# mackelab/poisson-gpfa

Measured on AMD Instinct MI355X. Metric: EM iterations/sec, higher is better.
Workload: dtype f64

## Files before the change

### poisson-gpfa_amd/csrc/core.hip

```cpp
#include "ctx.h"
#include "model.h"
#include "dual.h"
#include "thin.h"
#include "hook.h"
#include "plan.h"

using namespace pgpfa;

static_assert(plan::Dims{}.NB == NB && plan::Dims{}.WIDE_MAX == WIDE_MAX, "plan.h restates two constants of the kernel headers (workspace.hip includes none)");

thread_local std::string g_err;
thread_local unsigned long long g_fail_count = 0;

int fail(const char* fmt, ...) {
  char buf[1024];
  va_list ap;
  va_start(ap, fmt);
  vsnprintf(buf, sizeof(buf), fmt, ap);
  va_end(ap);
  g_err = buf;
  ++g_fail_count;
  return 1;
}

// ... 147 lines not shown
  c->dl_used = 0;
  return 0;
}
int dl_enqueue(pgpfa_ctx* c, void* host, const void* dev, size_t bytes) {
  if (bytes == 0) return 0;
  if (!c->dl_stage) {
    if (hipHostMalloc((void**)&c->dl_stage, DL_STAGE_BYTES, hipHostMallocMapped) != hipSuccess) { (void)hipGetLastError(); c->dl_stage = nullptr; }
    if (c->dl_stage && hipHostGetDevicePointer((void**)&c->dl_stage_dev, c->dl_stage, 0) != hipSuccess) { (void)hipGetLastError(); c->dl_stage_dev = nullptr; }
    if (!c->h_seq) {
      if (hipHostMalloc((void**)&c->h_seq, 64, hipHostMallocMapped) != hipSuccess ||
          hipHostGetDevicePointer((void**)&c->d_seq, c->h_seq, 0) != hipSuccess) { (void)hipGetLastError(); c->h_seq = nullptr; c->d_seq = nullptr; }
      if (c->h_seq) *c->h_seq = 0u;
    }
  }
  const size_t need = (bytes + 63) / 64 * 64;
  if (!c->dl_stage || need > DL_STAGE_BYTES) {
    CHK(dl_flush(c));
    const hipError_t e_copy = hipMemcpyAsync(host, dev, bytes, hipMemcpyDeviceToHost, c->st);
    if (e_copy != hipSuccess) return fail("device-to-host copy of %zu bytes: %s", bytes, hipGetErrorString(e_copy));
    return dl_flush(c);
  }
  dl_drop_stale(c);
  if (c->dl_used + need > DL_STAGE_BYTES) CHK(dl_flush(c));
  if (c->copy_kernels && c->dl_stage_dev && c->h_seq && bytes <= COPY_KERNEL_MAX && (bytes & 3) == 0 && (((size_t)dev) & 3) == 0) {
    const size_t nw = bytes / 4;
    hipLaunchKernelGGL(copy_words_kernel, dim3((unsigned)std::min<size_t>((nw + 255) / 256, 64)), dim3(256), 0, c->st,
                       reinterpret_cast<unsigned*>(c->dl_stage_dev + c->dl_used), reinterpret_cast<const unsigned*>(dev), nw);
    HIPC(hipGetLastError());
  } else {
    HIPC(hipMemcpyAsync(c->dl_stage + c->dl_used, dev, bytes, hipMemcpyDeviceToHost, c->st));
  }
  if (c->dl_pending.empty()) c->dl_fail_mark = g_fail_count;
  c->dl_pending.push_back({host, c->dl_used, bytes});
  c->dl_used += need;
  return 0;
}
int download(pgpfa_ctx* c, double* host, const double* dev, size_t n) {
  if (c->hbuf && host >= c->hbuf && host < c->hbuf + c->hbuf_len) {
    if (c->copy_kernels && n * sizeof(double) <= COPY_KERNEL_MAX) {
      CHK(dl_enqueue(c, host, dev, n * sizeof(double)));
      return dl_flush(c);
    }
    HIPC(hipMemcpyAsync(host, dev, n * sizeof(double), hipMemcpyDeviceToHost, c->st));
    return dl_flush(c);
  }
  CHK(dl_enqueue(c, host, dev, n * sizeof(double)));
  return dl_flush(c);
}
int upload(pgpfa_ctx* c, double* dev, const double* host, size_t n) {
  if (n * sizeof(double) <= (size_t)65536) return upload_nosync(c, dev, host, n * sizeof(double));
  HIPC(hipMemcpyAsync(dev, host, n * sizeof(double), hipMemcpyHostToDevice, c->st));
  HIPC(hipStreamSynchronize(c->st));
  c->ring_pending = 0;
  return 0;
}
constexpr int RING_N = 16;
int upload_nosync(pgpfa_ctx* c, void* dev, const void* host, size_t bytes) {
  if (bytes == 0) return 0;
  if (bytes > c->ring_slot) {
    HIPC(hipStreamSynchronize(c->st));
    if (c->ring) hipHostFree(c->ring);
    c->ring = nullptr; c->ring_dev = nullptr;
    const size_t slot = (bytes + 4095) / 4096 * 4096;
    HIPC(hipHostMalloc((void**)&c->ring, slot * RING_N, hipHostMallocMapped));
    if (hipHostGetDevicePointer((void**)&c->ring_dev, c->ring, 0) != hipSuccess) { (void)hipGetLastError(); c->ring_dev = nullptr; }
    c->ring_slot = slot; c->ring_cur = 0; c->ring_pending = 0;
  }
  if (c->ring_pending >= RING_N - 1) { HIPC(hipStreamSynchronize(c->st)); c->ring_pending = 0; }
  char* slot = c->ring + (size_t)c->ring_cur * c->ring_slot;
  std::memcpy(slot, host, bytes);
  if (c->copy_kernels && c->ring_dev && bytes <= COPY_KERNEL_MAX && (bytes & 3) == 0 && (((size_t)dev) & 3) == 0) {
    const size_t nw = bytes / 4;
    hipLaunchKernelGGL(copy_words_kernel, dim3((unsigned)std::min<size_t>((nw + 255) / 256, 64)), dim3(256), 0, c->st, reinterpret_cast<unsigned*>(dev),
                       reinterpret_cast<const unsigned*>(c->ring_dev + (size_t)c->ring_cur * c->ring_slot), nw);
    HIPC(hipGetLastError());
  } else {
    HIPC(hipMemcpyAsync(dev, slot, bytes, hipMemcpyHostToDevice, c->st));
  }
  c->ring_cur = (c->ring_cur + 1) % RING_N;
  c->ring_pending += 1;
  return 0;
}


int build_kinv(pgpfa_ctx* c) {
  c->kinv_serial += 1;
  const size_t slab = (size_t)c->Tp * c->Tp;
  CHK(copy_dev(c, c->kws.H, c->Kpad, slab * c->p * sizeof(double)));
  HIPC(hipMemsetAsync(c->kws.info, 0, sizeof(int) * c->p, c->st));
  CHK(factor(c, c->kws, nullptr, c->p));
  c->logdetK.assign(c->p, 0.0);
  hipLaunchKernelGGL(logdet_batch_kernel, dim3(c->p), dim3(256), 0, c->st, c->kws.H, (long long)c->kws.sH, c->Tp, c->Tp, c->tscal);
  CHK(download(c, c->logdetK.data(), c->tscal, c->p));
  CHK(inverse_t(c, c->kws, nullptr, c->p));
  GemmP g{};
  g.A = c->kws.Mt; g.sA = c->kws.sM; g.lda = c->Tp;
  g.B = c->kws.Mt; g.sB = c->kws.sM; g.ldb = c->Tp;
  g.C = c->Kinv; g.sC = slab; g.ldc = c->Tp;
  g.M = c->Tp; g.N = c->Tp; g.K = c->Tp; g.alpha = 1.0; g.beta = 0.0;
  g.slots = nullptr; g.nbatch = c->p; g.mode = GEMM_FULL; g.kflags = KF_BEGIN_MAXRC;
  CHK(gemm(c, false, g));
  std::vector<int> info(c->p);
  CHK(dl_enqueue(c, info.data(), c->kws.info, sizeof(int) * c->p));
  CHK(dl_flush(c));
  for (int k = 0; k < c->p; ++k)
    if (info[k] != 0) return fail("GP Gram matrix of latent %d is not positive definite (pivot %d)", k, info[k]);
  return 0;
}


int pivchol_launch(double* F, int Tf, int T, int p, const double* tau, double bin, double eps, double tol, bool pairs, int* rank, hipStream_t st, size_t* lds,
                   bool run) {
  const int rmax = std::min(T, Tf);
  const size_t shm = ((size_t)2 * T + rmax + 16) * sizeof(double) + 16 * sizeof(int);
  const int form = (T > 256 && pairs && Tf % 2 == 0) ? PIVCHOL_PAIRS : T > 256 ? PIVCHOL_512_2 : PIVCHOL_256_1;
  if (lds) *lds = form == PIVCHOL_PAIRS ? pivchol2_lds(T, rmax, 1024, 4) : shm;
  if (!run) return form;
  if (form == PIVCHOL_PAIRS)
    hipLaunchKernelGGL((rbf_pivchol2_kernel<256, 4>), dim3(p), dim3(1024), pivchol2_lds(T, rmax, 1024, 4), st, F, Tf, T, tau, bin, eps, tol, rmax, rank);
  else if (form == PIVCHOL_512_2)
    hipLaunchKernelGGL((rbf_pivchol_kernel<512, 2>), dim3(p), dim3(1024), shm, st, F, Tf, T, tau, bin, eps, tol, rmax, rank);
  else
    hipLaunchKernelGGL((rbf_pivchol_kernel<256, 1>), dim3(p), dim3(256), shm, st, F, Tf, T, tau, bin, eps, tol, rmax, rank);
  return form;
}

int launch_pivchol(pgpfa_ctx* c, hipStream_t st) {
  (void)pivchol_launch(c->Flr, c->Tp, c->T, c->p, c->tau, c->bin, c->eps, c->lr_tol, c->pivchol_pairs != 0, c->d_rank, st);
  HIPC(hipGetLastError());
  return 0;
}

ThinTables thin_tables(int p, int T, const int* rr, const int* rk, const int* roff, int rtot) {
  ThinTables tt;
  std::vector<int>&hft = tt.ft, &hf = tt.f, &hs = tt.s;
  for (int k = 0; k < p; ++k) {
    const int ngr = (rr[k] + 63) / 64, runs = rr[k] / 4;
    for (int g = 0, m0 = 0; g < ngr; ++g) {
      const int rows = 4 * (runs / ngr + (g < runs % ngr ? 1 : 0));
      hft.push_back(k); hft.push_back(m0); hft.push_back(rows); hft.push_back(roff[k]);
      m0 += rows;
    }
    for (int t0 = 0; t0 < T; t0 += 256) { hf.push_back(k); hf.push_back(t0); hf.push_back(rk[k]); hf.push_back(roff[k]); }
  }
  for (int m0 = 0; m0 < rtot; m0 += 64) { hs.push_back(0); hs.push_back(m0); hs.push_back(std::min(64, rtot - m0)); hs.push_back(0); }
  return tt;
}

RankLayout rank_layout(int p, const int* ranks, int gran, bool thin_all) {
  RankLayout L;
  const int G = ((gran == 4 || gran == 8) && thin_all) ? gran : 16;
  L.rk.assign(p, 0);
  L.roff.assign(p + 1, 0);
  L.rr.assign(p, 0);
  L.roff16.assign(p + 1, 0);
  int extent = 0;
  for (int k = 0; k < p; ++k) {
    L.rr[k] = round_up(std::max(ranks[k], 1), G);
    L.rk[k] = round_up(L.rr[k], 16);
    L.roff[k + 1] = L.roff[k] + L.rr[k];
    L.roff16[k + 1] = L.roff16[k] + L.rk[k];
    extent = std::max(extent, L.roff[k] + L.rk[k]);
  }
  L.rtot = L.roff[p];
  L.rtot16 = L.roff16[p];
  L.rank_compact = (G != 16);
// ... 4 lines not shown
  for (int k = 0; k < p; ++k)
    for (int b = L.roff16[k] / 16; b < L.roff16[k + 1] / 16; ++b) { L.blk_lat[b] = k; L.blk_col[b] = b * 16 - L.roff16[k]; }
  if (L.rank_compact) {
    const int n16 = round_up(L.rtot16, NB);
    std::vector<int> pmap(round_up(L.rtot, 16) + 16, 0);
    L.cmap.assign(n16, -1);
    for (int k = 0; k < p; ++k)
      for (int j = 0; j < L.rr[k]; ++j) { L.cmap[L.roff16[k] + j] = L.roff[k] + j; pmap[L.roff[k] + j] = L.roff16[k] + j; }
    L.nrtab.assign((round_up(L.rtot, 16)) / 16, 0);
    for (size_t b = 0; b < L.nrtab.size(); ++b) {
      const int last = std::min((int)b * 16 + 15, L.rtot - 1);
      L.nrtab[b] = std::min(L.rtot16, round_up(pmap[last] + 1, 16));
    }
    for (int i = 0; i + 1 < n16 && L.bad_pair < 0; i += 2)
      if (L.cmap[i] < 0 ? L.cmap[i + 1] >= 0 : ((L.cmap[i] & 1) != 0 || L.cmap[i + 1] != L.cmap[i] + 1)) L.bad_pair = i;
  }
  return L;
}

int build_lowrank(pgpfa_ctx* c, bool pivchol_launched) {
  const int p = c->p, T = c->T, Tp = c->Tp;
  if (pivchol_launched) HIPC(hipStreamWaitEvent(c->st, c->ev_join, 0));
  else CHK(launch_pivchol(c, c->st));
  std::vector<int> r(p);
  CHK(dl_enqueue(c, r.data(), c->d_rank, sizeof(int) * p));
  CHK(dl_flush(c));
  const bool thin_all = thin_possible(c) && c->thin_products >= 2;
  RankLayout rl = rank_layout(p, r.data(), c->rank_gran, thin_all);
  c->rk = rl.rk;
  c->roff = rl.roff;
  c->rr = rl.rr;
  c->roff16 = rl.roff16;
  c->rtot = rl.rtot;
  c->rtot16 = rl.rtot16;
  c->rank_compact = rl.rank_compact;
  c->rpad = rl.rpad;
  CHK(upload_list(c, c->d_blk_lat, rl.blk_lat));
  CHK(upload_list(c, c->d_blk_col, rl.blk_col));
  CHK(upload_list(c, c->d_roff, c->roff));
  CHK(upload_list(c, c->d_roff16, c->roff16));
  if (c->rank_compact) {
    if (rl.bad_pair >= 0) {
      const int i = rl.bad_pair;
      return fail("rank tables: padded rows %d, %d map to slab rows %d, %d - not a pair the panel staging can move whole", i, i + 1, rl.cmap[i], rl.cmap[i + 1]);
    }
    CHK(upload_list(c, c->d_cmap, rl.cmap));
    CHK(upload_list(c, c->d_nrtab, rl.nrtab));
  }
  {
    std::vector<int> tft, tf;
    c->kr_ft_len = 0; c->kr_f_len = 0;
    for (int k = 0; k < p; ++k) {
      const int kb = (k * T) / 16 * 16, ke = std::min(c->npad, round_up((k + 1) * T, 16));
      for (int r0 = c->roff[k]; r0 < c->roff[k + 1]; r0 += 64) { tft.push_back(r0); tft.push_back(c->roff[k + 1]); tft.push_back(kb); tft.push_back(ke); }
      c->kr_ft_len = std::max(c->kr_ft_len, ke - kb);
      for (int i0 = k * T; i0 < (k + 1) * T; i0 += 64) { tf.push_back(i0); tf.push_back((k + 1) * T); tf.push_back(c->roff[k]); tf.push_back(c->roff[k + 1]); }
      c->kr_f_len = std::max(c->kr_f_len, c->rk[k]);
    }
    c->ntab_ft = (int)tft.size() / 4; c->ntab_f = (int)tf.size() / 4;
    if (tft.size() > c->tab_cap || tf.size() > c->tab_cap) return fail("internal: row-tile table overflow");
    CHK(upload_list(c, c->d_kr_ft, tft));
    CHK(upload_list(c, c->d_kr_f, tf));
    const ThinTables tt = thin_tables(p, T, c->rr.data(), c->rk.data(), c->roff.data(), c->rtot);
    const std::vector<int>&hft = tt.ft, &hf = tt.f, &hs = tt.s;
    c->nthin_s = (int)hs.size() / 4;
    if (hs.size() > c->tab_cap) return fail("internal: thin-product table overflow");
    CHK(upload_list(c, c->d_thin_s, hs));
    c->nthin_ft = (int)hft.size() / 4; c->nthin_f = (int)hf.size() / 4;
    if (hft.size() > c->tab_cap || hf.size() > c->tab_cap) return fail("internal: thin-product table overflow");
    CHK(upload_list(c, c->d_thin_ft, hft));
    CHK(upload_list(c, c->d_thin_f, hf));
  }
  if ((size_t)c->rpad <= (size_t)c->ld) {
    HIPC(hipMemsetAsync(c->Fbig, 0, (size_t)c->ld * c->rpad * sizeof(double), c->st));
    HIPC(hipMemsetAsync(c->FTbig, 0, (size_t)c->rpad * c->ld * sizeof(double), c->st));
    int rkmax = 0;
    for (int k = 0; k < p; ++k) rkmax = std::max(rkmax, c->rk[k]);
    hipLaunchKernelGGL(build_fbig_kernel, dim3(rkmax, p), dim3(128), 0, c->st, c->Flr, Tp, T, c->d_roff, c->Fbig, c->ld, c->FTbig, c->rpad);
    HIPC(hipGetLastError());
  }
  c->info["lowrank_rtot"] = c->rtot;
  c->info["lowrank_rtot16"] = c->rtot16;
  c->info["lowrank_compact"] = c->rank_compact ? 1.0 : 0.0;
  c->flr32_valid = false;
  return 0;
}

BLayout b_layout_of(bool compact, int rtot16, int rpad, const int* cmap, const int* roff_padded, const int* nrtab) {
  const int n64 = round_up(rtot16, 64) / 64, d64 = rpad / 64;
  return compact ? BLayout{n64, n64 * (n64 + 1) / 2, cmap, roff_padded, nrtab, round_up(rtot16, (int)NB)}
                 : BLayout{d64, d64 * (d64 + 1) / 2, nullptr, roff_padded, nullptr, 0};
}
BLayout b_layout(const pgpfa_ctx* c) {
  return b_layout_of(c->rank_compact, c->rtot16, c->rpad, c->d_cmap, c->rank_compact ? c->d_roff16 : c->d_roff, c->d_nrtab);
}

namespace {
int thin_refuse(int code, const char* fmt, ...) {
  char buf[512];
  va_list ap;
  va_start(ap, fmt);
  vsnprintf(buf, sizeof(buf), fmt, ap);
  va_end(ap);
  (void)fail("pgpfa_test_thin refuses: %s", buf);
  return code;
}
}

int pgpfa_test_thin(pgpfa_ctx* c, int kind, int p, int T, int Tf, const int32_t* ranks, int gran, long long ldx, long long ldy, int Tx, int vec_f32, int nslots,
                    int ncols, const int32_t* cols, int live, int stop, double fill, const double* F, const double* Sb, const void* X, void* Y, int32_t* geom,
                    int tab_cap, int32_t* tab_ft, int32_t* tab_f, int32_t* tab_s, int32_t* ntab) {
  using namespace hook;
  if (!c || !ranks || !X || !Y || !geom || !tab_ft || !tab_f || !tab_s || !ntab) return thin_refuse(PGPFA_THIN_BAD_ARG, "null argument");
  if (kind < PGPFA_THIN_FT || kind > PGPFA_THIN_APPLY) return thin_refuse(PGPFA_THIN_BAD_ARG, "kind %d", kind);
  const bool use_f = kind != PGPFA_THIN_S, use_s = kind == PGPFA_THIN_S || kind == PGPFA_THIN_APPLY;
  if ((use_f && !F) || (use_s && !Sb)) return thin_refuse(PGPFA_THIN_BAD_ARG, "null argument");
  if (p < 1 || nslots < 1 || ncols < 1 || tab_cap < 4) return thin_refuse(PGPFA_THIN_BAD_ARG, "invalid sizes");
  if (gran != 4 && gran != 8 && gran != 16) return thin_refuse(PGPFA_THIN_BAD_ARG, "rank granularity %d (4, 8 or 16)", gran);
  if (vec_f32 && kind == PGPFA_THIN_S) return thin_refuse(PGPFA_THIN_BAD_ARG, "Sb u has no single-precision vectors");
  if (T < 4) return thin_refuse(PGPFA_THIN_REFUSED_T, "T = %d below 4 (the 4-bin runs of the vector loads are clamped to T - 4)", T);
  if (Tf < T || Tf % 4 != 0) return thin_refuse(PGPFA_THIN_BAD_ARG, "slab size Tf = %d below T = %d or no multiple of 4", Tf, T);
  std::vector<int> rr(p), rk(p), roff(p + 1, 0);
  int extent = 0;
  for (int k = 0; k < p; ++k) {
    if (ranks[k] < 1 || ranks[k] % 4 != 0) return thin_refuse(PGPFA_THIN_REFUSED_RANK, "rank %d of latent %d is no positive multiple of 4", ranks[k], k);
    rr[k] = round_up(std::max(ranks[k], 1), gran);
    rk[k] = round_up(rr[k], 16);
    if (rk[k] > Tf) return thin_refuse(PGPFA_THIN_REFUSED_RANK, "latent %d: %d rank columns do not fit a slab of %d", k, rk[k], Tf);
    roff[k + 1] = roff[k] + rr[k];
    extent = std::max(extent, roff[k] + rk[k]);
  }
  const int rtot = roff[p];
  if (rtot % 4 != 0) return thin_refuse(PGPFA_THIN_REFUSED_RANK, "rank total %d is no multiple of 4", rtot);
  const int rpad = round_up(std::max(rtot, extent), NB);
  const bool vec4 = T % 4 == 0;
  if (use_f) {
    if (Tx < T) return thin_refuse(PGPFA_THIN_REFUSED_TX, "latent stride Tx = %d below T = %d", Tx, T);
    if (vec4 && Tx % 4 != 0) return thin_refuse(PGPFA_THIN_REFUSED_TX, "latent stride Tx = %d is no multiple of 4 where T is one (vector loads)", Tx);
  } else {
    Tx = T;
  }
  const long long nrows = (long long)(p - 1) * Tx + T;
  const long long need_x = kind == PGPFA_THIN_FT || kind == PGPFA_THIN_APPLY ? nrows : rtot;
  const long long need_y = kind == PGPFA_THIN_F || kind == PGPFA_THIN_APPLY ? nrows : rtot;
  if (ldx < need_x || ldy < need_y) return thin_refuse(PGPFA_THIN_REFUSED_LD, "ldx = %lld, ldy = %lld below the rows read / written (%lld, %lld)", ldx, ldy, need_x, need_y);
  if (ldx % 4 != 0 || ldy % 4 != 0) return thin_refuse(PGPFA_THIN_REFUSED_LD, "ldx = %lld, ldy = %lld: no multiples of 4 (vector loads and stores)", ldx, ldy);
  if (ldx > (1ll << 24) || ldy > (1ll << 24)) return thin_refuse(PGPFA_THIN_REFUSED_LD, "leading dimension too large for a test");
  const long long ldr = std::max(ldx, ldy);
  const long long ld_rank = kind == PGPFA_THIN_FT ? ldy : kind == PGPFA_THIN_F ? ldx : kind == PGPFA_THIN_S ? std::min(ldx, ldy) : ldr;
  if (rpad > ld_rank) return thin_refuse(PGPFA_THIN_REFUSED_RPAD, "rpad = %d above the leading dimension %lld of the rank-space vectors", rpad, ld_rank);
  if (cols) {
    std::vector<char> seen(nslots, 0);
    for (int i = 0; i < ncols; ++i) {
      if (cols[i] < 0 || cols[i] >= nslots) return thin_refuse(PGPFA_THIN_REFUSED_COLS, "column list entry %d = %d outside the %d slots", i, cols[i], nslots);
      if (seen[cols[i]]) return thin_refuse(PGPFA_THIN_REFUSED_COLS, "column list names slot %d twice", cols[i]);
      seen[cols[i]] = 1;
    }
  } else if (ncols > nslots) {
    return thin_refuse(PGPFA_THIN_REFUSED_COLS, "%d columns of %d slots", ncols, nslots);
  }
  if (live < -1 || live > ncols) return thin_refuse(PGPFA_THIN_REFUSED_LIVE, "live count %d outside 0..%d", live, ncols);
  if (!c->mfma) return fail("the thin products run on the matrix cores (use_mfma = 1)");
  const ThinTables tt = thin_tables(p, T, rr.data(), rk.data(), roff.data(), rtot);
  if ((int)tt.ft.size() > tab_cap || (int)tt.f.size() > tab_cap || (int)tt.s.size() > tab_cap) return thin_refuse(PGPFA_THIN_BAD_ARG, "tables exceed tab_cap = %d", tab_cap);
  for (int k = 0; k < p; ++k) { geom[k] = rr[k]; geom[p + k] = rk[k]; }
  for (int k = 0; k <= p; ++k) geom[2 * p + k] = roff[k];
// ... 203 lines not shown
    (void)hipGetLastError();
    if (c->st2) { hipStreamDestroy(c->st2); c->st2 = nullptr; }
  }
  int rc = 0;
  const size_t slab = (size_t)c->Tp * c->Tp;
  rc |= dmalloc(c, &c->Y, (size_t)R * q * T);
  rc |= dmalloc(c, &c->C, (size_t)q * p); rc |= dmalloc(c, &c->d, q); rc |= dmalloc(c, &c->tau, p);
  rc |= dmalloc(c, &c->Kpad, slab * p); rc |= dmalloc(c, &c->Kinv, slab * p);
  rc |= dmalloc(c, &c->Xmode, (size_t)R * c->n + 64, true);
  rc |= dmalloc(c, &c->Xprev, (size_t)R * c->n + 64, true);
  c->mode_serial.assign(R, -10); c->prev_serial.assign(R, -10);
  c->info["last_log_evidence_sum"] = 0.0;
  rc |= dmalloc(c, &c->vsm, (size_t)R * T * p * p + 2048, true);
  rc |= dmalloc(c, &c->Pauto, slab * p, true);
  rc |= dmalloc(c, &c->Pacc, slab * p, true);
  c->gemm_part_len = (size_t)16 << 20;
  rc |= dmalloc(c, &c->gemm_part, c->gemm_part_len);
  c->qpad = round_up(q, 16);
  c->ccu_cols = round_up(p * (p + 1) / 2, 16);
  if (p <= 16) {
    dispatch_pw(p, [&](auto pw) { constexpr int PW = decltype(pw)::value; c->ccu_cols = round_up(PW * (PW + 1) / 2, 16); });
    rc |= dmalloc(c, &c->CCu, (size_t)c->qpad * c->ccu_cols + 64, true);
    rc |= dmalloc(c, &c->C16, (size_t)c->qpad * 16 + 64, true);
  }
  c->dual_npd = round_up(p * (p + 1) / 2, 16);
  c->dual_ncol = c->dual_npd + round_up(p, 16);
  rc |= dmalloc(c, &c->dual_tbl, (size_t)round_up(q, 128) * c->dual_ncol + 4096, true);
  rc |= dmalloc(c, &c->ppart, (size_t)p * (PACC_SPLITS + 1) * T * T + 256);
  c->vsmgp_ok.assign(R, 0);
  c->trial_snap.assign(R, -1);
  c->trial_dual.assign(R, 0);
  c->lam_resident.assign(R, 0);
  c->lam_valid.assign(R, 0);
  rc |= dmalloc(c, &c->Flr, slab * p + 256 * (size_t)c->Tp, true);
  rc |= dmalloc(c, &c->d_rank, p); rc |= dmalloc(c, &c->d_roff, p + 1); rc |= dmalloc(c, &c->d_roff16, p + 1);
  rc |= dmalloc(c, &c->d_cmap, (size_t)p * c->Tp + 2 * NB + 64); rc |= dmalloc(c, &c->d_nrtab, (size_t)p * c->Tp / 16 + 64);
  c->tab_cap = 4 * ((size_t)c->ld / 64 + 2 * (size_t)p + 4);
  rc |= dmalloc(c, &c->d_kr_ft, c->tab_cap); rc |= dmalloc(c, &c->d_kr_f, c->tab_cap);
  rc |= dmalloc(c, &c->sink, 128, true);
  rc |= dmalloc(c, &c->zero16, 2, true);
  rc |= dmalloc(c, &c->d_thin_ft, c->tab_cap); rc |= dmalloc(c, &c->d_thin_f, c->tab_cap); rc |= dmalloc(c, &c->d_thin_s, c->tab_cap);
  rc |= dmalloc(c, &c->Fbig, (size_t)c->ld * c->ld + 256 * (size_t)c->ld, true); rc |= dmalloc(c, &c->FTbig, (size_t)c->ld * c->ld + 256 * (size_t)c->ld, true);
  rc |= dmalloc(c, &c->Gbar, (size_t)T * p * p + 64); rc |= dmalloc(c, &c->Wtbar, (size_t)T * p * p + 64); rc |= dmalloc(c, &c->d_blk_lat, (size_t)p * c->Tp / 16 + 64); rc |= dmalloc(c, &c->d_blk_col, (size_t)p * c->Tp / 16 + 64);
  rc |= dmalloc(c, &c->vec, (size_t)q * (p + 1));
  rc |= dmalloc(c, &c->cdpart, (size_t)1024 * (p + 2) * q);
  rc |= dmalloc(c, &c->cdout, (size_t)(p + 2) * q + 8);
  rc |= dmalloc(c, &c->cdym, (size_t)(p + 1) * q + 8);
  rc |= dmalloc(c, &c->cdym_part, (size_t)1024 * (p + 1) * q);
  rc |= dmalloc(c, &c->last_trials, R);
  {
    const size_t NH = 1 + (size_t)(p + 1) + (size_t)(p + 1) * (p + 2) / 2;
    rc |= dmalloc(c, &c->cdhpart, (size_t)128 * NH * q);
    rc |= dmalloc(c, &c->cdhout, NH * q + 8);
    rc |= dmalloc(c, &c->cdcenter, (size_t)q * (p + 1));
    rc |= dmalloc(c, &c->cdpack, (size_t)q * (p + 3) + 8);
  }
  if (hipHostMalloc((void**)&c->h_pcg, 4 * sizeof(int), hipHostMallocMapped) != hipSuccess ||
      hipHostGetDevicePointer((void**)&c->d_hpcg, c->h_pcg, 0) != hipSuccess) { (void)hipGetLastError(); c->h_pcg = nullptr; c->d_hpcg = nullptr; }
  rc |= alloc_cholws(c, &c->kws, p * TAU_MULTI_MAX, c->Tp, true);
  c->kws.nact = round_up(T, 64);
  {
    const size_t nqmax = (size_t)p * TAU_MULTI_MAX;
    rc |= dmalloc(c, &c->tK, slab * nqmax); rc |= dmalloc(c, &c->tM, slab * nqmax); rc |= dmalloc(c, &c->tA1, slab * nqmax);
    rc |= dmalloc(c, &c->tA2, slab * nqmax);
    rc |= dmalloc(c, &c->tscal, 16 + 8 * nqmax); rc |= dmalloc(c, &c->tpart, 1024 + 64 * nqmax);
  }
  if (rc) { pgpfa_destroy(c); return 1; }
  e = hipStreamSynchronize(c->st);
  if (e != hipSuccess) { pgpfa_destroy(c); return fail("sync: %s", hipGetErrorString(e)); }
  if (const char* g = std::getenv("PGPFA_RANK_GRAN")) { const int v = std::atoi(g); if (v == 4 || v == 8 || v == 16) c->rank_gran = v; }
  c->info["n_pad"] = c->npad;
  c->info["counts_two_bytes"] = 0.0;
  c->info["trial_lengths_set"] = 0.0;
  c->info["observed_set"] = 0.0;
  c->info["observed_bins_set"] = 0.0;
  c->info["last_cd_unobserved_neurons"] = 0.0;
  c->info["arena_bytes"] = 0.0;
  c->info["last_eps_wt_norm"] = 0.0;
  c->info["last_eps_wt_rms"] = 0.0;
  c->info["last_split_cov"] = 0.0;
  c->info["last_syrk_tile"] = 0.0;
  c->info["last_split_sps"] = 0.0;
  c->info["last_cross_kernel"] = 0.0;
  c->info["last_mix_form"] = 0.0;
  c->info["last_yt_mix_fused"] = 0.0;
  c->info["last_cov_f32"] = 0.0;
  c->info["last_cov_f32_fallbacks"] = 0.0;
  for (const char* k : {"plan_ms_total", "plans", "set_params_calls", "last_retry_ms", "last_dense_retries", "last_param_step", "last_param_step_prev",
                        "last_fallback_no_descent", "last_fallback_line_search", "last_fallback_outer_cap", "arena_grow_ms_total", "last_cold_restarts"}) c->info[k] = 0.0;
  *out = c;
  return 0;
}

static void free_tables(LiveTables& L);

int pgpfa_destroy(pgpfa_ctx* c) {
  if (!c) return 0;
  hipSetDevice(c->device);
  if (c->st) hipStreamSynchronize(c->st);
  if (c->comm) ncclCommDestroy(c->comm);
  for (void* p : c->allocs) hipFree(p);
  if (c->vsmgp) hipFree(c->vsmgp);
  if (c->Flr32) hipFree(c->Flr32);
  if (c->lam_keep) hipFree(c->lam_keep);
  if (c->split_buf) hipFree(c->split_buf);
  if (c->Yhi) hipFree(c->Yhi);
  free_tables(c->live);
  if (c->trunc_q) hipFree(c->trunc_q);
  arena_release(c);
  if (c->hbuf) hipHostFree(c->hbuf);
  if (c->dl_stage) hipHostFree(c->dl_stage);
  if (c->hibuf) hipHostFree(c->hibuf);
  if (c->ring) hipHostFree(c->ring);
  if (c->h_pcg) hipHostFree(c->h_pcg);
  if (c->h_seq) hipHostFree(c->h_seq);
  for (auto e : c->prof.pool) hipEventDestroy(e);
  if (c->st2) { hipStreamSynchronize(c->st2); hipStreamDestroy(c->st2); }
  if (c->tau_pin) hipHostFree(c->tau_pin);
  if (c->ev_tau_fork) hipEventDestroy(c->ev_tau_fork);
  if (c->ev_tau_done) hipEventDestroy(c->ev_tau_done);
  if (c->ev_fork) hipEventDestroy(c->ev_fork);
  if (c->ev_join) hipEventDestroy(c->ev_join);
  if (c->st) hipStreamDestroy(c->st);
  delete c;
  return 0;
}

int pgpfa_set_option(pgpfa_ctx* c, const char* key, double v) {
  if (!c || !key) return fail("null argument");
  const std::string k(key);
  auto chunk_trials = [&](int* field) -> int {
    if (v < 0.0 || v != std::floor(v)) return fail("%s is a count of trials, or 0", key);
    *field = (int)v;
    return 0;
  };
  if (k == "newton_xtol") c->xtol = v;
  else if (k == "newton_max_iter") c->max_iter = (int)v;
  else if (k == "use_mfma") {
    const bool was = c->mfma;
    c->mfma = (v != 0.0);
    if (c->have_params && c->rank_gran != 16 && was != c->mfma)
      CHK(pgpfa_set_params(c, std::vector<double>(c->hC).data(), std::vector<double>(c->hd).data(), std::vector<double>(c->htau).data()));
  }
  else if (k == "cd_mfma") c->cd_mfma = (v != 0.0);
  else if (k == "cd_hess_mfma") c->cd_hess_mfma = (v != 0.0);
  else if (k == "cross_kernel") c->cross_kernel = (v != 0.0);
  else if (k == "cd_debug") c->cd_debug = (int)v;
  else if (k == "pcg_fused") c->pcg_fused = (int)v;
  else if (k == "pcg_w32") c->pcg_w32 = (v != 0.0);
  else if (k == "pcg_form") c->pcg_form = (int)v;
  else if (k == "pcg_vec32") c->pcg_vec32 = (int)v;
  else if (k == "pcg_rx32") c->pcg_rx32 = (int)v;
  else if (k == "pcg_adapt") c->pcg_adapt = (int)v;
  else if (k == "pcg_xcd") c->pcg_xcd = (int)v;
  else if (k == "mt_fill") c->mt_fill = (int)v;
  else if (k == "overlap_factors") c->overlap_factors = (int)v;
  else if (k == "mix_slot") c->mix_slot = (int)v;
  else if (k == "yt_mix") c->yt_mix = (v != 0.0);
  else if (k == "pivchol_pairs") c->pivchol_pairs = (v != 0.0);
  else if (k == "vsm_b4") c->vsm_b4 = (int)v;
  else if (k == "poisson_tiles") c->poisson_tiles = (int)v;
  else if (k == "yt_mix_dbg") c->yt_mix_dbg = (int)v;
  else if (k == "yt_mix_dma") c->yt_mix_dma = (v != 0.0);
  else if (k == "syrk_dbg") c->syrk_dbg = (int)v;
  else if (k == "syrk_tile") c->syrk_tile = (int)v;
  else if (k == "mix_wide") c->mix_wide = (int)v;
  else if (k == "thin_products") {
    const bool was = c->thin_products >= 2;
    c->thin_products = (int)v;
    if (c->have_params && c->rank_gran != 16 && was != (c->thin_products >= 2))
      CHK(pgpfa_set_params(c, std::vector<double>(c->hC).data(), std::vector<double>(c->hd).data(), std::vector<double>(c->htau).data()));
  }
  else if (k == "copy_kernels") c->copy_kernels = (v != 0.0);
  else if (k == "chord") c->chord = (v != 0.0);
  else if (k == "shared_pcg") c->shared_pcg = (v != 0.0);
  else if (k == "time_newton") c->time_newton = (v != 0.0);
  else if (k == "pcg_trace") c->pcg_trace = (v != 0.0);
  else if (k == "measure_mix") { c->measure_mix = (v != 0.0); c->info["last_eps_wt_norm"] = 0.0; c->info["last_eps_wt_rms"] = 0.0; }
  else if (k == "pcg_retire") c->pcg_retire = (v != 0.0);
  else if (k == "split_cov") c->split_cov = (v != 0.0);
  else if (k == "split_max_norm") c->split_max_norm = v;
  else if (k == "cov_mode") c->cov_mode = (int)v;
  else if (k == "lowrank_tol") {
    const bool changed = c->lr_tol != v;
    c->lr_tol = v;
    if (c->have_params && changed)
      CHK(pgpfa_set_params(c, std::vector<double>(c->hC).data(), std::vector<double>(c->hd).data(), std::vector<double>(c->htau).data()));
  }
  else if (k == "keep_trial_vsmgp") c->keep_trial_vsmgp = (v != 0.0);
  else if (k == "dual_lowrank") c->dual_lowrank = (v != 0.0);
  else if (k == "dual_f32") c->dual_f32 = (int)v;
  else if (k == "laplace_f32") { if (v != 0.0 && v != 1.0 && v != 2.0) return fail("laplace_f32 is 0, 1 or 2"); c->laplace_f32 = (int)v; }
  else if (k == "dual_masked") { if (v != 0.0 && v != 1.0) return fail("dual_masked is 0 or 1"); c->dual_masked = (int)v; }
  else if (k == "laplace_evidence") { if (v != 0.0 && v != 1.0) return fail("laplace_evidence is 0 or 1"); c->laplace_evidence = (int)v; }
  else if (k == "sample_chunk_trials") CHK(chunk_trials(&c->sample_chunk));
  else if (k == "interp_chunk_trials") CHK(chunk_trials(&c->interp_chunk));
  else if (k == "covat_chunk_trials") CHK(chunk_trials(&c->covat_chunk));
  else if (k == "velat_chunk_trials") CHK(chunk_trials(&c->velat_chunk));
  else if (k == "covat_block_times") { if (v < 0.0 || v != std::floor(v)) return fail("covat_block_times is a count of query times, or 0"); c->covat_block = (int)v; }
  else if (k == "func_chunk_trials") CHK(chunk_trials(&c->func_chunk));
  else if (k == "func_block_cols") {
    if (v < 0.0 || v != std::floor(v) || std::fmod(v, 16.0) != 0.0) return fail("func_block_cols is a count of functionals that is a multiple of 16, or 0");
    c->func_block = (int)v;
  }
  else if (k == "rates_chunk_trials") CHK(chunk_trials(&c->rates_chunk));
  else if (k == "counts_chunk_trials") CHK(chunk_trials(&c->counts_chunk));
  else if (k == "counts_nodes") { if (v < 8.0 || v > 64.0 || v != std::floor(v)) return fail("counts_nodes is a node count in 8 .. 64"); c->counts_Q = (int)v; }
  else if (k == "slab_row_align") c->slab_row_align = (v != 0.0);
  else if (k == "vsm_mfma") c->vsm_mfma = (v != 0.0);
  else if (k == "dual_gemm") c->dual_gemm = (v != 0.0);
  else if (k == "extrapolate_start") c->extrapolate = (v != 0.0);
  else if (k == "extrapolate_beta") c->extrapolate_beta = v;
  else if (k == "extrapolate_guard") c->extrapolate_guard = v;
  else if (k == "start_guard") c->start_guard = (v != 0.0);
  else if (k == "shared_min") c->shared_min = (int)v;
  else if (k == "pcg_inner") c->pcg_inner_max = std::max(1, (int)v);
  else if (k == "pcg_eta0") c->pcg_eta0 = v;
  else if (k == "splitk_target") c->splitk_target = std::max(1, (int)v);
  else if (k == "small_tile_below") c->small_tile_below = (int)v;
  else if (k == "f32_tile64") c->f32_tile64 = (int)v;
  else if (k == "splitk_below64") c->splitk_below64 = (int)v;
  else if (k == "pcg_outer_max") c->pcg_outer_max = (int)v;
  else if (k == "chord_xtol") c->chord_xtol = v;
  else if (k == "chord_rho") c->chord_rho = v;
  else if (k == "chord_max_step") c->chord_max_step = v;
  else if (k == "chord_max") c->chord_max = (int)v;
  else if (k == "chunk_trials") { if (c->B > 0) return fail("chunk_trials must be set before the first E-step"); c->chunk_opt = (int)v; }
  else if (k == "workspace_headroom") c->arena_headroom = std::max(1.0, v);
  else if (k == "rank_gran") { if (v != 4.0 && v != 8.0 && v != 16.0) return fail("rank_gran is 4, 8 or 16"); c->rank_gran = (int)v; if (c->have_params) CHK(pgpfa_set_params(c, std::vector<double>(c->hC).data(), std::vector<double>(c->hd).data(), std::vector<double>(c->htau).data())); }
// ... 555 lines not shown
```

### poisson-gpfa_amd/csrc/cov.hip

```cpp
#include "query.h"
#include "model.h"
#include "split.h"
#include "ytmix.h"
#include "hook.h"

using namespace pgpfa;

template <typename TIN>
void launch_post_vsm(pgpfa_ctx* c, const TIN* Mt, long long sM, int ncol, int ns, int full_range, const int* roff = nullptr, int ts = 0) {
  const int T = c->T, p = c->p;
  if (ts <= 0) ts = T;
  if (p > 10 && c->vsm_mfma) {
    const int CB = post_vsm_mfma_cb(p, sizeof(TIN) == 4);
    if (p <= 20 && c->vsm_b4) {
      constexpr int VW = 16 / (int)sizeof(TIN);
      const bool vec = c->vsm_b4 >= 2 && T % VW == 0 && ts % VW == 0 && c->ld % VW == 0 && sM % VW == 0 && (((size_t)Mt) & 15) == 0;
      auto go = [&](auto nbk, auto vv) {
        constexpr int NBK = decltype(nbk)::value;
        constexpr bool VEC = decltype(vv)::value;
        const size_t lds4 = (size_t)CB * post_vsm_b4_cs(p, VEC) * sizeof(TIN);
        constexpr int BINS = VEC ? 64 : 32;
        (void)hipFuncSetAttribute(reinterpret_cast<const void*>(&post_vsm_b4_kernel<NBK, TIN, VEC>), hipFuncAttributeMaxDynamicSharedMemorySize, (int)lds4);
        hipLaunchKernelGGL((post_vsm_b4_kernel<NBK, TIN, VEC>), dim3((T + BINS - 1) / BINS, ns), dim3(512), lds4, c->st, Mt, sM, c->ld, ncol, T, p, c->vsm,
                           c->ident, c->trial_of_slot, full_range, CB, roff, (int)GBN, ts);
      };
      auto gov = [&](auto nbk) { if (vec) go(nbk, std::true_type{}); else go(nbk, std::false_type{}); };
      if (p <= 12) gov(std::integral_constant<int, 3>{}); else if (p <= 16) gov(std::integral_constant<int, 4>{}); else gov(std::integral_constant<int, 5>{});
      return;
    }
    const size_t lds = (size_t)CB * p * 33 * sizeof(TIN);
    if (p <= 16)
      hipLaunchKernelGGL((post_vsm_mfma_kernel<1, TIN>), dim3((T + 31) / 32, ns), dim3(512), lds, c->st, Mt, sM, c->ld, ncol, T, p, c->vsm, c->ident,
                         c->trial_of_slot, full_range, CB, roff, (int)GBN, ts);
    else
      hipLaunchKernelGGL((post_vsm_mfma_kernel<2, TIN>), dim3((T + 31) / 32, ns), dim3(512), lds, c->st, Mt, sM, c->ld, ncol, T, p, c->vsm, c->ident,
                         c->trial_of_slot, full_range, CB, roff, (int)GBN, ts);
    return;
  }
  const int KY = post_vsm_rows(p);
  dispatch_pmax(p, [&](auto pm) {
    hipLaunchKernelGGL((post_vsm_kernel<decltype(pm)::value, TIN>), dim3((T + 63) / 64, ns), dim3(64, KY), 0, c->st, Mt, sM, c->ld, ncol, T, p, c->vsm,
                       c->ident, c->trial_of_slot, full_range, ts);
  });
}


int post_vsm_from_mt(pgpfa_ctx* c, int nslots) {
  launch_post_vsm(c, (const double*)c->ws.Mt, (long long)c->ws.sM, c->npad, nslots, 0);
  HIPC(hipGetLastError());
  return 0;
}

__global__ void scatter_vsmgp_kernel(const double* __restrict__ src, long long sSrc, double* __restrict__ dst, int T, int p, int k,
                                     const int* __restrict__ trial_of_slot) {
  const int slot = blockIdx.y;
  const size_t r = trial_of_slot[slot];
  const size_t e = (size_t)blockIdx.x * blockDim.x + threadIdx.x;
  if (e < (size_t)T * T) {
    const size_t a = e % T, b = e / T;
    dst[(r * p + k) * T * T + e] = (a >= b) ? src[(size_t)slot * sSrc + e] : src[(size_t)slot * sSrc + a * T + b];
  }
}


int ensure_mt_clean(pgpfa_ctx* c) {
  if (!c->mt_dirty) return 0;
  HIPC(hipMemsetAsync(c->ws.Mt, 0, (size_t)c->ws.sM * c->B * sizeof(double), c->st));
  c->mt_dirty = false;
  return 0;
}

int ensure_vsmgp_buffer(pgpfa_ctx* c) {
  if (c->vsmgp) return 0;
  const size_t bytes = (size_t)c->R * c->p * c->T * c->T * sizeof(double);
  void* ptr = nullptr;
  hipError_t e = hipMalloc(&ptr, bytes);
  if (e != hipSuccess) { (void)hipGetLastError(); return fail("hipMalloc(%zu bytes) for the per-trial post_vsmGP blocks failed: %s", bytes, hipGetErrorString(e)); }
  e = hipMemsetAsync(ptr, 0, bytes, c->st);
  if (e != hipSuccess) { hipFree(ptr); return fail("hipMemset failed: %s", hipGetErrorString(e)); }
  c->vsmgp = reinterpret_cast<double*>(ptr);
  c->bytes += bytes;
  return 0;
}

int ensure_evidence_buffers(pgpfa_ctx* c) {
  if (!c->ldet_buf) CHK(dmalloc(c, &c->ldet_buf, (size_t)c->B * c->T + 16));
  if (!c->evid_ld) CHK(dmalloc(c, &c->evid_ld, (size_t)c->B));
  return 0;
}

static int posterior_blocks_dense(pgpfa_ctx* c, int nb, double diag_scale, bool want_vsmgp, double* ld_dev) {
  const int T = c->T, p = c->p;
  c->info["last_cov_f32"] = 0.0;
  CHK(ensure_mt_clean(c));
  c->last_cov_lowrank = false;
  CHK(assemble(c, c->ident, nb, diag_scale));
  CHK(factor(c, c->ws, c->ident, nb));
  if (ld_dev) {
    double ldk = 0.0;
    for (double v : c->logdetK) ldk += v;
    hipLaunchKernelGGL(evidence_logdet_kernel, dim3(nb), dim3(256), 0, c->st, (const double*)nullptr, 0, c->ws.H, (long long)c->ws.sH, c->ld, c->npad, ldk, ld_dev);
  }
  CHK(inverse_t(c, c->ws, c->ident, nb));
  if (want_vsmgp) {
    CHK(ensure_vsmgp_buffer(c));
    for (int k = 0; k < p; ++k) {
      const int kal = (k * T) / 16 * 16;
      GemmP g{};
      g.A = c->ws.Mt + (size_t)kal * c->ld + (size_t)k * T; g.sA = c->ws.sM; g.lda = c->ld;
      g.B = g.A; g.sB = c->ws.sM; g.ldb = c->ld;
      g.C = c->ws.H; g.sC = c->ws.sH; g.ldc = T;
      g.M = T; g.N = T; g.K = c->npad - kal; g.alpha = 1.0; g.beta = 0.0;
      g.slots = c->ident; g.nbatch = nb; g.mode = GEMM_LOWER; g.kflags = KF_BEGIN_MAXRC;
      CHK(gemm(c, false, g));
      hipLaunchKernelGGL(scatter_vsmgp_kernel, dim3((unsigned)(((size_t)T * T + 255) / 256), nb), dim3(256), 0, c->st, c->ws.H, c->ws.sH, c->vsmgp,
                         T, p, k, c->trial_of_slot);
    }
  }
  prof_begin(c, TAG_VSM, (double)nb * c->npad * c->npad * p);
  launch_post_vsm(c, (const double*)c->ws.Mt, (long long)c->ws.sM, c->npad, nb, 0);
  prof_end(c);
  HIPC(hipGetLastError());
  return 0;
}


constexpr int SPLIT_NS = 256;

static int split_syrk_launch(pgpfa_ctx* c, const float* D, long long sD, int ldd, int Ts, int T, int p, int ract, int nb, int sps_req, int tile_req, double* part,
                             int* tile_used, int* sps_out, int* ngroups_out) {
  const int sps = sps_req > 0 ? sps_req : std::max(1, (nb + PACC_SPLITS - 1) / PACC_SPLITS);
  const int ngroups = (nb + sps - 1) / sps;
  SyrkF16Args a{};
  a.D = D; a.sD = sD; a.ldd = ldd; a.ts = Ts; a.part = part;
  a.T = T; a.p = p; a.ract = ract; a.nslots = nb; a.sps = sps; a.ngroups = ngroups;
  a.dbg = c->syrk_dbg;
  const int t256 = (T + 255) / 256;
  const bool big = tile_req >= 256 && T > 256 && (Ts & 3) == 0 && (ldd & 3) == 0 && t256 * 256 <= Ts && (((size_t)D) & 15) == 0 && (sD & 3) == 0;
  a.tiles = big ? t256 : (T + 127) / 128; a.ntiles = a.tiles * (a.tiles + 1) / 2;
  const long long blocks = (long long)a.ntiles * ngroups * p;
  prof_begin(c, TAG_VSM, 3.0 * (double)nb * ract * T * T * p);
  if (big) {
    const size_t lds = (size_t)4 * 2 * 256 * 32 * sizeof(_Float16);
    (void)hipFuncSetAttribute(reinterpret_cast<const void*>(&syrk256_f16x2_kernel), hipFuncAttributeMaxDynamicSharedMemorySize, (int)lds);
    hipLaunchKernelGGL(syrk256_f16x2_kernel, dim3((unsigned)blocks), dim3(512), lds, c->st, a);
  } else {
    hipLaunchKernelGGL(syrk_f16x2_kernel, dim3((unsigned)blocks), dim3(256), 0, c->st, a);
  }
  prof_end(c);
  *tile_used = big ? 256 : 128;
  *sps_out = sps;
  *ngroups_out = ngroups;
  return 0;
}

static int split_latent_sums(pgpfa_ctx* c, const double* A0, long long sM, int lda, const float* Dk, long long sD, int ldd, int rk, int kw, int T, int nb, int sps,
                             bool cross, double* Spart, double* Xpart, double* Ssum, double* Xsum, int* cross_used) {
  const int ngroups = (nb + sps - 1) / sps;
  const int spsS = std::max(1, (nb + SPLIT_NS - 1) / SPLIT_NS);
  auto seg = [&](int sper, bool is_x, double* out) -> int {
    const int nfull = nb / sper, rem = nb - nfull * sper;
    for (int part = 0; part < 2; ++part) {
      const int first = part ? nfull * sper : 0, per = part ? rem : sper, ng = part ? (rem ? 1 : 0) : nfull;
      if (ng == 0 || per == 0) continue;
      GemmP g{};
      g.A = A0 + (size_t)first * sM; g.sA = (long long)per * sM; g.lda = lda;
      g.kseg = kw; g.sAseg = sM;
      g.K = per * kw; g.alpha = 1.0; g.beta = 0.0; g.slots = nullptr; g.nbatch = ng; g.kflags = 0; g.bm = 64;
      g.M = rk;
      if (is_x) {
        g.B = reinterpret_cast<const double*>(Dk + (size_t)first * sD);
        g.sB = (long long)per * sD; g.ldb = ldd; g.sBseg = sD; g.b_f32 = 1;
        g.N = T; g.mode = GEMM_FULL;
        g.C = out + (size_t)(part ? nfull : 0) * rk * T; g.sC = (long long)rk * T; g.ldc = rk;
      } else {
        g.B = g.A; g.sB = g.sA; g.ldb = lda; g.sBseg = sM;
        g.N = rk; g.mode = GEMM_LOWER;
        g.C = out + (size_t)(part ? nfull : 0) * rk * rk; g.sC = (long long)rk * rk; g.ldc = rk;
      }
      CHK(gemm(c, false, g));
    }
    return 0;
  };
  CHK(seg(spsS, false, Spart));
  const bool use_cross = cross && c->mfma && rk % 16 == 0 && kw % 16 == 0;
  if (use_cross) {
    for (int row0 = 0; row0 < rk; row0 += 128) {
      CrossArgs ca{};
      ca.A = A0; ca.sM = sM; ca.lda = lda;
      ca.D = Dk; ca.sD = sD; ca.ldd = ldd;
      ca.C = Xpart; ca.sC = (long long)rk * T;
      ca.rk = std::min(128, rk - row0); ca.T = T; ca.kw = kw; ca.nslots = nb; ca.sps = sps;
      ca.row0 = row0; ca.ldc = rk;
      prof_begin(c, TAG_GEMM, 2.0 * (double)nb * ca.rk * (double)kw * T);
      cross_term_launch<float, false>(ca, dim3((T + 63) / 64, ngroups), c->st);
      prof_end(c);
    }
    HIPC(hipGetLastError());
  } else {
    CHK(seg(sps, true, Xpart));
  }
  const int ngS = (nb + spsS - 1) / spsS;
  hipLaunchKernelGGL(sum_groups_kernel, dim3((unsigned)(((size_t)rk * rk + 63) / 64)), dim3(256), 0, c->st, Spart, ngS, rk, rk, 32, Ssum);
  hipLaunchKernelGGL(sum_groups_kernel, dim3((unsigned)(((size_t)rk * T + 63) / 64)), dim3(256), 0, c->st, Xpart, ngroups, rk, T, 0, Xsum);
  *cross_used = use_cross ? 1 : 0;
  return 0;
}

template <typename TB>
void assemble_rxr_launch(TB* Bm, long long sB, int rpad, int rtot, int nact, const BLayout& L, const TB* F, int Tf, int T, int p, const int* blk_lat,
                         const int* blk_col, const double* Wt, long long sW, const int* slots, int nb, hipStream_t st) {
  hipLaunchKernelGGL(assemble_b_kernel_t<TB>, dim3(L.npairs, (nb + AB_SLOTS - 1) / AB_SLOTS), dim3(256), 0, st, Bm, sB, rpad, L.nblk64, F, Tf, T, p,
                     blk_lat, blk_col, Wt, sW, slots, nb, L.cmap);
  if (L.cmap && rpad > rtot)
    hipLaunchKernelGGL(pad_identity_kernel<TB>, dim3((rpad + 3) / 4, nb), dim3(256), 0, st, Bm, sB, rpad, rtot, rpad, nact, (int)NB, slots);
}

template <typename TB>
int assemble_rxr(pgpfa_ctx* c, const CholWS& view, int nb, const TB* F, const double* Wt, long long sW, const int* slots) {
  TB* Bm = reinterpret_cast<TB*>(view.H);
  assemble_rxr_launch<TB>(Bm, view.sH, c->rpad, c->rtot, view.nact, b_layout(c), F, c->Tp, c->T, c->p, c->d_blk_lat, c->d_blk_col, Wt, sW, slots, nb, c->st);
  HIPC(hipGetLastError());
  return 0;
}
template int assemble_rxr<double>(pgpfa_ctx*, const CholWS&, int, const double*, const double*, long long, const int*);
template int assemble_rxr<float>(pgpfa_ctx*, const CholWS&, int, const float*, const double*, long long, const int*);

namespace {

template <typename T>
int clear_and_invert(pgpfa_ctx* c, const CholWS& w, int nb, int lower_ctile = 0) {
  const int rpad = c->rpad;
  constexpr bool f32 = sizeof(T) == 4;
  if constexpr (f32)
    hipLaunchKernelGGL(fill_slabs_f32_kernel, dim3((unsigned)(((size_t)rpad * rpad + 1023) / 1024), nb), dim3(256), 0, c->st, reinterpret_cast<float*>(w.Mt), w.sM,
                       (size_t)rpad * rpad, 0.0f);
  else if (lower_ctile > 0)
    hipLaunchKernelGGL(clear_lower_reads_kernel, dim3(c->p, nb), dim3(256), 0, c->st, w.Mt, w.sM, rpad, c->d_roff, lower_ctile, c->ident);
  else
    hipLaunchKernelGGL(fill_slabs_kernel, dim3((unsigned)(((size_t)rpad * rpad + 1023) / 1024), nb), dim3(256), 0, c->st, w.Mt, w.sM, (size_t)rpad * rpad, 0.0);
  return inverse_t(c, w, c->ident, nb, f32);
}

struct CovPass {
  int nb;
  bool want_vsmgp, accumulate;
  int ract;
  long long sW;
  bool split_candidate;
  unsigned* norm_bits;
  int f32_mode;
  bool f32, lap32;
  bool skip_zero_cols;
  int ctile;
  int Ts;
  CholWS lw;
  CholWS lwf;
  float* Ytf;
};

CovPass cov_pass(const pgpfa_ctx* c, int nb, bool want_vsmgp, bool accumulate, bool allow_lap32) {
  const int T = c->T, p = c->p;
  CovPass P{};
  P.nb = nb; P.want_vsmgp = want_vsmgp; P.accumulate = accumulate;
  P.ract = round_up(c->rtot, 16);
  P.sW = (long long)T * p * p;
  P.split_candidate = want_vsmgp && accumulate && c->split_cov && c->mfma && (p <= 16 || (p <= 20 && c->mix_wide));
  P.norm_bits = reinterpret_cast<unsigned*>(c->pcg_ratio);
  P.f32_mode = want_vsmgp ? (allow_lap32 ? c->laplace_f32 : 0) : c->dual_f32;
  P.f32 = P.f32_mode != 0;
  P.lap32 = P.f32 && want_vsmgp;
  P.skip_zero_cols = want_vsmgp ? p <= 16 : (p > 10 && c->vsm_mfma);
  P.ctile = (want_vsmgp && p <= 16) ? 16 : (int)GBN;
  P.Ts = (c->slab_row_align && p * round_up(T, 16) <= c->ld) ? round_up(T, 16) : T;
  P.lw = lowrank_view(c, c->ws);
  P.lwf = P.lw;
  if (P.f32) {
    P.lwf.H = P.lw.Mt; P.lwf.sH = 2 * P.lw.sM;
    P.lwf.Mt = P.lw.H; P.lwf.sM = 2 * P.lw.sH;
    P.lwf.sD = 2 * P.lw.sD; P.lwf.sP = 2 * P.lw.sP;
    P.Ytf = reinterpret_cast<float*>(P.lw.H) + (size_t)c->rpad * c->rpad;
  }
  return P;
}


struct SplitScratch {
  double *Spart, *Xpart, *Ssum, *Xsum, *Zb, *T1, *Xfull;
  float* D;
  long long sD;
  int ldd;
};

int split_scratch(pgpfa_ctx* c, const CholWS& lw, SplitScratch* s) {
  const int T = c->T, p = c->p;
  const size_t tt = (size_t)T * T;
  constexpr int NS = SPLIT_NS, NG = PACC_SPLITS + 1;
  const size_t tq = (size_t)round_up(T, 16) * round_up(T, 16);
  if (!c->split_buf) {
    const size_t len = ((size_t)NS + NG + 3) * tq + 2 * (size_t)p * tt + 1024;
    if (hipMalloc((void**)&c->split_buf, len * sizeof(double)) != hipSuccess) { (void)hipGetLastError(); c->split_buf = nullptr; return fail("out of device memory for the split accumulation (%zu bytes)", len * sizeof(double)); }
    c->bytes += len * sizeof(double);
  }
  s->Spart = c->split_buf;
  s->Xpart = s->Spart + (size_t)NS * tq;
  s->Ssum = s->Xpart + (size_t)NG * tq;
  s->Xsum = s->Ssum + tq;
  s->Zb = s->Xsum + tq;
  s->T1 = s->Zb + tq;
  s->Xfull = s->T1 + (size_t)p * tt;
  s->D = reinterpret_cast<float*>(lw.H + (size_t)c->ld * c->rpad);
  s->sD = 2 * (long long)lw.sH;
  s->ldd = c->ld;
  return 0;
}

int mix_split(pgpfa_ctx* c, const CovPass& P, const SplitScratch& s, bool fused) {
  const int T = c->T, p = c->p, Tp = c->Tp, rpad = c->rpad, nb = P.nb, ract = P.ract, Ts = P.Ts, ctile = P.ctile, ldd = s.ldd;
  const long long sW = P.sW, sD = s.sD;
  const CholWS& lw = P.lw;
  float* D = s.D;
  int mix_form = 0;
  double mix_cols = 0.0;
  for (int k = 0; k < p; ++k) mix_cols += std::max(0, ract - (ctile > 0 ? (c->roff[k] / ctile) * ctile : 0));
  if (fused) {
    prof_begin(c, TAG_MIX, (double)nb * T * ((double)ract * ract + 16.0 * ract + (double)ract * (2.0 * p * p + p * (p + 1.0))));
    dispatch_pw(p, [&](auto pw) {
      constexpr int PW = decltype(pw)::value;
      if constexpr (PW <= 10) {
        YtMixArgs a{};
        a.F = c->Flr; a.Tp = Tp; a.Mts = lw.Mt; a.sM = (long long)lw.sM; a.rpad = rpad;
        a.D = D; a.sD = sD; a.ldd = ldd; a.G = c->Gbin; a.sG = sW;
        a.T = T; a.p = p; a.ract = ract; a.nbx = (T + YTM_BINS - 1) / YTM_BINS; a.nslots = nb; a.eps = c->eps;
        a.vsm = c->vsm; a.slots = c->ident; a.trial_of_slot = c->trial_of_slot; a.ts = Ts; a.dbg = c->yt_mix_dbg;
        const BLayout L = b_layout(c);
        a.roff = L.roff_padded; a.cmap = L.cmap; a.nrtab = L.nrtab;
        a.ncmap = L.ncmap_rows;
        if (ytmix_lds(PW) + (size_t)a.ncmap * sizeof(int) > (size_t)160 * 1024) a.ncmap = 0;
        const size_t lds = ytmix_lds(PW) + (size_t)a.ncmap * sizeof(int);
        a.zero16 = c->zero16;
        const bool dma = c->yt_mix_dma && c->zero16 && (!a.cmap || a.ncmap > 0) && rpad % 2 == 0 && lw.sM % 2 == 0 && (reinterpret_cast<uintptr_t>(lw.Mt) & 15) == 0;
        auto launch = [&](auto kern) {
          (void)hipFuncSetAttribute(reinterpret_cast<const void*>(kern), hipFuncAttributeMaxDynamicSharedMemorySize, (int)lds);
          hipLaunchKernelGGL(kern, dim3((unsigned)(a.nbx * nb)), dim3(YTM_THREADS), lds, c->st, a);
        };
        if (dma) launch(&yt_mix_kernel<PW, true>); else launch(&yt_mix_kernel<PW, false>);
      }
    });
    prof_end(c);
    mix_form = 4;
  } else {
  prof_begin(c, TAG_MIX, (double)nb * T * (mix_cols * 8.0 + (double)p * ract * 4.0));
  mix_form = p > 16 ? 5 : 0;
  if (p > 16)
    hipLaunchKernelGGL((mix_vsm_wide2_kernel<20, true>), dim3((T + 63) / 64, nb), dim3(256), 0, c->st, lw.H, (long long)lw.sH, c->ld, c->Gbin, sW, T, p, ract, c->eps,
                       c->vsm, c->ident, c->trial_of_slot, Ts, c->sink, D, sD, ldd);
  else
  dispatch_pw(p, [&](auto pw) {
    constexpr int PW = decltype(pw)::value;
    if constexpr (PW <= 10) {
      if (c->mix_slot >= 3 && p == PW && ract % 4 == 0) {
        (void)hipFuncSetAttribute(reinterpret_cast<const void*>(&mix_slot3_kernel<PW, 128, 2>), hipFuncAttributeMaxDynamicSharedMemorySize, (int)mix_slot_lds(PW, 128));
        hipLaunchKernelGGL((mix_slot3_kernel<PW, 128, 2>), dim3((T + 127) / 128, nb), dim3(256), mix_slot_lds(PW, 128), c->st, (const double*)lw.H, (long long)lw.sH, c->ld, D, sD, ldd,
                           c->Gbin, sW, T, ract, c->eps, c->vsm, c->ident, c->trial_of_slot, c->d_roff, ctile, Ts);
        mix_form = 3;
        return;
      }
      if (c->mix_slot >= 2 && p == PW && ract % 4 == 0) {
        (void)hipFuncSetAttribute(reinterpret_cast<const void*>(&mix_slot2_kernel<PW, 256, 2>), hipFuncAttributeMaxDynamicSharedMemorySize, (int)mix_slot_lds(PW, 256));
        hipLaunchKernelGGL((mix_slot2_kernel<PW, 256, 2>), dim3((T + 255) / 256, nb), dim3(256), mix_slot_lds(PW, 256), c->st, (const double*)lw.H, (long long)lw.sH, c->ld, D, sD, ldd,
                           c->Gbin, sW, T, ract, c->eps, c->vsm, c->ident, c->trial_of_slot, c->d_roff, ctile, Ts);
        mix_form = 2;
        return;
      }
      if (c->mix_slot) {
        (void)hipFuncSetAttribute(reinterpret_cast<const void*>(&mix_slot_kernel<PW, 256, 2>), hipFuncAttributeMaxDynamicSharedMemorySize, (int)mix_slot_lds(PW, 256));
        hipLaunchKernelGGL((mix_slot_kernel<PW, 256, 2>), dim3((T + 255) / 256, nb), dim3(256), mix_slot_lds(PW, 256), c->st, (const double*)lw.H, (long long)lw.sH, c->ld, D, sD, ldd,
                           c->Gbin, sW, T, p, ract, c->eps, c->vsm, c->ident, c->trial_of_slot, c->d_roff, ctile, Ts);
        mix_form = 1;
        return;
      }
    }
    if constexpr (PW <= 16)
      hipLaunchKernelGGL(mix_vsm_split_kernel<PW>, dim3((T + 63) / 64, nb), dim3(256), 0, c->st, (const double*)lw.H, (long long)lw.sH, c->ld, D, sD, ldd,
                         c->Gbin, sW, T, p, ract, c->eps, c->vsm, c->ident, c->trial_of_slot, c->d_roff, ctile, Ts);
  });
  prof_end(c);
  }
  return mix_form;
}

int split_latent_terms(pgpfa_ctx* c, const CovPass& P, const SplitScratch& s, int sps, bool* cross_ran_out) {
  const int T = c->T, p = c->p, Tp = c->Tp, rpad = c->rpad, nb = P.nb, ract = P.ract, Ts = P.Ts, ldd = s.ldd;
  const size_t tt = (size_t)T * T;
  const long long sD = s.sD;
  const CholWS& lw = P.lw;
  float* D = s.D;
  double *Spart = s.Spart, *Xpart = s.Xpart, *Ssum = s.Ssum, *Xsum = s.Xsum, *Zb = s.Zb, *T1 = s.T1, *Xfull = s.Xfull;
  bool cross_ran = false;
  for (int k = 0; k < p; ++k) {
    const int rk = c->rk[k], r0 = c->roff[k] & ~15;
    const int rrow = c->roff[k];
    const int kw = ract - r0;
    if (kw <= 0 || rk <= 0) {
      HIPC(hipMemsetAsync(T1 + (size_t)k * tt, 0, tt * sizeof(double), c->st));
      HIPC(hipMemsetAsync(Xfull + (size_t)k * tt, 0, tt * sizeof(double), c->st));
      continue;
    }
    const double* A0 = lw.Mt + rrow + (size_t)r0 * rpad;
    int cross_used = 0;
    CHK(split_latent_sums(c, A0, (long long)lw.sM, rpad, D + (size_t)k * Ts + (size_t)r0 * ldd, sD, ldd, rk, kw, T, nb, sps, c->cross_kernel, Spart, Xpart, Ssum, Xsum,
                          &cross_used));
    cross_ran = cross_ran || cross_used != 0;
    const double* Fk = c->Flr + (size_t)k * Tp * Tp;
    GemmP z{};
    z.A = Fk; z.lda = Tp; z.B = Ssum; z.ldb = rk; z.C = Zb; z.ldc = T;
    z.M = T; z.N = rk; z.K = rk; z.alpha = 1.0; z.beta = 0.0; z.nbatch = 1; z.mode = GEMM_FULL;
    CHK(gemm(c, true, z));
    GemmP t1 = z;
    t1.A = Zb; t1.lda = T; t1.B = Fk; t1.ldb = Tp; t1.C = T1 + (size_t)k * tt; t1.ldc = T; t1.N = T;
    CHK(gemm(c, false, t1));
    GemmP xf = z;
    xf.B = Xsum; xf.ldb = rk; xf.C = Xfull + (size_t)k * tt; xf.ldc = T; xf.N = T;
    CHK(gemm(c, true, xf));
  }
  *cross_ran_out = cross_ran;
  return 0;
}

int accumulate_split(pgpfa_ctx* c, const CovPass& P, bool fused) {
  const int T = c->T, p = c->p;
  SplitScratch s{};
  CHK(split_scratch(c, P.lw, &s));
  c->info["last_mix_form"] = (double)mix_split(c, P, s, fused);
  int sps = 0, ngroups = 0, tile_used = 0;
  CHK(split_syrk_launch(c, s.D, s.sD, s.ldd, P.Ts, T, p, P.ract, P.nb, 0, c->syrk_tile, c->ppart, &tile_used, &sps, &ngroups));
  c->info["last_syrk_tile"] = (double)tile_used;
  c->info["last_split_sps"] = (double)sps;
  bool cross_ran = false;
  CHK(split_latent_terms(c, P, s, sps, &cross_ran));
  c->info["last_cross_kernel"] = cross_ran ? 1.0 : 0.0;
  const int nt64 = (T + PACC_TS - 1) / PACC_TS;
  hipLaunchKernelGGL(pacc_split_reduce_kernel, dim3(nt64 * (nt64 + 1) / 2, p), dim3(256), 0, c->st, s.T1, s.Xfull, c->ppart, ngroups, c->Gbin, P.sW, P.nb, c->eps, T, c->Tp,
                     p, c->Pacc);
  HIPC(hipGetLastError());
  c->pacc_used = true;
  return 0;
}


int blocks_and_norm(pgpfa_ctx* c, const CovPass& P, double* ldet) {
  CHK(bin_blocks(c, c->W, P.sW, c->Gbin, c->Wt, P.sW, P.nb, ldet));
  if (P.split_candidate || c->measure_mix) {
    HIPC(hipMemsetAsync(P.norm_bits, 0, 4 * sizeof(unsigned), c->st));
    const long long nblk = (long long)P.nb * c->T;
    hipLaunchKernelGGL(block_norm_max_kernel, dim3((unsigned)std::min<long long>((nblk * c->p + 255) / 256, 2048)), dim3(256), 0, c->st, c->Wt, nblk, c->p, c->eps,
                       P.norm_bits, reinterpret_cast<double*>(P.norm_bits + 2));
  }
  return 0;
}

int ensure_f32_factors(pgpfa_ctx* c) {
  const size_t nf = (size_t)c->Tp * c->Tp * c->p;
  if (!c->Flr32) {
    if (hipMalloc((void**)&c->Flr32, (nf + 256 * (size_t)c->Tp) * sizeof(float)) != hipSuccess) { (void)hipGetLastError(); return fail("out of device memory for the single-precision factors"); }
    c->flr32_valid = false;
  }
  if (!c->flr32_valid) {
    hipLaunchKernelGGL(cvt_f32_kernel, dim3((unsigned)((nf + 255) / 256)), dim3(256), 0, c->st, c->Flr, c->Flr32, nf);
    c->flr32_valid = true;
  }
  return 0;
}

int assemble_and_factor(pgpfa_ctx* c, const CovPass& P) {
  const int rpad = c->rpad, nb = P.nb;
  HIPC(hipMemsetAsync(c->ws.info, 0, sizeof(int) * nb, c->st));
  if (P.f32_mode == 1) CHK(assemble_rxr<float>(c, P.lwf, nb, c->Flr32, c->Wt, P.sW, c->ident));
  else CHK(assemble_rxr<double>(c, P.lw, nb, c->Flr, c->Wt, P.sW, c->ident));
  if (!P.f32) return factor(c, P.lw, c->ident, nb);
  if (P.f32_mode != 1)
    hipLaunchKernelGGL(cvt_lower_f32_kernel, dim3((unsigned)(((size_t)rpad * rpad + 1023) / 1024), nb), dim3(256), 0, c->st, P.lw.H, P.lw.sH,
                       reinterpret_cast<float*>(P.lwf.H), P.lwf.sH, rpad);
  c->mt_dirty = true;
  return factor(c, P.lwf, c->ident, nb, true, P.lap32);
}

int log_determinants(pgpfa_ctx* c, const CovPass& P, double* logdet_out, double* ld_dev) {
  const int T = c->T, rpad = c->rpad, nb = P.nb;
  const CholWS &lw = P.lw, &lwf = P.lwf;
  if (ld_dev) {
    if (P.f32) return fail("internal: log evidence requested from a single-precision factor");
    hipLaunchKernelGGL(evidence_logdet_kernel, dim3(nb), dim3(256), 0, c->st, (const double*)c->ldet_buf, T, lw.H, (long long)lw.sH, rpad, rpad, 0.0, ld_dev);
  }
  if (logdet_out) {
    std::vector<double> a(nb), b2(nb);
    hipLaunchKernelGGL(sum_rows_kernel, dim3(nb), dim3(256), 0, c->st, c->ldet_buf, T, c->sc_f);
    CHK(download(c, a.data(), c->sc_f, nb));
    if (P.f32)
      hipLaunchKernelGGL(logdet_batch_f32_kernel, dim3(nb), dim3(256), 0, c->st, reinterpret_cast<const float*>(lwf.H), (long long)lwf.sH, rpad, rpad,
                         c->sc_f);
    else
      hipLaunchKernelGGL(logdet_batch_kernel, dim3(nb), dim3(256), 0, c->st, lw.H, (long long)lw.sH, rpad, rpad, c->sc_f);
    CHK(download(c, b2.data(), c->sc_f, nb));
    double ldk = 0.0;
    for (double v : c->logdetK) ldk += v;
    for (int s2 = 0; s2 < nb; ++s2) logdet_out[s2] = -ldk + a[s2] + b2[s2];
  }
  return 0;
}

template <typename T>
int yt_product(pgpfa_ctx* c, const CovPass& P, const T* F, const T* Linv, long long sL, T* Yt, long long sY) {
  const int Tp = c->Tp, rpad = c->rpad;
  for (int k = 0; k < c->p; ++k) {
    const int c0 = P.skip_zero_cols ? (c->roff[k] / P.ctile) * P.ctile : 0;
    if (c0 >= P.ract) continue;
    GemmP g{};
    g.A = reinterpret_cast<const double*>(F + (size_t)k * Tp * Tp); g.sA = 0; g.lda = Tp;
    g.B = reinterpret_cast<const double*>(Linv + c->roff[k] + (size_t)c0 * rpad); g.sB = sL; g.ldb = rpad;
    g.C = reinterpret_cast<double*>(Yt + (size_t)k * P.Ts + (size_t)c0 * c->ld); g.sC = sY; g.ldc = c->ld;
    g.M = c->T; g.N = P.ract - c0; g.K = c->rk[k]; g.alpha = 1.0; g.beta = 0.0;
    g.slots = c->ident; g.nbatch = P.nb; g.mode = GEMM_FULL; g.kflags = 0;
// ... 87 lines not shown
      hipLaunchKernelGGL((mix_vsm_wide2_kernel<20, false>), dim3((T + 63) / 64, nb), dim3(256), 0, c->st, lw.H, (long long)lw.sH, c->ld, c->Gbin, sW, T, p, ract, c->eps,
                         c->vsm, c->ident, c->trial_of_slot, Ts, c->sink, (float*)nullptr, 0LL, 0);
    } else {
      const int bins = wide_bins(p);
      hipLaunchKernelGGL(mix_vsm_wide_kernel, dim3((T + bins - 1) / bins, nb), dim3(bins * 32), wide_lds_bytes(p, bins, 1), c->st, lw.H, lw.sH,
                         c->ld, c->Gbin, sW, T, p, ract, c->eps, c->vsm, c->ident, c->trial_of_slot, bins, Ts);
    }
  });
  prof_end(c);
  return 0;
}

int pacc_sum(pgpfa_ctx* c, const CovPass& P) {
  const int T = c->T, p = c->p, nb = P.nb, ract = P.ract;
  const CholWS& lw = P.lw;
  const int sps = std::max(1, (nb + PACC_SPLITS - 1) / PACC_SPLITS);
  const int nfull = nb / sps, rem = nb - nfull * sps, nsplit = nfull + (rem ? 1 : 0);
  auto launch = [&](int first_slot, int slots_per, int ngroups, int part_first) -> int {
    GemmP g{};
    g.A = lw.H + (size_t)first_slot * lw.sH; g.sA = (long long)slots_per * lw.sH; g.lda = c->ld;
    g.B = g.A; g.sB = g.sA; g.ldb = c->ld;
    g.C = c->ppart + (size_t)part_first * T * T; g.sC = (long long)T * T; g.ldc = T;
    g.M = T; g.N = T; g.K = slots_per * ract; g.alpha = 1.0; g.beta = 0.0;
    g.slots = nullptr; g.nb_lo = ngroups; g.nbatch = ngroups * p;
    g.sA_hi = P.Ts; g.sB_hi = P.Ts; g.sC_hi = (long long)nsplit * T * T;
    g.kseg = ract; g.sAseg = lw.sH; g.sBseg = lw.sH;
    g.mode = GEMM_LOWER; g.kflags = 0;
    return gemm(c, false, g);
  };
  if (nfull) CHK(launch(0, sps, nfull, 0));
  if (rem) CHK(launch(nfull * sps, rem, 1, nfull));
  hipLaunchKernelGGL(pacc_reduce_kernel, dim3(T, p), dim3(128), 0, c->st, c->ppart, nsplit, c->Gbin, P.sW, nb, c->eps, T, c->Tp, p, c->Pacc);
  c->pacc_used = true;
  return 0;
}

int trial_blocks(pgpfa_ctx* c, const CovPass& P) {
  const int T = c->T, p = c->p, rpad = c->rpad, nb = P.nb;
  const CholWS& lw = P.lw;
  CHK(ensure_vsmgp_buffer(c));
  const size_t off_stage = (size_t)c->ld * rpad + (size_t)c->Tp * rpad;
  for (int k = 0; k < p; ++k) {
    GemmP g{};
    g.A = lw.H + (size_t)k * P.Ts; g.sA = lw.sH; g.lda = c->ld;
    g.B = g.A; g.sB = lw.sH; g.ldb = c->ld;
    g.C = lw.H + off_stage; g.sC = lw.sH; g.ldc = T;
    g.M = T; g.N = T; g.K = P.ract; g.alpha = 1.0; g.beta = 0.0;
    g.slots = c->ident; g.nbatch = nb; g.mode = GEMM_LOWER; g.kflags = 0;
    CHK(gemm(c, false, g));
    hipLaunchKernelGGL(scatter_vsmgp_lr_kernel, dim3((unsigned)(((size_t)T * T + 255) / 256), nb), dim3(256), 0, c->st, lw.H + off_stage, lw.sH, T,
                       c->vsmgp, T, p, k, c->Gbin, P.sW, c->eps, c->trial_of_slot);
  }
  return 0;
}

}

static int posterior_blocks_lowrank_impl(pgpfa_ctx* c, int nb, bool want_vsmgp, bool accumulate, double* logdet_out, bool allow_lap32, double* ld_dev) {
  c->last_cov_lowrank = true;
  const CovPass P = cov_pass(c, nb, want_vsmgp, accumulate, allow_lap32);
  CHK(blocks_and_norm(c, P, (logdet_out || ld_dev) ? c->ldet_buf : nullptr));
  c->info["last_cov_f32"] = P.lap32 ? 1.0 : 0.0;
  if (P.f32) CHK(ensure_f32_factors(c));
  CHK(assemble_and_factor(c, P));
  CHK(log_determinants(c, P, logdet_out, ld_dev));
  c->mt_dirty = true;
  if (P.f32 && !P.lap32) return dual_f32_tail(c, P);
  if (P.lap32) {
    bool redo = false;
    CHK(lap32_inverse(c, P, &redo));
    if (redo) return posterior_blocks_lowrank_impl(c, nb, want_vsmgp, accumulate, logdet_out, false, ld_dev);
  } else {
    CHK(clear_and_invert<double>(c, P.lw, nb, (P.skip_zero_cols && c->mt_fill) ? P.ctile : 0));
  }
  if (c->p > WIDE_MAX) return fail("low-rank covariance engine supports up to %d latents (p=%d)", WIDE_MAX, c->p);
  const bool fuse_candidate = P.split_candidate && c->yt_mix && c->mfma && c->p <= 10 && (P.ract == c->rtot || (c->rank_compact && P.ract <= P.lw.nact));
  bool split = false;
  if (fuse_candidate) CHK(split_verdict(c, P, &split));
  const bool fused = fuse_candidate && split;
  c->info["last_yt_mix_fused"] = fused ? 1.0 : 0.0;
  if (!fused) CHK(yt_product<double>(c, P, c->Flr, P.lw.Mt, P.lw.sM, P.lw.H, P.lw.sH));
  if (!fuse_candidate) CHK(split_verdict(c, P, &split));
  c->info["last_split_cov"] = split ? 1.0 : 0.0;
  if (!split) for (const char* key : {"last_syrk_tile", "last_split_sps", "last_cross_kernel", "last_mix_form"}) c->info[key] = 0.0;
  if (!want_vsmgp) CHK(vsm_from_yt<double>(c, P, P.lw.H, P.lw.sH));
  else if (split) CHK(accumulate_split(c, P, fused));
  else {
    CHK(mix_in_place(c, P));
    CHK(accumulate ? pacc_sum(c, P) : trial_blocks(c, P));
  }
  HIPC(hipGetLastError());
  return 0;
}

int posterior_blocks_lowrank(pgpfa_ctx* c, int nb, bool want_vsmgp, bool accumulate, double* logdet_out, double* ld_dev) {
  return posterior_blocks_lowrank_impl(c, nb, want_vsmgp, accumulate, logdet_out, true, ld_dev);
}

int posterior_blocks(pgpfa_ctx* c, int nb, double diag_scale, bool want_vsmgp, bool accumulate, double* ld_dev) {
  if (c->plan_lowrank) {
    if (diag_scale != 1.0) return fail("internal: jittered covariance requested under the low-rank workspace plan");
    return posterior_blocks_lowrank(c, nb, want_vsmgp, accumulate, nullptr, ld_dev);
  }
  return posterior_blocks_dense(c, nb, diag_scale, want_vsmgp, ld_dev);
}


int posterior_factor_only(pgpfa_ctx* c, int nb, double diag_scale) {
  if (!c->plan_lowrank) {
    CHK(ensure_mt_clean(c));
    CHK(assemble(c, c->ident, nb, diag_scale));
    CHK(factor(c, c->ws, c->ident, nb));
    CHK(inverse_t(c, c->ws, c->ident, nb));
    HIPC(hipGetLastError());
    return 0;
  }
  if (diag_scale != 1.0) return fail("internal: jittered factor requested under the low-rank workspace plan");
  if (c->p > WIDE_MAX) return fail("low-rank covariance engine supports up to %d latents (p=%d)", WIDE_MAX, c->p);
  const long long sW = (long long)c->T * c->p * c->p;
  CHK(bin_blocks(c, c->W, sW, c->Gbin, c->Wt, sW, nb, nullptr));
  const CholWS lw = lowrank_view(c, c->ws);
  CHK(assemble_rxr<double>(c, lw, nb, c->Flr, c->Wt, sW, c->ident));
  CHK(factor(c, lw, c->ident, nb));
  c->mt_dirty = true;
  CHK(clear_and_invert<double>(c, lw, nb));
  HIPC(hipGetLastError());
  return 0;
}

static int get_rows(pgpfa_ctx* c, int n, const int32_t* idx, const double* src, size_t len, double* out) {
  if (!c || !out) return fail("null argument");
  HIPC(hipSetDevice(c->device));
  Trials tr;
  CHK(resolve_trials(c, n, idx, &tr));
  for (size_t i = 0; i < tr.v.size(); ++i)
    CHK(dl_enqueue(c, out + i * len, src + (size_t)tr.v[i] * len, len * sizeof(double)));
  CHK(dl_flush(c));
  return 0;
}
int pgpfa_get_post_mean(pgpfa_ctx* c, int n, const int32_t* idx, double* out) { return get_rows(c, n, idx, c ? c->Xmode : nullptr, c ? (size_t)c->n : 0, out); }
int pgpfa_get_post_vsm(pgpfa_ctx* c, int n, const int32_t* idx, double* out) {
  return get_rows(c, n, idx, c ? c->vsm : nullptr, c ? (size_t)c->T * c->p * c->p : 0, out);
}


int resident_curvature(pgpfa_ctx* c, const std::vector<int>& tos, bool dual, const char* where, const std::function<int(double diag_scale)>& finish) {
  const int nb = (int)tos.size();
  const size_t m = (size_t)c->q * c->T;
  CHK(upload_list(c, c->trial_of_slot, tos));
  HIPC(hipMemsetAsync(c->ws.info, 0, sizeof(int) * nb, c->st));
  double scale = 1.0;
  if (dual) {
    for (int s = 0; s < nb; ++s)
      HIPC(hipMemcpyAsync(c->lamd + (size_t)s * m, c->lam_keep + (size_t)tos[s] * m, m * sizeof(double), hipMemcpyDeviceToDevice, c->st));
    std::vector<double> sB, sD, vKv;
    CHK(dual_common(c, nb, &sB, &sD, &vKv));
    if (c->plan_lowrank) CHK(dual_jitter(c, nb));
    else CHK(dual_dense_scale(c, nb, &scale));
  } else {
    hipLaunchKernelGGL(gather_rows_kernel, dim3((c->n + 255) / 256, nb), dim3(256), 0, c->st, c->Xmode, c->n, c->Xc, (long long)c->ld,
                       c->trial_of_slot, 0);
    CHK(poisson(c, c->ident, nb, c->Xc, c->Gl, c->W, c->sc_f, 1));
  }
  CHK(finish(scale));
  std::vector<int> info(nb);
  CHK(dl_enqueue(c, info.data(), c->ws.info, sizeof(int) * nb));
  CHK(dl_flush(c));
// ... 273 lines not shown
```

### poisson-gpfa_amd/csrc/ctx.h

```cpp
#pragma once
#include <hip/hip_runtime.h>
#include <rccl/rccl.h>

#include <algorithm>
#include <limits>
#include <chrono>
#include <cmath>
#include <cstdarg>
#include <cstdio>
#include <cstring>
#include <deque>
#include <functional>
#include <map>
#include <string>
#include <type_traits>
#include <vector>

#include <mutex>
#include <rocprofiler-sdk-roctx/roctx.h>
#include "../../include/pgpfa.h"
#include "types.h"
#include "live.h"

namespace pgpfa { struct ThinP; }
using namespace pgpfa;


extern thread_local std::string g_err;
extern thread_local unsigned long long g_fail_count;

int fail(const char* fmt, ...);

#define HIPC(expr)                                                                         \
  do {                                                                                     \
    hipError_t _e = (expr);                                                                \
    if (_e != hipSuccess) return fail("%s:%d %s -> %s", __FILE__, __LINE__, #expr, hipGetErrorString(_e)); \
  } while (0)
#define CHK(expr)            \
  do {                       \
    int _r = (expr);         \
    if (_r != 0) return _r;  \
  } while (0)

inline int round_up(int v, int m) { return (v + m - 1) / m * m; }

struct PhaseRange {
  explicit PhaseRange(const char* name) { roctxRangePushA(name); }
  ~PhaseRange() { roctxRangePop(); }
  PhaseRange(const PhaseRange&) = delete;
  PhaseRange& operator=(const PhaseRange&) = delete;
};

struct Prof {
  bool on = false;
  bool configured = false;
  int only_tag = -1;
  std::vector<hipEvent_t> pool;
  std::vector<hipEvent_t> idle;
  struct Rec { int tag; hipEvent_t e0, e1; double flops; std::string shape; };
  std::deque<Rec> recs;
  bool open = false;
  std::map<int, double> ms, flops, count;
  std::map<int, double> max_ms, max_flops;
  struct Shape { double ms = 0.0, flops = 0.0, count = 0.0; };
  std::map<std::string, Shape> shapes;
};
constexpr int TAU_MULTI_MAX = 4;
constexpr int PACC_SPLITS = 64;
enum { TAG_GEMM = 0, TAG_POTRF = 1, TAG_SOLVE = 2, TAG_POISSON = 3, TAG_ASSEMBLE = 4, TAG_VSM = 5, TAG_CD = 6, TAG_MIX = 7, TAG_N };


struct pgpfa_ctx {
  int device = 0, q = 0, p = 0, T = 0, R = 0, n = 0, npad = 0, ld = 0, Tp = 0;
  double bin = 10.0, eps = 1e-3;
  hipStream_t st = nullptr;
  double* tau_pin = nullptr; hipEvent_t ev_tau_fork = nullptr, ev_tau_done = nullptr; int tau_inflight = 0;
  hipStream_t st2 = nullptr;
  hipEvent_t ev_fork = nullptr, ev_join = nullptr;
  int overlap_factors = 1;
  double xtol = 1e-5;
  int max_iter = 60;
  bool chord = true;
  double chord_xtol = 1e-9, chord_rho = 0.6, chord_max_step = 1.0;
  int chord_max = 40;
  bool mfma = true;
  int chunk_opt = 0;
  uint8_t* Y = nullptr;
  uint8_t* Yhi = nullptr;
  LiveTables live;
  double *C = nullptr, *d = nullptr, *tau = nullptr;
  double *Kpad = nullptr, *Kinv = nullptr;
  double* Xmode = nullptr;
  double* Xprev = nullptr;
  std::vector<int> mode_serial, prev_serial;
  int estep_serial = 0;
  bool extrapolate = true;
  double extrapolate_beta = 1.0;
  std::vector<double> estepC, estepd, esteptau;
  double par_step = -1.0, par_step_prev = -1.0;
  double extrapolate_guard = 3.0;
  bool start_guard = true;
  double* vsm = nullptr;
  double* vsmgp = nullptr;
  double* Pauto = nullptr;
  double* Pacc = nullptr;
  double* gemm_part = nullptr; size_t gemm_part_len = 0;
  bool no_splitk = false;
  double *CCu = nullptr, *C16 = nullptr;
  int qpad = 0, ccu_cols = 0;
  double* ppart = nullptr;
  double* split_buf = nullptr;
  bool split_cov = true;
  double split_max_norm = 0.07;
  double *cdym = nullptr, *cdym_part = nullptr;
  bool cdym_valid = false, cd_mfma = true, cd_hess_mfma = true; int cd_debug = 0;
  bool cd_hess_valid = false;
  std::vector<double> logdetK;
  bool dual_lowrank = true;
  double* dual_tbl = nullptr; int dual_ncol = 0, dual_npd = 0; bool dual_gemm = true;
  bool vsm_mfma = true;
  bool slab_row_align = true;
  int dual_f32 = 0;
  float* Flr32 = nullptr; bool flr32_valid = false;
  int laplace_f32 = 0;
  int dual_masked = 0;
  double* trunc_q = nullptr;
  std::vector<double> trunc_ld;
  int kinv_serial = 0, trunc_serial = -1;
  int laplace_evidence = 0;
  double* evid_ld = nullptr;
  std::vector<double> log_evidence;
  std::vector<int> evid_serial;
  bool keep_trial_vsmgp = false;
  bool pacc_used = false, pacc_valid = false;
  std::vector<char> vsmgp_ok;
  std::vector<double> hC, hd, htau;
  struct ParamSnap { std::vector<double> C, d, tau; };
  std::map<int, ParamSnap> snaps;
  std::vector<int> trial_snap;
  std::vector<char> trial_dual;
  std::vector<char> lam_resident;
  std::vector<char> lam_valid;
  double* lam_keep = nullptr;
  int snap_serial = 0;
  double *vec = nullptr, *cdpart = nullptr, *cdout = nullptr;
  double *cdhpart = nullptr, *cdhout = nullptr, *cdcenter = nullptr, *cdpack = nullptr;
  int* last_trials = nullptr;
  std::vector<int> last_trials_h;
  bool have_counts = false, have_params = false, have_post = false, have_precomp = false;
  double n_trials_global = 0.0;
  int B = 0;
  double grow_budget_ms = 200.0;
  int grow_floor_slots = 128;
  bool use_pool = true;
  int plan_target = 0;
  int want_slots = 0;
  bool B_capped = false;
  CholWS ws{};
  double *Xc = nullptr, *Xt = nullptr, *KX = nullptr, *KD = nullptr, *Gl = nullptr, *Glt = nullptr, *Gt = nullptr, *Dl = nullptr;
  double *W = nullptr, *Wt = nullptr, *fpart = nullptr;
  double *lamd = nullptr, *dgrad = nullptr, *dpart = nullptr, *ldet_buf = nullptr;
  double* voff = nullptr;
  bool var_active = false, lam_out_active = false;
  double* dual_scr = nullptr; long long dual_sscr = 0;
  CholWS sws{};
  double *sU = nullptr, *sDinvT = nullptr, *Wbar = nullptr;
  double *Rv = nullptr, *Zv = nullptr, *Pv = nullptr, *Qv = nullptr;
  PcgCtl* pcgctl = nullptr;
  int* live0 = nullptr; float *pcg_ratio = nullptr, *pcg_eta = nullptr;
  int* live1 = nullptr;
  int* pcg_blk = nullptr;
  const int* cur_ndev = nullptr;
  bool live_gemm_collect = false;
  std::vector<std::pair<std::string, double>> live_gemms;
  bool pcg_retire = true;
  int* h_pcg = nullptr; int* d_hpcg = nullptr;
  float* W32 = nullptr;
  double* sc_part2 = nullptr;
  int pcg_fused = 1; bool pcg_w32 = true;
  int mt_fill = 1;
  int pcg_xcd = 1;
  int pcg_adapt = 1;
  int pcg_form = 2;
  int pcg_rx32 = 1;
  int pcg_vec32 = 1;
  double *Sv = nullptr, *cg_scal = nullptr;
  double *GbT = nullptr, *WbT = nullptr;
  double *sc_rz = nullptr, *sc_pq = nullptr, *sc_rr = nullptr, *sc_rr0 = nullptr, *sc_pack = nullptr;
  double* Flr = nullptr;
  double* Gbin = nullptr;
  int *d_rank = nullptr, *d_blk_lat = nullptr, *d_blk_col = nullptr, *d_roff = nullptr;
  int *d_kr_ft = nullptr, *d_kr_f = nullptr;
  int kr_ft_len = 0, kr_f_len = 0;
  int ntab_ft = 0, ntab_f = 0; size_t tab_cap = 0;
// ... 153 lines not shown
void dispatch_obs(int state, F&& f) {
  switch (state) {
    case 2: f(std::integral_constant<int, 2>{}); break;
    case 1: f(std::integral_constant<int, 1>{}); break;
    default: f(std::integral_constant<int, 0>{}); break;
  }
}

template <typename F>
void dispatch_pmax(int p, F&& f) {
  if (p <= 4) f(std::integral_constant<int, 4>{});
  else if (p <= 8) f(std::integral_constant<int, 8>{});
  else if (p <= 16) f(std::integral_constant<int, 16>{});
  else if (p <= 24) f(std::integral_constant<int, 24>{});
  else f(std::integral_constant<int, 32>{});
}

inline int post_vsm_rows(int p) { return p <= 16 ? p : (p <= 24 ? 12 : 16); }
inline int poisson_rows(int p) { return p <= 16 ? p : (p <= 20 ? 10 : 16); }

struct Trials {
  std::vector<int> v;
};

struct LooJob {
  const std::vector<int>* mask;
  double* y_pred;
  double* err;
};

struct VarJob {
  double* rho;
  int max_outer;
  double tol;
  double* fopt;
  int32_t* outer;
  int32_t* vstatus;
  int start;
  double* lam_out;
};


int alloc_cholws(pgpfa_ctx* c, pgpfa::CholWS* w, int nslots, int npad, bool with_mt, size_t slab_elems = 0, bool zero_mt = true, size_t mt_elems = 0);
bool lowrank_pays(const pgpfa_ctx* c);
bool want_lowrank(const pgpfa_ctx* c);
int free_workspace(pgpfa_ctx* c);
int arena_grow(pgpfa_ctx* c, size_t need, double budget_ms = 0.0, size_t must = 0);
void arena_release(pgpfa_ctx* c, bool unmap = false);
int ensure_workspace(pgpfa_ctx* c, bool plan_lr);
int ensure_hbuf(pgpfa_ctx* c, size_t len);
int ensure_hibuf(pgpfa_ctx* c, size_t len);
void prof_harvest(Prof& P, bool all);
hipEvent_t prof_event(Prof& P);
void prof_begin(pgpfa_ctx* c, int tag, double flops);
void prof_end(pgpfa_ctx* c);
void prof_collect(pgpfa_ctx* c);
int upload_list(pgpfa_ctx* c, int* dst, const std::vector<int>& v);
int copy_dev(pgpfa_ctx* c, void* dst, const void* src, size_t bytes);
int dl_flush(pgpfa_ctx* c);
int dl_enqueue(pgpfa_ctx* c, void* host, const void* dev, size_t bytes);
int download(pgpfa_ctx* c, double* host, const double* dev, size_t n);
int upload(pgpfa_ctx* c, double* dev, const double* host, size_t n);
int upload_nosync(pgpfa_ctx* c, void* dev, const void* host, size_t bytes);
int build_kinv(pgpfa_ctx* c);
int launch_pivchol(pgpfa_ctx* c, hipStream_t st);
enum { PIVCHOL_256_1 = 0, PIVCHOL_512_2 = 1, PIVCHOL_PAIRS = 2 };
int pivchol_launch(double* F, int Tf, int T, int p, const double* tau, double bin, double eps, double tol, bool pairs, int* rank, hipStream_t st,
                   size_t* lds = nullptr, bool run = true);
int build_lowrank(pgpfa_ctx* c, bool pivchol_launched = false);
struct ThinTables { std::vector<int> ft, f, s; };
ThinTables thin_tables(int p, int T, const int* rr, const int* rk, const int* roff, int rtot);
int resolve_trials(pgpfa_ctx* c, int n, const int32_t* idx, Trials* out, bool distinct = false);
void counts_changed(pgpfa_ctx* c, const std::vector<int>* trials);
int refuse_tables(const pgpfa_ctx* c, const char* entry, int allowed = 0, int with_dual_masked = 0);
int ensure_high_plane(pgpfa_ctx* c);
int ready(pgpfa_ctx* c);
int ready_estep(pgpfa_ctx* c, bool allow_lowrank);
void snapshot_params(pgpfa_ctx* c, const std::vector<int>& trials);
int with_snapshot(pgpfa_ctx* c, int id, const std::function<int()>& fn);
int remember_trials(pgpfa_ctx* c, const std::vector<int>& v);
int get_slabs(pgpfa_ctx* c, const double* src, double* out);
double gemm_flops(const pgpfa::GemmP& g);
int gemm(pgpfa_ctx* c, bool transb, pgpfa::GemmP g, bool f32 = false);
int factor(pgpfa_ctx* c, const pgpfa::CholWS& w, const int* slots, int nb, bool f32 = false, bool wide_diag = false);
int inverse_t(pgpfa_ctx* c, const pgpfa::CholWS& w, const int* slots, int nb, bool f32 = false);
int poisson(pgpfa_ctx* c, const int* d_list, int nl, const double* X, double* G, double* W, double* flik, int full);
int prior_mv(pgpfa_ctx* c, const int* d_list, int nl, const double* in, double* out, const double* mat = nullptr);
int prior_mv_all(pgpfa_ctx* c, int nb, const double* in, double* out, const double* mat = nullptr, const int* skip = nullptr,
                 const int* cols = nullptr, int ncols = 0);
int assemble(pgpfa_ctx* c, const int* d_list, int nl, double diag_scale = 1.0);
int bin_blocks(pgpfa_ctx* c, const double* W, long long sW, double* G, double* Wt, long long sO, int nslots, double* ldet);
void bin_blocks_launch(const double* W, long long sW, double* G, double* Wt, long long sO, int T, int p, double eps, const int* slots, int nslots, double* ldet,
                       hipStream_t st);
void thin_launch_ft(const pgpfa::ThinP& tp, int ntab, int ncols, bool vec_f32, hipStream_t st);
void thin_launch_s(const pgpfa::ThinP& ts, int ntab, int ncols, hipStream_t st);
void thin_launch_f(const pgpfa::ThinP& tp, int ntab, int ncols, bool vec_f32, hipStream_t st);
int estep_impl(pgpfa_ctx* c, const Trials& tr, int warm_start, bool allow_lr, double* obj_sum, int32_t* iters, int32_t* status,
               const LooJob* loo = nullptr, const VarJob* var = nullptr);
int ensure_mt_clean(pgpfa_ctx* c);
int ensure_vsmgp_buffer(pgpfa_ctx* c);
template <typename TB>
int assemble_rxr(pgpfa_ctx* c, const pgpfa::CholWS& view, int nb, const TB* F, const double* Wt, long long sW, const int* slots);
int posterior_blocks_lowrank(pgpfa_ctx* c, int nb, bool want_vsmgp, bool accumulate, double* logdet_out = nullptr, double* ld_dev = nullptr);
int posterior_blocks(pgpfa_ctx* c, int nb, double diag_scale, bool want_vsmgp, bool accumulate = false, double* ld_dev = nullptr);
int ensure_evidence_buffers(pgpfa_ctx* c);
int post_vsm_from_mt(pgpfa_ctx* c, int nslots);
int ensure_trial_vsmgp(pgpfa_ctx* c, const std::vector<int>& trials);
int posterior_factor_only(pgpfa_ctx* c, int nb, double diag_scale);
int resident_curvature(pgpfa_ctx* c, const std::vector<int>& tos, bool dual, const char* where, const std::function<int(double diag_scale)>& finish);
int ensure_lambda(pgpfa_ctx* c);
int dual_common(pgpfa_ctx* c, int nb, std::vector<double>* sB, std::vector<double>* sD, std::vector<double>* vKv);
int dual_jitter(pgpfa_ctx* c, int nb);
bool dual_masking(const pgpfa_ctx* c);
int dual_mask(pgpfa_ctx* c, int nb, double* buf);
int dual_dense_scale(pgpfa_ctx* c, int nb, double* scale);
int ensure_trunc_prior(pgpfa_ctx* c);
int dual_eval_slots(pgpfa_ctx* c, int nb, const std::vector<int>& tos, bool want_grad, double* cost, bool tolerate = false);
int var_offsets(pgpfa_ctx* c, int nb, double* out);
int check_distinct(const std::vector<int>& v);
int post_cov_dual_impl(pgpfa_ctx* c, int trial, double* out);
int allreduce_dev(pgpfa_ctx* c, double* buf, size_t count);
```

### poisson-gpfa_amd/csrc/gemm.h

```cpp
#pragma once
#include <hip/hip_runtime.h>
#include <type_traits>

#include "types.h"

namespace pgpfa {

template <int TRANSB, typename T, int BT, bool BF32 = false>
__global__ __launch_bounds__(256, BT == 128 ? 2 : 3) void gemm_mfma_kernel_t(GemmP g) {
  using T2 = typename GemmVec<T>::v2;
  using T4 = typename GemmVec<T>::v4;
  constexpr int LS = BT + 16;
  constexpr int WT = BT / 2;
  constexpr int MI = WT / 16;
  constexpr int NU = BT / 32;
  __shared__ __attribute__((aligned(16))) T As[2][GBK][LS];
  __shared__ __attribute__((aligned(16))) T Bs[2][GBK][LS];
  if (g.skip && *g.skip) return;

  const int tid = threadIdx.x;
  const int lane = tid & 63;
  const int wave = __builtin_amdgcn_readfirstlane(tid >> 6);
  const int wm = wave >> 1, wn = wave & 1;

  int b, tile;
  gemm_decode_block(g, blockIdx.x, b, tile);
  int ti, tj;
  gemm_decode_tile(g, tile, ti, tj);
  const T* A;
  const T* B;
  T* C;
  const int hi = gemm_bind_t<T>(g, b, A, B, C);
  const float* B32 = nullptr;
  if (BF32) {
    int lo2 = b, hi2 = 0;
    if (g.nb_lo > 0) { hi2 = b / g.nb_lo; lo2 = b - hi2 * g.nb_lo; }
    const long long slot2 = g.slots ? g.slots[lo2] : lo2;
    B32 = reinterpret_cast<const float*>(g.B) + slot2 * g.sB + hi2 * g.sB_hi;
  }

  int i0 = ti * BT, iend = g.M;
  const int j0 = tj * BT;
  if (g.n_dev) {
    g.N = *g.n_dev;
    if (j0 >= g.N) return;
  }
  int kb = 0, ke = g.K;
  if (g.kflags & KF_BEGIN_ROW) kb = i0;
  if (g.kflags & KF_BEGIN_MAXRC) kb = (i0 > j0 ? i0 : j0);
  if (g.kflags & KF_END_ROW) ke = (i0 + BT < g.K ? i0 + BT : g.K);
  if (g.rtab) { i0 = g.rtab[4 * ti]; iend = g.rtab[4 * ti + 1]; kb = g.rtab[4 * ti + 2]; ke = g.rtab[4 * ti + 3]; }
  if (kb > ke) kb = ke;
  gemm_split_range(g.ksplit, hi, kb, ke);

  const bool a_vec = ((((size_t)A) & (2 * sizeof(T) - 1)) == 0) && ((g.lda & 1) == 0) && ((i0 & 1) == 0);
  const bool b_vec = ((((size_t)B) & (2 * sizeof(T) - 1)) == 0) && ((g.ldb & 1) == 0);

  T raA[2 * NU], rbA[2 * NU], raB[2 * NU], rbB[2 * NU];
  int bcol[NU];
#pragma unroll
  for (int s = 0; s < NU; ++s) {
    const int jj = j0 + (tid + 256 * s) / 8;
    bcol[s] = (TRANSB && g.cols) ? g.cols[jj < g.N ? jj : g.N - 1] : jj;
  }
  auto bswz = [](int k) { return TRANSB ? (((k >> 1) & 7) << 3) : 0; };

  auto load_tiles = [&](auto vec, int k0, T (&ra)[2 * NU], T (&rb)[2 * NU]) {
    constexpr bool VEC = decltype(vec)::value;
#pragma unroll
    for (int s = 0; s < NU; ++s) {
      const int u = tid + 256 * s;
      {
        const int k = u / (BT / 2), r2 = (u % (BT / 2)) * 2;
        const T* src = A + gemm_koff(g.kseg, g.sAseg, g.lda, k0) + (size_t)k * g.lda + (i0 + r2);
        if constexpr (VEC) {
          const T2 v = *reinterpret_cast<const T2*>(src);
          ra[2 * s] = v.x; ra[2 * s + 1] = v.y;
        } else {
          ra[2 * s] = src[0]; ra[2 * s + 1] = src[1];
        }
      }
      if (TRANSB == 0 && BF32) {
        const int k = u / (BT / 2), r2 = (u % (BT / 2)) * 2;
        const float* src = B32 + gemm_koff(g.kseg, g.sBseg, g.ldb, k0) + (size_t)k * g.ldb + (j0 + r2);
        rb[2 * s] = (T)src[0]; rb[2 * s + 1] = (T)src[1];
      } else if (TRANSB == 0) {
        const int k = u / (BT / 2), r2 = (u % (BT / 2)) * 2;
        const T* src = B + gemm_koff(g.kseg, g.sBseg, g.ldb, k0) + (size_t)k * g.ldb + (j0 + r2);
        if constexpr (VEC) {
          const T2 v = *reinterpret_cast<const T2*>(src);
          rb[2 * s] = v.x; rb[2 * s + 1] = v.y;
        } else {
          rb[2 * s] = src[0]; rb[2 * s + 1] = src[1];
        }
      } else {
        const int k2 = (u % 8) * 2;
        const T* src = B + (size_t)bcol[s] * g.ldb + (k0 + k2);
        if constexpr (VEC) {
          const T2 v = *reinterpret_cast<const T2*>(src);
          rb[2 * s] = v.x; rb[2 * s + 1] = v.y;
        } else {
          rb[2 * s] = src[0]; rb[2 * s + 1] = src[1];
        }
      }
    }
  };
  auto store_tiles = [&](int buf, const T (&ra)[2 * NU], const T (&rb)[2 * NU]) {
#pragma unroll
    for (int s = 0; s < NU; ++s) {
      const int u = tid + 256 * s;
      {
        const int k = u / (BT / 2), r2 = (u % (BT / 2)) * 2;
        *reinterpret_cast<T2*>(&As[buf][k][r2]) = T2{ra[2 * s], ra[2 * s + 1]};
      }
      if (TRANSB == 0) {
        const int k = u / (BT / 2), r2 = (u % (BT / 2)) * 2;
        *reinterpret_cast<T2*>(&Bs[buf][k][r2]) = T2{rb[2 * s], rb[2 * s + 1]};
      } else {
        const int nn = (u / 8) ^ bswz(u % 8 * 2), k2 = (u % 8) * 2;
        Bs[buf][k2][nn] = rb[2 * s];
        Bs[buf][k2 + 1][nn] = rb[2 * s + 1];
      }
    }
  };

  T4 acc[MI][MI];
#pragma unroll
  for (int mi = 0; mi < MI; ++mi)
#pragma unroll
    for (int ni = 0; ni < MI; ++ni) acc[mi][ni] = T4{(T)0, (T)0, (T)0, (T)0};

  const bool wave_live = (i0 + wm * WT < iend) && (j0 + wn * WT < g.N) &&
                         !((g.mode == GEMM_LOWER) && (i0 + wm * WT + WT - 1 < j0 + wn * WT));

  const int nk = (ke - kb) / GBK;
  const int l15 = lane & 15, l4 = lane >> 4;
  auto multiply = [&](int buf) {
    if (!wave_live) return;
#pragma unroll
    for (int kk = 0; kk < GBK; kk += 4) {
      T af[MI], bf[MI];
#pragma unroll
      for (int mi = 0; mi < MI; ++mi) af[mi] = As[buf][kk + l4][wm * WT + mi * 16 + l15];
#pragma unroll
      for (int ni = 0; ni < MI; ++ni) bf[ni] = Bs[buf][kk + l4][(wn * WT + ni * 16 + l15) ^ bswz(kk + l4)];
#pragma unroll
      for (int mi = 0; mi < MI; ++mi)
#pragma unroll
        for (int ni = 0; ni < MI; ++ni)
          acc[mi][ni] = gemm_mfma16(bf[ni], af[mi], acc[mi][ni]);
    }
  };
  constexpr bool DEEP = (BT == 64) || (sizeof(T) == 4);
  auto run = [&](auto vec) {
    if constexpr (!DEEP) {
      if (nk > 0) {
        load_tiles(vec, kb, raA, rbA);
        store_tiles(0, raA, rbA);
      }
      __syncthreads();
      for (int it = 0; it < nk; ++it) {
        const int buf = it & 1;
        if (it + 1 < nk) load_tiles(vec, kb + (it + 1) * GBK, raA, rbA);
        multiply(buf);
        if (it + 1 < nk) store_tiles(buf ^ 1, raA, rbA);
        __syncthreads();
      }
      return;
    }
    if (nk > 0) {
      load_tiles(vec, kb, raA, rbA);
      if (nk > 1) load_tiles(vec, kb + GBK, raB, rbB);
      store_tiles(0, raA, rbA);
    }
    __syncthreads();
    int it = 0;
    for (; it + 3 < nk; it += 2) {
      load_tiles(vec, kb + (it + 2) * GBK, raA, rbA);
      multiply(0);
      store_tiles(1, raB, rbB);
      __syncthreads();
      load_tiles(vec, kb + (it + 3) * GBK, raB, rbB);
      multiply(1);
      store_tiles(0, raA, rbA);
      __syncthreads();
    }
    const int rem = nk - it;
    if (rem == 1) {
      multiply(0);
    } else if (rem == 2) {
      multiply(0);
      store_tiles(1, raB, rbB);
      __syncthreads();
      multiply(1);
    } else if (rem == 3) {
      load_tiles(vec, kb + (it + 2) * GBK, raA, rbA);
      multiply(0);
      store_tiles(1, raB, rbB);
      __syncthreads();
      multiply(1);
      store_tiles(0, raA, rbA);
      __syncthreads();
      multiply(0);
    }
  };
  if (a_vec && b_vec) run(std::true_type{}); else run(std::false_type{});

  if (!wave_live) return;
  const bool mask_diag = (g.kflags & KF_MASK_DIAG) && (ti == tj);
#pragma unroll
  for (int mi = 0; mi < MI; ++mi) {
    const int i = i0 + wm * WT + mi * 16 + l15;
    if (i >= iend) continue;
#pragma unroll
    for (int ni = 0; ni < MI; ++ni) {
#pragma unroll
      for (int r = 0; r < 4; ++r) {
        const int j = j0 + wn * WT + ni * 16 + (sizeof(T) == 8 ? l4 + 4 * r : 4 * l4 + r);
        if (j >= g.N) continue;
        if (mask_diag && i < j) continue;
        T* dst = C + (size_t)((TRANSB && g.cols && !g.cols_c_off) ? g.cols[j] : j) * g.ldc + i;
        T v = (T)g.alpha * acc[mi][ni][r];
        if (g.beta != 0.0) v += (T)g.beta * (*dst);
        *dst = v;
      }
    }
  }
}

template <int TRANSB>
__global__ void gemm_check_kernel(GemmP g) {
  if (g.skip && *g.skip) return;
  int b, tile;
  gemm_decode_block(g, blockIdx.x, b, tile);
  int ti, tj;
  gemm_decode_tile(g, tile, ti, tj);
  const double* A;
  const double* B;
  double* C;
  const int hi = gemm_bind(g, b, A, B, C);
  const int BT = g.bm;
  int i0 = ti * BT, iend = g.M;
  const int j0 = tj * BT;
  if (g.n_dev) {
    g.N = *g.n_dev;
    if (j0 >= g.N) return;
  }
  int kb = 0, ke = g.K;
  if (g.kflags & KF_BEGIN_ROW) kb = i0;
  if (g.kflags & KF_BEGIN_MAXRC) kb = (i0 > j0 ? i0 : j0);
  if (g.kflags & KF_END_ROW) ke = (i0 + BT < g.K ? i0 + BT : g.K);
  if (g.rtab) { i0 = g.rtab[4 * ti]; iend = g.rtab[4 * ti + 1]; kb = g.rtab[4 * ti + 2]; ke = g.rtab[4 * ti + 3]; }
  if (kb > ke) kb = ke;
  gemm_split_range(g.ksplit, hi, kb, ke);
  const bool mask_diag = (g.kflags & KF_MASK_DIAG) && (ti == tj);
  double vals[GBM * GBN / 256];
  int cnt = 0;
  for (int e = threadIdx.x; e < BT * BT; e += 256, ++cnt) {
    const int i = i0 + (e % BT), j = j0 + (e / BT);
    double s = 0.0;
    if (i < iend && j < g.N) {
      for (int k = kb; k < ke; ++k) {
        const double a = A[gemm_koff(g.kseg, g.sAseg, g.lda, k) + i];
        const double bb = TRANSB ? B[(size_t)(g.cols ? g.cols[j] : j) * g.ldb + k] : B[gemm_koff(g.kseg, g.sBseg, g.ldb, k) + j];
        s += a * bb;
      }
    }
    vals[cnt] = s;
  }
  __syncthreads();
  cnt = 0;
  const int WT = BT / 2;
  for (int e = threadIdx.x; e < BT * BT; e += 256, ++cnt) {
    const int i = i0 + (e % BT), j = j0 + (e / BT);
    if (i >= iend || j >= g.N) continue;
    if (mask_diag && i < j) continue;
    if (g.mode == GEMM_LOWER && ((i - i0) / WT) * WT + i0 + WT - 1 < ((j - j0) / WT) * WT + j0) continue;
    double* dst = C + (size_t)((TRANSB && g.cols && !g.cols_c_off) ? g.cols[j] : j) * g.ldc + i;
    double v = g.alpha * vals[cnt];
    if (g.beta != 0.0) v += g.beta * (*dst);
    *dst = v;
  }
}

inline __global__ void gemm_splitk_reduce_kernel(const double* __restrict__ part, int ksplit, int M, int N, int nbatch, double* __restrict__ C,
                                          long long sC, int ldc, const int* __restrict__ slots, double beta, const int* __restrict__ skip,
                                          const int* __restrict__ cols, const int* __restrict__ n_dev) {
  if (skip && *skip) return;
  const size_t e = (size_t)blockIdx.x * blockDim.x + threadIdx.x;
  if (e >= (size_t)M * N) return;
  if (n_dev && e / M >= (size_t)*n_dev) return;
  const int b = blockIdx.y;
  const long long slot = slots ? slots[b] : b;
  const size_t i = e % M, j = e / M;
  double s = 0.0;
  for (int k = 0; k < ksplit; ++k) s += part[((size_t)k * nbatch + b) * M * N + e];
  double* dst = C + slot * sC + (cols ? (size_t)cols[j] : j) * ldc + i;
  *dst = (beta != 0.0) ? beta * (*dst) + s : s;
}

inline __global__ __launch_bounds__(256) void mfma_peak_kernel(double* out, int iters) {
  double4_t acc[8];
#pragma unroll
  for (int i = 0; i < 8; ++i) acc[i] = (double4_t){0.0, 0.0, 0.0, 0.0};
  double a = 1.0 + threadIdx.x * 1e-6, b = 1.0 - threadIdx.x * 1e-6;
  for (int it = 0; it < iters; ++it) {
#pragma unroll
    for (int i = 0; i < 8; ++i) acc[i] = __builtin_amdgcn_mfma_f64_16x16x4f64(a, b, acc[i], 0, 0, 0);
  }
  double s = 0.0;
#pragma unroll
  for (int i = 0; i < 8; ++i) s += acc[i][0] + acc[i][1] + acc[i][2] + acc[i][3];
  out[blockIdx.x * blockDim.x + threadIdx.x] = s;
}

inline int gemm_count_tiles(int mode, int tilesM, int tilesN) {
  if (mode == GEMM_FULL) return tilesM * tilesN;
  int n = 0;
  for (int tj = 0; tj < tilesN && tj < tilesM; ++tj) n += tilesM - tj;
  return n;
}

hipError_t gemm_launch(hipStream_t st, bool use_mfma, bool transb, GemmP g, bool f32) {
  if (g.bm != 64) g.bm = 128;
  g.tilesM = g.rtab ? g.ntab : (g.M + g.bm - 1) / g.bm;
  g.tilesN = (g.N + g.bm - 1) / g.bm;
  g.ntiles = gemm_count_tiles(g.mode, g.tilesM, g.tilesN);
  if (g.ntiles <= 0 || g.nbatch <= 0 || g.M <= 0 || g.N <= 0) return hipSuccess;
  if (g.kseg != 0 && (transb || g.kseg % GBK != 0)) return hipErrorInvalidValue;
  if (g.rtab && g.mode != GEMM_FULL) return hipErrorInvalidValue;
  if (g.cols && !transb) return hipErrorInvalidValue;
  const long long blocks = (long long)g.ntiles * g.nbatch;
  dim3 grid((unsigned)blocks);
  if (f32) {
    if (g.kseg != 0) return hipErrorInvalidValue;
    if (g.bm == 64) {
      if (transb) hipLaunchKernelGGL((gemm_mfma_kernel_t<1, float, 64>), grid, dim3(256), 0, st, g);
      else hipLaunchKernelGGL((gemm_mfma_kernel_t<0, float, 64>), grid, dim3(256), 0, st, g);
    } else {
      if (transb) hipLaunchKernelGGL((gemm_mfma_kernel_t<1, float, 128>), grid, dim3(256), 0, st, g);
      else hipLaunchKernelGGL((gemm_mfma_kernel_t<0, float, 128>), grid, dim3(256), 0, st, g);
    }
  } else if (use_mfma) {
    if (g.b_f32) {
      if (transb || g.bm != 64) return hipErrorInvalidValue;
      hipLaunchKernelGGL((gemm_mfma_kernel_t<0, double, 64, true>), grid, dim3(256), 0, st, g);
    } else if (g.bm == 64) {
      if (transb) hipLaunchKernelGGL((gemm_mfma_kernel_t<1, double, 64>), grid, dim3(256), 0, st, g);
      else hipLaunchKernelGGL((gemm_mfma_kernel_t<0, double, 64>), grid, dim3(256), 0, st, g);
    } else {
      if (transb) hipLaunchKernelGGL((gemm_mfma_kernel_t<1, double, 128>), grid, dim3(256), 0, st, g);
      else hipLaunchKernelGGL((gemm_mfma_kernel_t<0, double, 128>), grid, dim3(256), 0, st, g);
    }
  } else {
    if (g.b_f32) return hipErrorInvalidValue;
    if (transb) hipLaunchKernelGGL(gemm_check_kernel<1>, grid, dim3(256), 0, st, g);
    else hipLaunchKernelGGL(gemm_check_kernel<0>, grid, dim3(256), 0, st, g);
  }
  return hipGetLastError();
}

}
```

### poisson-gpfa_amd/csrc/linalg.hip

```cpp
#include "ctx.h"
#include "model.h"
#include "gemm.h"
#include "chol.h"

using namespace pgpfa;

double gemm_flops(const GemmP& g) {
  if (g.flops_hint > 0.0) return g.flops_hint;
  const double M = g.M, N = g.N, K = g.K;
  double per;
  if (g.mode == GEMM_LOWER) {
    const double elems = N * (M - N) + N * (N + 1) / 2.0;
    per = 2.0 * K * elems;
  } else if (g.kflags & KF_BEGIN_ROW) {
    per = 2.0 * N * (M * K - M * (M - 1) / 2.0);
  } else if (g.kflags & KF_BEGIN_MAXRC) {
    per = 0.0;
    const double m = std::min(M, N);
    per = 2.0 * (M * N * K - (m * (m - 1) * (m + 1) / 3.0 + (M > N ? N * (M - N) * (M + N - 1) / 2.0 : M * (N - M) * (M + N - 1) / 2.0)));
  } else {
    per = 2.0 * M * N * K;
  }
  return per * g.nbatch;
}

int gemm(pgpfa_ctx* c, bool transb, GemmP g, bool f32) {
  const bool live_cols = g.cols && c->cur_ndev;
  prof_begin(c, TAG_GEMM, live_cols ? 0.0 : gemm_flops(g));
  if (c->prof.on && c->prof.open) {
    char key[176];
    std::snprintf(key, sizeof key, "%s %s M=%d N=%s%d K=%d%s batch=%d%s%s%s", f32 ? "f32" : "f64", transb ? "NN" : "NT", g.M, live_cols ? "<=" : "", g.N,
                  g.K, g.kseg ? " (segmented)" : "", std::max(g.nbatch, 1), g.mode == GEMM_LOWER ? " lower" : "",
                  g.kflags ? " triangular-k" : "", g.rtab ? " block-sparse" : "");
    c->prof.recs.back().shape = key;
    if (live_cols && c->live_gemm_collect) c->live_gemms.emplace_back(key, gemm_flops(g) / std::max(g.N, 1));
  }
  if (g.bm == 0) {
    const long long t128 = (long long)((g.M + GBM - 1) / GBM) * ((g.N + GBN - 1) / GBN) * std::max(g.nbatch, 1);
    g.bm = ((!f32 || c->f32_tile64) && c->mfma && (g.rtab || t128 < c->small_tile_below)) ? 64 : 128;
  }
  if (g.rtab) g.bm = 64;
  if (g.cols && c->cur_ndev) g.n_dev = c->cur_ndev;
  if ((const double*)g.C == g.A || (const double*)g.C == g.B) g.bm = 128;
  const int tiles = (g.rtab ? g.ntab : (g.M + g.bm - 1) / g.bm) * ((g.N + g.bm - 1) / g.bm) * std::max(g.nbatch, 1);
  int ksplit = 1;
  const double k_eff = g.k_loop_hint > 0 ? (double)g.k_loop_hint
                       : (g.flops_hint > 0.0 && g.M > 0 && g.N > 0) ? g.flops_hint / (2.0 * g.M * g.N * std::max(g.nbatch, 1)) : (double)g.K;
  const int split_below = g.bm == 64 ? c->splitk_below64 : 384;
  if (!f32 && c->gemm_part && !c->no_splitk && g.mode == GEMM_FULL && g.kflags == 0 && g.nb_lo == 0 && g.kseg == 0 && tiles > 0 && tiles < split_below && k_eff >= 128.0) {
    ksplit = std::min(std::min(8, (int)(k_eff / (tiles < 64 ? 32.0 : 64.0))), (c->splitk_target + tiles - 1) / tiles);
    while (ksplit > 1 && (size_t)ksplit * g.nbatch * g.M * g.N > c->gemm_part_len) --ksplit;
  }
  hipError_t e;
  if (ksplit > 1) {
    GemmP s = g;
    s.C = c->gemm_part; s.sC = (long long)g.M * g.N; s.ldc = g.M; s.beta = 0.0;
    s.nb_lo = g.nbatch; s.nbatch = g.nbatch * ksplit; s.sA_hi = 0; s.sB_hi = 0; s.sC_hi = (long long)g.nbatch * g.M * g.N;
    s.ksplit = ksplit;
    s.c_by_pos = 1;
    s.cols_c_off = 1;
    e = gemm_launch(c->st, c->mfma, transb, s);
    if (e == hipSuccess) {
      hipLaunchKernelGGL(gemm_splitk_reduce_kernel, dim3((unsigned)(((size_t)g.M * g.N + 255) / 256), g.nbatch), dim3(256), 0, c->st, c->gemm_part,
                         ksplit, g.M, g.N, g.nbatch, g.C, g.sC, g.ldc, g.slots, g.beta, g.skip, g.cols, g.n_dev);
      e = hipGetLastError();
    }
  } else {
    e = gemm_launch(c->st, c->mfma, transb, g, f32);
  }
  prof_end(c);
  if (e != hipSuccess) return fail("gemm launch failed: %s", hipGetErrorString(e));
  return 0;
}

int factor(pgpfa_ctx* c, const CholWS& w, const int* slots, int nb, bool f32, bool wide_diag) {
  auto at = [f32](double* base, size_t off) { return f32 ? reinterpret_cast<double*>(reinterpret_cast<float*>(base) + off) : base + off; };
  const int np = w.npad, ld = w.ld;
  const int na = (w.nact > 0 && w.nact <= np) ? w.nact : np;
  for (int c0 = 0; c0 < np; c0 += NSUP) {
    const int c1 = std::min(c0 + NSUP, np);
    for (int k0 = c0; k0 < c1; k0 += NB) {
      prof_begin(c, TAG_POTRF, 2.0 * nb * (double)NB * NB * NB / 3.0);
      if (f32 && wide_diag)
        hipLaunchKernelGGL((potrf_diag_kernel_t<double, 3, 2, float>), dim3(nb), dim3(512), 0, c->st, reinterpret_cast<float*>(w.H), w.sH, ld, k0,
                           reinterpret_cast<float*>(w.Dinv), w.sD, slots, w.info);
      else if (f32)
        hipLaunchKernelGGL(potrf_diag_kernel_t<float>, dim3(nb), dim3(512), 0, c->st, reinterpret_cast<float*>(w.H), w.sH, ld, k0,
                           reinterpret_cast<float*>(w.Dinv), w.sD, slots, w.info);
      else
        hipLaunchKernelGGL(potrf_diag_kernel_t<double>, dim3(nb), dim3(512), 0, c->st, w.H, w.sH, ld, k0, w.Dinv, w.sD, slots, w.info);
      prof_end(c);
      const int r0 = k0 + NB;
      if (r0 >= np) break;
      GemmP g{};
      g.A = at(w.H, (size_t)k0 * ld + r0); g.sA = w.sH; g.lda = ld;
      g.B = at(w.Dinv, (size_t)(k0 / NB) * NB * NB); g.sB = w.sD; g.ldb = NB;
      g.C = at(w.H, (size_t)k0 * ld + r0); g.sC = w.sH; g.ldc = ld;
      g.M = na - r0; g.N = NB; g.K = NB; g.alpha = 1.0; g.beta = 0.0;
      g.slots = slots; g.nbatch = nb; g.mode = GEMM_FULL; g.kflags = 0;
      if (g.M > 0) CHK(gemm(c, false, g, f32));
      if (r0 < c1 && r0 < na) {
        GemmP s{};
        s.A = at(w.H, (size_t)k0 * ld + r0); s.sA = w.sH; s.lda = ld;
        s.B = s.A; s.sB = w.sH; s.ldb = ld;
        s.C = at(w.H, (size_t)r0 * ld + r0); s.sC = w.sH; s.ldc = ld;
        s.M = na - r0; s.N = std::min(c1, na) - r0; s.K = NB; s.alpha = -1.0; s.beta = 1.0;
        s.slots = slots; s.nbatch = nb; s.mode = GEMM_LOWER; s.kflags = KF_MASK_DIAG;
        CHK(gemm(c, false, s, f32));
      }
    }
    if (c1 < na) {
      GemmP s{};
      s.A = at(w.H, (size_t)c0 * ld + c1); s.sA = w.sH; s.lda = ld;
      s.B = s.A; s.sB = w.sH; s.ldb = ld;
      s.C = at(w.H, (size_t)c1 * ld + c1); s.sC = w.sH; s.ldc = ld;
      s.M = na - c1; s.N = na - c1; s.K = c1 - c0; s.alpha = -1.0; s.beta = 1.0;
      s.slots = slots; s.nbatch = nb; s.mode = GEMM_LOWER; s.kflags = KF_MASK_DIAG;
      CHK(gemm(c, false, s, f32));
    }
  }
  HIPC(hipGetLastError());
  return 0;
}

int inverse_t(pgpfa_ctx* c, const CholWS& w, const int* slots, int nb, bool f32) {
  auto at = [f32](double* base, size_t off) { return f32 ? reinterpret_cast<double*>(reinterpret_cast<float*>(base) + off) : base + off; };
  const int np = w.npad, ld = w.ld;
  const int na = (w.nact > 0 && w.nact <= np) ? w.nact : np;
  if (f32)
    hipLaunchKernelGGL(diag_transpose_kernel_t<float>, dim3(nb, np / NB), dim3(256), 0, c->st, reinterpret_cast<float*>(w.Mt), w.sM, ld, 0,
                       reinterpret_cast<const float*>(w.Dinv), w.sD, slots);
  else
    hipLaunchKernelGGL(diag_transpose_kernel_t<double>, dim3(nb, np / NB), dim3(256), 0, c->st, w.Mt, w.sM, ld, 0, w.Dinv, w.sD, slots);
  for (int j0 = NB; j0 < np; j0 += NB) {
    const int nbw = std::min(NB, na - j0);
    if (nbw <= 0) continue;
    GemmP a{};
    a.A = w.Mt; a.sA = w.sM; a.lda = ld;
    a.B = at(w.H, j0); a.sB = w.sH; a.ldb = ld;
    a.C = w.P; a.sC = w.sP; a.ldc = np;
    a.M = std::min(j0, na); a.N = nbw; a.K = j0; a.alpha = 1.0; a.beta = 0.0;
    a.slots = slots; a.nbatch = nb; a.mode = GEMM_FULL; a.kflags = KF_BEGIN_ROW;
    CHK(gemm(c, false, a, f32));
    GemmP b{};
    b.A = w.P; b.sA = w.sP; b.lda = np;
    b.B = at(w.Dinv, (size_t)(j0 / NB) * NB * NB); b.sB = w.sD; b.ldb = NB;
    b.C = at(w.Mt, (size_t)j0 * ld); b.sC = w.sM; b.ldc = ld;
    b.M = std::min(j0, na); b.N = nbw; b.K = nbw; b.alpha = -1.0; b.beta = 0.0;
    b.slots = slots; b.nbatch = nb; b.mode = GEMM_FULL; b.kflags = 0;
    CHK(gemm(c, false, b, f32));
  }
  HIPC(hipGetLastError());
  return 0;
}
// ... 245 lines not shown
```

### poisson-gpfa_amd/csrc/split.h

```cpp
#pragma once
#include <type_traits>
#include <hip/hip_runtime.h>

namespace pgpfa {

typedef _Float16 half8_t __attribute__((ext_vector_type(8)));
typedef float float4v_t __attribute__((ext_vector_type(4)));

constexpr float SPLIT_SCALE = 2048.0f;


template <int PW>
__global__ __launch_bounds__(256, 2) void mix_vsm_split_kernel(const double* __restrict__ Yt, long long sY, int ldy, float* __restrict__ D, long long sD,
                                                            int ldd, const double* __restrict__ G, long long sG, int T, int p, int rpad, double eps,
                                                            double* __restrict__ vsm, const int* __restrict__ slots,
                                                            const int* __restrict__ trial_of_slot, const int* __restrict__ roff, int col_tile, int ts) {
  constexpr int PP = PW * PW, LD = PP + 1, NPAIR = PW * (PW + 1) / 2;
  __shared__ double Gs[64 * LD];
  const int pp = p * p;
  const int slot = slots[blockIdx.y];
  const int t0 = blockIdx.x * 64;
  const int nt = min(64, T - t0);
  const double* gbase = G + (size_t)slot * sG + (size_t)t0 * pp;
  if (p < PW)
// ... 714 lines not shown
  auto load = [&](int, double (&ra)[NA], TB (&rb)[4]) {
    const int c0 = cur_c * GK;
    const double* Ap = a.A + (size_t)cur_s * a.sM + (size_t)c0 * a.lda + a.row0;
    const TB* Dp = Dall + (size_t)cur_s * a.sD + (size_t)c0 * a.ldd + t0;
#pragma unroll
    for (int u = 0; u < NA; ++u) ra[u] = Ap[aoff[u]];
#pragma unroll
    for (int u = 0; u < 4; ++u) rb[u] = Dp[doff[u]];
    if (cur_c + 1 < cps) ++cur_c;
    else if (cur_s + 1 < s_end) { ++cur_s; cur_c = 0; }
  };
  auto store = [&](int buf, const double (&ra)[NA], const TB (&rb)[4]) {
#pragma unroll
    for (int u = 0; u < NA; ++u) {
      const int e = tid + 256 * u;
      const int kk = e / (NTR * 16), i = e - kk * (NTR * 16);
      if (kk < GK) As[buf][kk][i] = (i < rk) ? ra[u] : 0.0;
    }
#pragma unroll
    for (int u = 0; u < 4; ++u) {
      const int e = tid + 256 * u;
      Bs[buf][e >> 6][e & 63] = (t0 + (e & 63) < a.T) ? (double)rb[u] : 0.0;
    }
  };
  mdouble4 acc[NTR];
#pragma unroll
  for (int mi = 0; mi < NTR; ++mi) acc[mi] = mdouble4{0.0, 0.0, 0.0, 0.0};
  auto multiply = [&](int buf) {
    if (!wave_live) return;
#pragma unroll
    for (int kk = 0; kk < GK; kk += 4) {
      const double bf = Bs[buf][kk + l4][wave * 16 + l15];
#pragma unroll
      for (int mi = 0; mi < NTR; ++mi)
        if (!LOWER || mi >= ct) acc[mi] = __builtin_amdgcn_mfma_f64_16x16x4f64(bf, As[buf][kk + l4][mi * 16 + l15], acc[mi], 0, 0, 0);
    }
  };
  if (nchunks > 0) {
    load(0, raA, rbA);
    load(1, raB, rbB);
    store(0, raA, rbA);
  }
  __syncthreads();
  for (int ch = 0; ch < nchunks; ch += 2) {
    load(ch + 2, raA, rbA);
    multiply(0);
    if (ch + 1 < nchunks) store(1, raB, rbB);
    __syncthreads();
    if (ch + 1 >= nchunks) break;
    load(ch + 3, raB, rbB);
    multiply(1);
    if (ch + 2 < nchunks) store(0, raA, rbA);
    __syncthreads();
  }
  if (!wave_live) return;
  double* C = a.C + (size_t)g * a.sC + a.row0;
#pragma unroll
  for (int mi = 0; mi < NTR; ++mi) {
    const int i = mi * 16 + l15;
    if (i >= rk || (LOWER && mi < ct)) continue;
#pragma unroll
    for (int r = 0; r < 4; ++r) {
      const int t = t0 + wave * 16 + l4 + 4 * r;
      if (t < a.T) C[(size_t)t * a.ldc + i] = acc[mi][r];
    }
  }
}

template <typename TB, bool LOWER>
inline void cross_term_launch(const CrossArgs& ca, dim3 grid, hipStream_t st) {
  switch (ca.rk / 16) {
    case 1: hipLaunchKernelGGL((cross_term_kernel<1, TB, LOWER>), grid, dim3(256), 0, st, ca); break;
    case 2: hipLaunchKernelGGL((cross_term_kernel<2, TB, LOWER>), grid, dim3(256), 0, st, ca); break;
    case 3: hipLaunchKernelGGL((cross_term_kernel<3, TB, LOWER>), grid, dim3(256), 0, st, ca); break;
    case 4: hipLaunchKernelGGL((cross_term_kernel<4, TB, LOWER>), grid, dim3(256), 0, st, ca); break;
    case 5: hipLaunchKernelGGL((cross_term_kernel<5, TB, LOWER>), grid, dim3(256), 0, st, ca); break;
    case 6: hipLaunchKernelGGL((cross_term_kernel<6, TB, LOWER>), grid, dim3(256), 0, st, ca); break;
    case 7: hipLaunchKernelGGL((cross_term_kernel<7, TB, LOWER>), grid, dim3(256), 0, st, ca); break;
    default: hipLaunchKernelGGL((cross_term_kernel<8, TB, LOWER>), grid, dim3(256), 0, st, ca); break;
  }
}

inline __global__ __launch_bounds__(256) void sum_groups_kernel(const double* __restrict__ part, int ngroups, int M, int N, int lower, double* __restrict__ out) {
  __shared__ double red[4][64];
  const int el = threadIdx.x & 63, q = threadIdx.x >> 6;
  const size_t e = (size_t)blockIdx.x * 64 + el;
  const bool in = e < (size_t)M * N;
  const size_t ec = in ? e : 0;
  const int i = (int)(ec % M), j = (int)(ec / M);
  const size_t src = (lower > 0 && (i / lower) < (j / lower)) ? (size_t)i * M + j : ec;
  const size_t gs = (size_t)M * N;
  double s8[8] = {0.0, 0.0, 0.0, 0.0, 0.0, 0.0, 0.0, 0.0};
  int g = q;
  for (; g + 28 < ngroups; g += 32) {
    double v[8];
#pragma unroll
    for (int u = 0; u < 8; ++u) v[u] = part[(size_t)(g + 4 * u) * gs + src];
#pragma unroll
    for (int u = 0; u < 8; ++u) s8[u] += v[u];
  }
  for (; g < ngroups; g += 4) s8[0] += part[(size_t)g * gs + src];
  red[q][el] = ((s8[0] + s8[1]) + (s8[2] + s8[3])) + ((s8[4] + s8[5]) + (s8[6] + s8[7]));
  __syncthreads();
  if (q == 0 && in) out[e] = (red[0][el] + red[1][el]) + (red[2][el] + red[3][el]);
}

constexpr int PACC_TS = 32;
inline __global__ __launch_bounds__(256) void pacc_split_reduce_kernel(const double* __restrict__ T1, const double* __restrict__ X, const double* __restrict__ DD, int ngroups,
                                                                const double* __restrict__ G, long long sG, int nslots, double eps, int T, int Tp, int p,
                                                                double* __restrict__ Pacc) {
  constexpr int TS = PACC_TS;
  __shared__ double Xa[TS][TS + 1], Xb[TS][TS + 1], Ss[TS][TS + 1];
  __shared__ double gd[TS];
  const int k = blockIdx.y;
  int tj = 0, rem = blockIdx.x;
  const int ntile = (T + TS - 1) / TS;
  while (rem >= ntile - tj) { rem -= ntile - tj; ++tj; }
  const int ti = tj + rem;
  const int i0 = ti * TS, j0 = tj * TS;
  const size_t tt = (size_t)T * T;
  const double* t1 = T1 + (size_t)k * tt;
  const double* x = X + (size_t)k * tt;
  const double* dd = DD + (size_t)k * ngroups * tt;
  double* out = Pacc + (size_t)k * Tp * Tp;
  const int tid = threadIdx.x;
  for (int e = tid; e < TS * TS; e += 256) {
    const int r = e % TS, cc = e / TS;
    Xa[cc][r] = (i0 + r < T && j0 + cc < T) ? x[(size_t)(j0 + cc) * T + i0 + r] : 0.0;
    Xb[cc][r] = (j0 + r < T && i0 + cc < T) ? x[(size_t)(i0 + cc) * T + j0 + r] : 0.0;
    double sum = 0.0;
    if (i0 + r < T && j0 + cc < T) {
      const size_t e2 = (size_t)(j0 + cc) * T + i0 + r;
      for (int g2 = 0; g2 < ngroups; ++g2) sum += dd[(size_t)g2 * tt + e2];
    }
    Ss[cc][r] = sum;
  }
  if (ti == tj) {
    constexpr int PER = 256 / TS;
    const int t = tid / PER, part = tid % PER;
    double gs = 0.0;
    if (i0 + t < T)
      for (int sl = part; sl < nslots; sl += PER) gs += G[(size_t)sl * sG + (size_t)(i0 + t) * p * p + (size_t)k * p + k];
#pragma unroll
    for (int o = 1; o < PER; o <<= 1) gs += __shfl_xor(gs, o);
    if (part == 0) gd[t] = eps * gs;
  }
  __syncthreads();
  for (int e = tid; e < TS * TS; e += 256) {
    const int r = e % TS, cc = e / TS;
    const int i = i0 + r, j = j0 + cc;
    if (i < T && j < T) {
      double v = t1[(size_t)j * T + i] - Xa[cc][r] - Xb[r][cc] + Ss[cc][r];
      if (ti == tj && r == cc) v += gd[r];
      out[(size_t)j * Tp + i] += v;
    }
  }
  if (ti != tj) {
    for (int e = tid; e < TS * TS; e += 256) {
      const int r = e % TS, cc = e / TS;
      const int i = j0 + r, j = i0 + cc;
      if (i < T && j < T) out[(size_t)j * Tp + i] += t1[(size_t)j * T + i] - Xb[cc][r] - Xa[r][cc] + Ss[r][cc];
    }
  }
}

}
```

### poisson-gpfa_amd/csrc/types.h

```cpp
#pragma once
#include <hip/hip_runtime.h>
#include <type_traits>

namespace pgpfa {

typedef double double4_t __attribute__((ext_vector_type(4)));

enum : int {
  GEMM_FULL = 0,
  GEMM_LOWER = 1,
};
enum : int {
  KF_BEGIN_ROW = 1,
  KF_END_ROW = 2,
  KF_MASK_DIAG = 4,
  KF_BEGIN_MAXRC = 8,
};

struct GemmP {
  const double* A; long long sA; int lda;
  const double* B; long long sB; int ldb;
  double* C; long long sC; int ldc;
  int M, N, K;
  double alpha, beta;
  const int* slots;
  const int* rtab; int ntab;
  int bm;
  int nbatch;
  int mode, kflags;
  int tilesM, tilesN, ntiles;
  double flops_hint;
  int k_loop_hint;
  int nb_lo;
  long long sA_hi, sB_hi, sC_hi;
  int kseg;
  long long sAseg, sBseg;
  int ksplit;
  int c_by_pos;
  const int* skip;
  const int* cols;
  int cols_c_off;
  const int* n_dev;
  int b_f32;
};

__device__ __forceinline__ size_t gemm_koff(int kseg, long long sseg, int ld, int k) {
  if (kseg == 0) return (size_t)k * ld;
  const int seg = k / kseg;
  return (size_t)seg * sseg + (size_t)(k - seg * kseg) * ld;
}

__device__ __forceinline__ int gemm_bind(const GemmP& g, int b, const double*& A, const double*& B, double*& C) {
  int lo = b, hi = 0;
  if (g.nb_lo > 0) { hi = b / g.nb_lo; lo = b - hi * g.nb_lo; }
  const long long slot = g.slots ? g.slots[lo] : lo;
  A = g.A + slot * g.sA + hi * g.sA_hi;
  B = g.B + slot * g.sB + hi * g.sB_hi;
  C = g.C + (g.c_by_pos ? (long long)lo : slot) * g.sC + hi * g.sC_hi;
  return hi;
}

__device__ __forceinline__ void gemm_split_range(int ksplit, int part, int& kb, int& ke) {
  if (ksplit <= 1) return;
  const int len = ke - kb;
  const int chunk = ((len + ksplit - 1) / ksplit + 15) / 16 * 16;
  const int b0 = kb + part * chunk;
  ke = (b0 + chunk < ke) ? b0 + chunk : ke;
  kb = (b0 < ke) ? b0 : ke;
}

__device__ __forceinline__ void gemm_decode_tile(const GemmP& g, int tile, int& ti, int& tj) {
  if (g.mode == GEMM_FULL) {
    ti = tile % g.tilesM;
    tj = tile / g.tilesM;
  } else {
    int tjj = 0, rem = tile;
    while (rem >= g.tilesM - tjj) { rem -= g.tilesM - tjj; ++tjj; }
    tj = tjj;
    ti = tjj + rem;
  }
}

__device__ __forceinline__ void gemm_decode_block(const GemmP& g, int bid, int& b, int& tile) {
  const int full = g.nbatch >> 3;
  const int per_group = g.ntiles << 3;
  const int grp = bid / per_group;
  if (grp < full) {
    const int r = bid - grp * per_group;
    tile = r >> 3;
    b = (grp << 3) + (r & 7);
  } else {
    const int m = g.nbatch - (full << 3);
    const int r = bid - full * per_group;
    tile = r / m;
    b = (full << 3) + (r - tile * m);
  }
}

constexpr int GBM = 128, GBN = 128, GBK = 16;

typedef float float2_t __attribute__((ext_vector_type(2)));
typedef float float4_t __attribute__((ext_vector_type(4)));
typedef double double2_t __attribute__((ext_vector_type(2)));
template <typename T> struct GemmVec;
template <> struct GemmVec<double> { using v2 = double2_t; using v4 = double4_t; };
template <> struct GemmVec<float> { using v2 = float2_t; using v4 = float4_t; };
__device__ __forceinline__ double4_t gemm_mfma16(double a, double b, double4_t c) { return __builtin_amdgcn_mfma_f64_16x16x4f64(a, b, c, 0, 0, 0); }
__device__ __forceinline__ float4_t gemm_mfma16(float a, float b, float4_t c) { return __builtin_amdgcn_mfma_f32_16x16x4f32(a, b, c, 0, 0, 0); }

template <typename T>
__device__ __forceinline__ int gemm_bind_t(const GemmP& g, int b, const T*& A, const T*& B, T*& C) {
  int lo = b, hi = 0;
  if (g.nb_lo > 0) { hi = b / g.nb_lo; lo = b - hi * g.nb_lo; }
  const long long slot = g.slots ? g.slots[lo] : lo;
  A = reinterpret_cast<const T*>(g.A) + slot * g.sA + hi * g.sA_hi;
  B = reinterpret_cast<const T*>(g.B) + slot * g.sB + hi * g.sB_hi;
  C = reinterpret_cast<T*>(g.C) + (g.c_by_pos ? (long long)lo : slot) * g.sC + hi * g.sC_hi;
  return hi;
}

constexpr int NB = 128;
constexpr int NSUP = 512;

struct CholWS {
  double* H; long long sH;
  double* Mt; long long sM;
  double* Dinv; long long sD;
  double* P; long long sP;
  int* info;
  int ld, npad;
  int nact = 0;
};

struct PcgCtl {
  int stop; int iters; unsigned worst_bits; int nlive; unsigned long long slot_iters;
  int nl[2];
  int pad_[2];
};

hipError_t gemm_launch(hipStream_t st, bool use_mfma, bool transb, GemmP g, bool f32 = false);

}
```

Measured before the change: 12.40.

## Group per-latent split-covariance tail GEMMs and group sums into table-driven launches

Result: no change. 12.42 (median of 2 runs) (+0.1%).

```diff
diff --git a/poisson-gpfa_amd/csrc/core.hip b/poisson-gpfa_amd/csrc/core.hip
--- a/poisson-gpfa_amd/csrc/core.hip
+++ b/poisson-gpfa_amd/csrc/core.hip
@@ -253,6 +253,19 @@
   return 0;
 }
 
+int table_sync(pgpfa_ctx* c, DevTable& t, const void* image, size_t bytes, size_t cap) {
+  if (bytes > cap) return fail("internal: a device table of %zu bytes exceeds its %zu", bytes, cap);
+  if (!t.dev) {
+    if (hipMalloc(&t.dev, cap) != hipSuccess) { (void)hipGetLastError(); t.dev = nullptr; return fail("out of device memory for a launch table (%zu bytes)", cap); }
+    t.cap = cap;
+    t.host.clear();
+    c->bytes += cap;
+  }
+  if (t.host.size() == bytes && std::memcmp(t.host.data(), image, bytes) == 0) return 0;
+  CHK(upload_nosync(c, t.dev, image, bytes));
+  t.host.assign(static_cast<const char*>(image), static_cast<const char*>(image) + bytes);
+  return 0;
+}
 
 int build_kinv(pgpfa_ctx* c) {
   c->kinv_serial += 1;
@@ -423,6 +436,12 @@
   c->info["lowrank_rtot"] = c->rtot;
   c->info["lowrank_rtot16"] = c->rtot16;
   c->info["lowrank_compact"] = c->rank_compact ? 1.0 : 0.0;
+  {
+    int lo = c->rk.empty() ? 0 : c->rk[0], hi = 0;
+    for (int k = 0; k < p; ++k) { lo = std::min(lo, c->rk[k]); hi = std::max(hi, c->rk[k]); }
+    c->info["lowrank_rk_min"] = lo;
+    c->info["lowrank_rk_max"] = hi;
+  }
   c->flr32_valid = false;
   return 0;
 }
@@ -792,6 +811,7 @@
   c->info["last_syrk_tile"] = 0.0;
   c->info["last_split_sps"] = 0.0;
   c->info["last_cross_kernel"] = 0.0;
+  c->info["last_split_tail_grouped"] = 0.0;
   c->info["last_mix_form"] = 0.0;
   c->info["last_yt_mix_fused"] = 0.0;
   c->info["last_cov_f32"] = 0.0;
@@ -814,6 +834,7 @@
   if (c->Flr32) hipFree(c->Flr32);
   if (c->lam_keep) hipFree(c->lam_keep);
   if (c->split_buf) hipFree(c->split_buf);
+  for (DevTable& t : c->tail_tab) if (t.dev) hipFree(t.dev);
   if (c->Yhi) hipFree(c->Yhi);
   free_tables(c->live);
   if (c->trunc_q) hipFree(c->trunc_q);
@@ -855,6 +876,7 @@
   else if (k == "cd_mfma") c->cd_mfma = (v != 0.0);
   else if (k == "cd_hess_mfma") c->cd_hess_mfma = (v != 0.0);
   else if (k == "cross_kernel") c->cross_kernel = (v != 0.0);
+  else if (k == "split_tail_grouped") c->split_tail_grouped = (v != 0.0);
   else if (k == "cd_debug") c->cd_debug = (int)v;
   else if (k == "pcg_fused") c->pcg_fused = (int)v;
   else if (k == "pcg_w32") c->pcg_w32 = (v != 0.0);
diff --git a/poisson-gpfa_amd/csrc/cov.hip b/poisson-gpfa_amd/csrc/cov.hip
--- a/poisson-gpfa_amd/csrc/cov.hip
+++ b/poisson-gpfa_amd/csrc/cov.hip
@@ -1,6 +1,7 @@
 #include "query.h"
 #include "model.h"
 #include "split.h"
+#include "split_plan.h"
 #include "ytmix.h"
 #include "hook.h"
 
@@ -154,35 +155,40 @@
   return 0;
 }
 
-static int split_latent_sums(pgpfa_ctx* c, const double* A0, long long sM, int lda, const float* Dk, long long sD, int ldd, int rk, int kw, int T, int nb, int sps,
-                             bool cross, double* Spart, double* Xpart, double* Ssum, double* Xsum, int* cross_used) {
+static GemmP split_seg_problem(const double* A0, long long sM, int lda, const float* Dk, long long sD, int ldd, int rk, int kw, int T, int first, int per, int ng,
+                               int group0, bool is_x, double* out) {
+  GemmP g{};
+  g.A = A0 + (size_t)first * sM; g.sA = (long long)per * sM; g.lda = lda;
+  g.kseg = kw; g.sAseg = sM;
+  g.K = per * kw; g.alpha = 1.0; g.beta = 0.0; g.slots = nullptr; g.nbatch = ng; g.kflags = 0; g.bm = 64;
+  g.M = rk;
+  if (is_x) {
+    g.B = reinterpret_cast<const double*>(Dk + (size_t)first * sD);
+    g.sB = (long long)per * sD; g.ldb = ldd; g.sBseg = sD; g.b_f32 = 1;
+    g.N = T; g.mode = GEMM_FULL;
+    g.C = out + (size_t)group0 * rk * T; g.sC = (long long)rk * T; g.ldc = rk;
+  } else {
+    g.B = g.A; g.sB = g.sA; g.ldb = lda; g.sBseg = sM;
+    g.N = rk; g.mode = GEMM_LOWER;
+    g.C = out + (size_t)group0 * rk * rk; g.sC = (long long)rk * rk; g.ldc = rk;
+  }
+  return g;
+}
+
+static int split_seg(pgpfa_ctx* c, const double* A0, long long sM, int lda, const float* Dk, long long sD, int ldd, int rk, int kw, int T, int nb, int sper, bool is_x,
+                     double* out) {
+  const int nfull = nb / sper, rem = nb - nfull * sper;
+  for (int part = 0; part < 2; ++part) {
+    const int first = part ? nfull * sper : 0, per = part ? rem : sper, ng = part ? (rem ? 1 : 0) : nfull;
+    if (ng == 0 || per == 0) continue;
+    CHK(gemm(c, false, split_seg_problem(A0, sM, lda, Dk, sD, ldd, rk, kw, T, first, per, ng, part ? nfull : 0, is_x, out)));
+  }
+  return 0;
+}
+
+static int split_x_parts(pgpfa_ctx* c, const double* A0, long long sM, int lda, const float* Dk, long long sD, int ldd, int rk, int kw, int T, int nb, int sps,
+                         bool cross, double* Xpart, int* cross_used) {
   const int ngroups = (nb + sps - 1) / sps;
-  const int spsS = std::max(1, (nb + SPLIT_NS - 1) / SPLIT_NS);
-  auto seg = [&](int sper, bool is_x, double* out) -> int {
-    const int nfull = nb / sper, rem = nb - nfull * sper;
-    for (int part = 0; part < 2; ++part) {
-      const int first = part ? nfull * sper : 0, per = part ? rem : sper, ng = part ? (rem ? 1 : 0) : nfull;
-      if (ng == 0 || per == 0) continue;
-      GemmP g{};
-      g.A = A0 + (size_t)first * sM; g.sA = (long long)per * sM; g.lda = lda;
-      g.kseg = kw; g.sAseg = sM;
-      g.K = per * kw; g.alpha = 1.0; g.beta = 0.0; g.slots = nullptr; g.nbatch = ng; g.kflags = 0; g.bm = 64;
-      g.M = rk;
-      if (is_x) {
-        g.B = reinterpret_cast<const double*>(Dk + (size_t)first * sD);
-        g.sB = (long long)per * sD; g.ldb = ldd; g.sBseg = sD; g.b_f32 = 1;
-        g.N = T; g.mode = GEMM_FULL;
-        g.C = out + (size_t)(part ? nfull : 0) * rk * T; g.sC = (long long)rk * T; g.ldc = rk;
-      } else {
-        g.B = g.A; g.sB = g.sA; g.ldb = lda; g.sBseg = sM;
-        g.N = rk; g.mode = GEMM_LOWER;
-        g.C = out + (size_t)(part ? nfull : 0) * rk * rk; g.sC = (long long)rk * rk; g.ldc = rk;
-      }
-      CHK(gemm(c, false, g));
-    }
-    return 0;
-  };
-  CHK(seg(spsS, false, Spart));
   const bool use_cross = cross && c->mfma && rk % 16 == 0 && kw % 16 == 0;
   if (use_cross) {
     for (int row0 = 0; row0 < rk; row0 += 128) {
@@ -198,12 +204,21 @@
     }
     HIPC(hipGetLastError());
   } else {
-    CHK(seg(sps, true, Xpart));
-  }
+    CHK(split_seg(c, A0, sM, lda, Dk, sD, ldd, rk, kw, T, nb, sps, true, Xpart));
+  }
+  *cross_used = use_cross ? 1 : 0;
+  return 0;
+}
+
+static int split_latent_sums(pgpfa_ctx* c, const double* A0, long long sM, int lda, const float* Dk, long long sD, int ldd, int rk, int kw, int T, int nb, int sps,
+                             bool cross, double* Spart, double* Xpart, double* Ssum, double* Xsum, int* cross_used) {
+  const int ngroups = (nb + sps - 1) / sps;
+  const int spsS = std::max(1, (nb + SPLIT_NS - 1) / SPLIT_NS);
+  CHK(split_seg(c, A0, sM, lda, Dk, sD, ldd, rk, kw, T, nb, spsS, false, Spart));
+  CHK(split_x_parts(c, A0, sM, lda, Dk, sD, ldd, rk, kw, T, nb, sps, cross, Xpart, cross_used));
   const int ngS = (nb + spsS - 1) / spsS;
   hipLaunchKernelGGL(sum_groups_kernel, dim3((unsigned)(((size_t)rk * rk + 63) / 64)), dim3(256), 0, c->st, Spart, ngS, rk, rk, 32, Ssum);
   hipLaunchKernelGGL(sum_groups_kernel, dim3((unsigned)(((size_t)rk * T + 63) / 64)), dim3(256), 0, c->st, Xpart, ngroups, rk, T, 0, Xsum);
-  *cross_used = use_cross ? 1 : 0;
   return 0;
 }
 
@@ -287,21 +302,36 @@
 
 struct SplitScratch {
   double *Spart, *Xpart, *Ssum, *Xsum, *Zb, *T1, *Xfull;
+  double* pack;
   float* D;
   long long sD;
   int ldd;
 };
 
-int split_scratch(pgpfa_ctx* c, const CholWS& lw, SplitScratch* s) {
+int split_scratch(pgpfa_ctx* c, const CholWS& lw, SplitScratch* s, size_t packed = 0) {
   const int T = c->T, p = c->p;
   const size_t tt = (size_t)T * T;
   constexpr int NS = SPLIT_NS, NG = PACC_SPLITS + 1;
   const size_t tq = (size_t)round_up(T, 16) * round_up(T, 16);
-  if (!c->split_buf) {
-    const size_t len = ((size_t)NS + NG + 3) * tq + 2 * (size_t)p * tt + 1024;
-    if (hipMalloc((void**)&c->split_buf, len * sizeof(double)) != hipSuccess) { (void)hipGetLastError(); c->split_buf = nullptr; return fail("out of device memory for the split accumulation (%zu bytes)", len * sizeof(double)); }
+  const size_t base = ((size_t)NS + NG + 3) * tq + 2 * (size_t)p * tt + 1024;
+  auto alloc = [&](size_t len) -> bool {
+    if (c->split_buf) {
+      if (hipStreamSynchronize(c->st) != hipSuccess) return false;
+      hipFree(c->split_buf);
+      c->bytes -= c->split_buf_len * sizeof(double);
+      c->split_buf = nullptr; c->split_buf_len = 0;
+      for (DevTable& t : c->tail_tab) t.host.clear();
+    }
+    if (hipMalloc((void**)&c->split_buf, len * sizeof(double)) != hipSuccess) { (void)hipGetLastError(); c->split_buf = nullptr; return false; }
+    c->split_buf_len = len;
     c->bytes += len * sizeof(double);
-  }
+    return true;
+  };
+  if (!c->split_buf || c->split_buf_len < base + packed) {
+    const size_t roomy = std::max(packed, std::min(2 * packed, split_plan::PACKED_BUDGET_BYTES / sizeof(double)));
+    if (!alloc(base + roomy) && (packed == 0 || !alloc(base))) return fail("out of device memory for the split accumulation (%zu bytes)", base * sizeof(double));
+  }
+  s->pack = (packed > 0 && c->split_buf_len >= base + packed) ? c->split_buf + base : nullptr;
   s->Spart = c->split_buf;
   s->Xpart = s->Spart + (size_t)NS * tq;
   s->Ssum = s->Xpart + (size_t)NG * tq;
@@ -428,17 +458,98 @@
   return 0;
 }
 
+static std::vector<split_plan::Latent> tail_latents(const pgpfa_ctx* c, int ract) {
+  std::vector<split_plan::Latent> lat((size_t)c->p);
+  for (int k = 0; k < c->p; ++k) lat[k] = {c->rk[k], ract - (c->roff[k] & ~15)};
+  return lat;
+}
+
+int split_latent_terms_grouped(pgpfa_ctx* c, const CovPass& P, const SplitScratch& s, int sps, const split_plan::Plan& plan, bool* cross_ran_out) {
+  const int T = c->T, p = c->p, Tp = c->Tp, rpad = c->rpad, nb = P.nb, ract = P.ract, Ts = P.Ts, ldd = s.ldd;
+  const size_t tt = (size_t)T * T;
+  const long long sD = s.sD, sM = (long long)P.lw.sM;
+  double* pack = s.pack;
+  auto A0 = [&](int k) { return P.lw.Mt + c->roff[k] + (size_t)(c->roff[k] & ~15) * rpad; };
+  for (int k = 0; k < p; ++k)
+    if (!plan.reg[k].live) {
+      HIPC(hipMemsetAsync(s.T1 + (size_t)k * tt, 0, tt * sizeof(double), c->st));
+      HIPC(hipMemsetAsync(s.Xfull + (size_t)k * tt, 0, tt * sizeof(double), c->st));
+    }
+  std::vector<GemmP> probs;
+  for (const split_plan::SProb& sp : plan.sprobs)
+    probs.push_back(split_seg_problem(A0(sp.latent), sM, rpad, nullptr, 0, 0, sp.M, sp.kseg, T, sp.first, sp.per, sp.ng, sp.group0, false, pack + plan.reg[sp.latent].Spart));
+  CHK(gemm_grouped(c, false, probs, c->tail_tab[pgpfa_ctx::TAB_S], c->tail_tab[pgpfa_ctx::TAB_NT_RED], plan.sblk0.back()));
+  bool cross_ran = false;
+  std::vector<SumGroupsTab> sums(2);
+  int nblk[2] = {0, 0};
+  for (int k = 0; k < p; ++k) {
+    const split_plan::Region& r = plan.reg[k];
+    if (!r.live) continue;
+    const int rk = c->rk[k], r0 = c->roff[k] & ~15, kw = ract - r0;
+    int cross_used = 0;
+    CHK(split_x_parts(c, A0(k), sM, rpad, s.D + (size_t)k * Ts + (size_t)r0 * ldd, sD, ldd, rk, kw, T, nb, sps, c->cross_kernel, pack + r.Xpart, &cross_used));
+    cross_ran = cross_ran || cross_used != 0;
+    const SumGroupsEntry es{pack + r.Spart, pack + r.Ssum, plan.ngS, rk, rk, 32}, ex{pack + r.Xpart, pack + r.Xsum, plan.ngroups, rk, T, 0};
+    const SumGroupsEntry* e2[2] = {&es, &ex};
+    for (int w = 0; w < 2; ++w) {
+      SumGroupsTab& t = sums[w];
+      t.ent[t.nent] = *e2[w];
+      t.blk0[t.nent] = nblk[w];
+      nblk[w] += (int)(((size_t)e2[w]->M * e2[w]->N + 63) / 64);
+      t.blk0[++t.nent] = nblk[w];
+    }
+  }
+  for (int w = 0; w < 2; ++w) {
+    if (sums[w].nent == 0) continue;
+    DevTable& dt = c->tail_tab[w ? pgpfa_ctx::TAB_SUM_X : pgpfa_ctx::TAB_SUM_S];
+    CHK(table_sync(c, dt, &sums[w], offsetof(SumGroupsTab, ent) + (size_t)sums[w].nent * sizeof(SumGroupsEntry), sizeof(SumGroupsTab)));
+    hipLaunchKernelGGL(sum_groups_table_kernel, dim3((unsigned)nblk[w]), dim3(256), 0, c->st, static_cast<const SumGroupsTab*>(dt.dev));
+  }
+  HIPC(hipGetLastError());
+  std::vector<GemmP> nn, nt;
+  for (int k = 0; k < p; ++k) {
+    const split_plan::Region& r = plan.reg[k];
+    if (!r.live) continue;
+    const int rk = c->rk[k];
+    const double* Fk = c->Flr + (size_t)k * Tp * Tp;
+    GemmP z{};
+    z.A = Fk; z.lda = Tp; z.B = pack + r.Ssum; z.ldb = rk; z.C = pack + r.Zb; z.ldc = T;
+    z.M = T; z.N = rk; z.K = rk; z.alpha = 1.0; z.beta = 0.0; z.nbatch = 1; z.mode = GEMM_FULL;
+    nn.push_back(z);
+    GemmP xf = z;
+    xf.B = pack + r.Xsum; xf.ldb = rk; xf.C = s.Xfull + (size_t)k * tt; xf.ldc = T; xf.N = T;
+    nn.push_back(xf);
+    GemmP t1 = z;
+    t1.A = pack + r.Zb; t1.lda = T; t1.B = Fk; t1.ldb = Tp; t1.C = s.T1 + (size_t)k * tt; t1.ldc = T; t1.N = T;
+    nt.push_back(t1);
+  }
+  CHK(gemm_grouped(c, true, nn, c->tail_tab[pgpfa_ctx::TAB_NN], c->tail_tab[pgpfa_ctx::TAB_NN_RED]));
+  CHK(gemm_grouped(c, false, nt, c->tail_tab[pgpfa_ctx::TAB_NT], c->tail_tab[pgpfa_ctx::TAB_NT_RED]));
+  *cross_ran_out = cross_ran;
+  return 0;
+}
+
 int accumulate_split(pgpfa_ctx* c, const CovPass& P, bool fused) {
   const int T = c->T, p = c->p;
   SplitScratch s{};
-  CHK(split_scratch(c, P.lw, &s));
+  const int sps_plan = std::max(1, (P.nb + PACC_SPLITS - 1) / PACC_SPLITS);
+  split_plan::Plan plan{};
+  bool grouped = c->split_tail_grouped && c->mfma && p <= SUM_GROUPS_MAX;
+  if (grouped) {
+    plan = split_plan::plan_tail(tail_latents(c, P.ract), T, P.nb, sps_plan);
+    grouped = plan.total > 0 && plan.total * sizeof(double) <= split_plan::PACKED_BUDGET_BYTES && plan.sprobs.size() <= (size_t)GEMM_GROUP_MAX;
+  }
+  CHK(split_scratch(c, P.lw, &s, grouped ? plan.total : 0));
   c->info["last_mix_form"] = (double)mix_split(c, P, s, fused);
   int sps = 0, ngroups = 0, tile_used = 0;
   CHK(split_syrk_launch(c, s.D, s.sD, s.ldd, P.Ts, T, p, P.ract, P.nb, 0, c->syrk_tile, c->ppart, &tile_used, &sps, &ngroups));
   c->info["last_syrk_tile"] = (double)tile_used;
   c->info["last_split_sps"] = (double)sps;
   bool cross_ran = false;
-  CHK(split_latent_terms(c, P, s, sps, &cross_ran));
+  grouped = grouped && s.pack && sps == sps_plan;
+  if (grouped) CHK(split_latent_terms_grouped(c, P, s, sps, plan, &cross_ran));
+  else CHK(split_latent_terms(c, P, s, sps, &cross_ran));
+  c->info["last_split_tail_grouped"] = grouped ? 1.0 : 0.0;
   c->info["last_cross_kernel"] = cross_ran ? 1.0 : 0.0;
   const int nt64 = (T + PACC_TS - 1) / PACC_TS;
   hipLaunchKernelGGL(pacc_split_reduce_kernel, dim3(nt64 * (nt64 + 1) / 2, p), dim3(256), 0, c->st, s.T1, s.Xfull, c->ppart, ngroups, c->Gbin, P.sW, P.nb, c->eps, T, c->Tp,
@@ -692,7 +803,7 @@
   if (!fused) CHK(yt_product<double>(c, P, c->Flr, P.lw.Mt, P.lw.sM, P.lw.H, P.lw.sH));
   if (!fuse_candidate) CHK(split_verdict(c, P, &split));
   c->info["last_split_cov"] = split ? 1.0 : 0.0;
-  if (!split) for (const char* key : {"last_syrk_tile", "last_split_sps", "last_cross_kernel", "last_mix_form"}) c->info[key] = 0.0;
+  if (!split) for (const char* key : {"last_syrk_tile", "last_split_sps", "last_cross_kernel", "last_split_tail_grouped", "last_mix_form"}) c->info[key] = 0.0;
   if (!want_vsmgp) CHK(vsm_from_yt<double>(c, P, P.lw.H, P.lw.sH));
   else if (split) CHK(accumulate_split(c, P, fused));
   else {
diff --git a/poisson-gpfa_amd/csrc/ctx.h b/poisson-gpfa_amd/csrc/ctx.h
--- a/poisson-gpfa_amd/csrc/ctx.h
+++ b/poisson-gpfa_amd/csrc/ctx.h
@@ -64,6 +64,11 @@
   std::map<int, double> max_ms, max_flops;
   struct Shape { double ms = 0.0, flops = 0.0, count = 0.0; };
   std::map<std::string, Shape> shapes;
+};
+struct DevTable {
+  void* dev = nullptr;
+  size_t cap = 0;
+  std::vector<char> host;
 };
 constexpr int TAU_MULTI_MAX = 4;
 constexpr int PACC_SPLITS = 64;
@@ -110,6 +115,10 @@
   int qpad = 0, ccu_cols = 0;
   double* ppart = nullptr;
   double* split_buf = nullptr;
+  size_t split_buf_len = 0;
+  bool split_tail_grouped = true;
+  enum { TAB_S = 0, TAB_SUM_S, TAB_SUM_X, TAB_NN, TAB_NN_RED, TAB_NT, TAB_NT_RED, TAB_N };
+  DevTable tail_tab[TAB_N];
   bool split_cov = true;
   double split_max_norm = 0.07;
   double *cdym = nullptr, *cdym_part = nullptr;
@@ -429,6 +438,8 @@
 int get_slabs(pgpfa_ctx* c, const double* src, double* out);
 double gemm_flops(const pgpfa::GemmP& g);
 int gemm(pgpfa_ctx* c, bool transb, pgpfa::GemmP g, bool f32 = false);
+int gemm_grouped(pgpfa_ctx* c, bool transb, const std::vector<pgpfa::GemmP>& probs, DevTable& tab, DevTable& red, int expect_blocks = -1);
+int table_sync(pgpfa_ctx* c, DevTable& t, const void* image, size_t bytes, size_t cap);
 int factor(pgpfa_ctx* c, const pgpfa::CholWS& w, const int* slots, int nb, bool f32 = false, bool wide_diag = false);
 int inverse_t(pgpfa_ctx* c, const pgpfa::CholWS& w, const int* slots, int nb, bool f32 = false);
 int poisson(pgpfa_ctx* c, const int* d_list, int nl, const double* X, double* G, double* W, double* flik, int full);
diff --git a/poisson-gpfa_amd/csrc/gemm.h b/poisson-gpfa_amd/csrc/gemm.h
--- a/poisson-gpfa_amd/csrc/gemm.h
+++ b/poisson-gpfa_amd/csrc/gemm.h
@@ -8,224 +8,21 @@
 
 template <int TRANSB, typename T, int BT, bool BF32 = false>
 __global__ __launch_bounds__(256, BT == 128 ? 2 : 3) void gemm_mfma_kernel_t(GemmP g) {
-  using T2 = typename GemmVec<T>::v2;
-  using T4 = typename GemmVec<T>::v4;
-  constexpr int LS = BT + 16;
-  constexpr int WT = BT / 2;
-  constexpr int MI = WT / 16;
-  constexpr int NU = BT / 32;
-  __shared__ __attribute__((aligned(16))) T As[2][GBK][LS];
-  __shared__ __attribute__((aligned(16))) T Bs[2][GBK][LS];
-  if (g.skip && *g.skip) return;
+#define GEMM_TILE_BID blockIdx.x
+#include "gemm_tile.inc"
+#undef GEMM_TILE_BID
+}
 
-  const int tid = threadIdx.x;
-  const int lane = tid & 63;
-  const int wave = __builtin_amdgcn_readfirstlane(tid >> 6);
-  const int wm = wave >> 1, wn = wave & 1;
-
-  int b, tile;
-  gemm_decode_block(g, blockIdx.x, b, tile);
-  int ti, tj;
-  gemm_decode_tile(g, tile, ti, tj);
-  const T* A;
-  const T* B;
-  T* C;
-  const int hi = gemm_bind_t<T>(g, b, A, B, C);
-  const float* B32 = nullptr;
-  if (BF32) {
-    int lo2 = b, hi2 = 0;
-    if (g.nb_lo > 0) { hi2 = b / g.nb_lo; lo2 = b - hi2 * g.nb_lo; }
-    const long long slot2 = g.slots ? g.slots[lo2] : lo2;
-    B32 = reinterpret_cast<const float*>(g.B) + slot2 * g.sB + hi2 * g.sB_hi;
-  }
-
-  int i0 = ti * BT, iend = g.M;
-  const int j0 = tj * BT;
-  if (g.n_dev) {
-    g.N = *g.n_dev;
-    if (j0 >= g.N) return;
-  }
-  int kb = 0, ke = g.K;
-  if (g.kflags & KF_BEGIN_ROW) kb = i0;
-  if (g.kflags & KF_BEGIN_MAXRC) kb = (i0 > j0 ? i0 : j0);
-  if (g.kflags & KF_END_ROW) ke = (i0 + BT < g.K ? i0 + BT : g.K);
-  if (g.rtab) { i0 = g.rtab[4 * ti]; iend = g.rtab[4 * ti + 1]; kb = g.rtab[4 * ti + 2]; ke = g.rtab[4 * ti + 3]; }
-  if (kb > ke) kb = ke;
-  gemm_split_range(g.ksplit, hi, kb, ke);
-
-  const bool a_vec = ((((size_t)A) & (2 * sizeof(T) - 1)) == 0) && ((g.lda & 1) == 0) && ((i0 & 1) == 0);
-  const bool b_vec = ((((size_t)B) & (2 * sizeof(T) - 1)) == 0) && ((g.ldb & 1) == 0);
-
-  T raA[2 * NU], rbA[2 * NU], raB[2 * NU], rbB[2 * NU];
-  int bcol[NU];
-#pragma unroll
-  for (int s = 0; s < NU; ++s) {
-    const int jj = j0 + (tid + 256 * s) / 8;
-    bcol[s] = (TRANSB && g.cols) ? g.cols[jj < g.N ? jj : g.N - 1] : jj;
-  }
-  auto bswz = [](int k) { return TRANSB ? (((k >> 1) & 7) << 3) : 0; };
-
-  auto load_tiles = [&](auto vec, int k0, T (&ra)[2 * NU], T (&rb)[2 * NU]) {
-    constexpr bool VEC = decltype(vec)::value;
-#pragma unroll
-    for (int s = 0; s < NU; ++s) {
-      const int u = tid + 256 * s;
-      {
-        const int k = u / (BT / 2), r2 = (u % (BT / 2)) * 2;
-        const T* src = A + gemm_koff(g.kseg, g.sAseg, g.lda, k0) + (size_t)k * g.lda + (i0 + r2);
-        if constexpr (VEC) {
-          const T2 v = *reinterpret_cast<const T2*>(src);
-          ra[2 * s] = v.x; ra[2 * s + 1] = v.y;
-        } else {
-          ra[2 * s] = src[0]; ra[2 * s + 1] = src[1];
-        }
-      }
-      if (TRANSB == 0 && BF32) {
-        const int k = u / (BT / 2), r2 = (u % (BT / 2)) * 2;
-        const float* src = B32 + gemm_koff(g.kseg, g.sBseg, g.ldb, k0) + (size_t)k * g.ldb + (j0 + r2);
-        rb[2 * s] = (T)src[0]; rb[2 * s + 1] = (T)src[1];
-      } else if (TRANSB == 0) {
-        const int k = u / (BT / 2), r2 = (u % (BT / 2)) * 2;
-        const T* src = B + gemm_koff(g.kseg, g.sBseg, g.ldb, k0) + (size_t)k * g.ldb + (j0 + r2);
-        if constexpr (VEC) {
-          const T2 v = *reinterpret_cast<const T2*>(src);
-          rb[2 * s] = v.x; rb[2 * s + 1] = v.y;
-        } else {
-          rb[2 * s] = src[0]; rb[2 * s + 1] = src[1];
-        }
-      } else {
-        const int k2 = (u % 8) * 2;
-        const T* src = B + (size_t)bcol[s] * g.ldb + (k0 + k2);
-        if constexpr (VEC) {
-          const T2 v = *reinterpret_cast<const T2*>(src);
-          rb[2 * s] = v.x; rb[2 * s + 1] = v.y;
-        } else {
-          rb[2 * s] = src[0]; rb[2 * s + 1] = src[1];
-        }
-      }
-    }
-  };
-  auto store_tiles = [&](int buf, const T (&ra)[2 * NU], const T (&rb)[2 * NU]) {
-#pragma unroll
-    for (int s = 0; s < NU; ++s) {
-      const int u = tid + 256 * s;
-      {
-        const int k = u / (BT / 2), r2 = (u % (BT / 2)) * 2;
-        *reinterpret_cast<T2*>(&As[buf][k][r2]) = T2{ra[2 * s], ra[2 * s + 1]};
-      }
-      if (TRANSB == 0) {
-        const int k = u / (BT / 2), r2 = (u % (BT / 2)) * 2;
-        *reinterpret_cast<T2*>(&Bs[buf][k][r2]) = T2{rb[2 * s], rb[2 * s + 1]};
-      } else {
-        const int nn = (u / 8) ^ bswz(u % 8 * 2), k2 = (u % 8) * 2;
-        Bs[buf][k2][nn] = rb[2 * s];
-        Bs[buf][k2 + 1][nn] = rb[2 * s + 1];
-      }
-    }
-  };
-
-  T4 acc[MI][MI];
-#pragma unroll
-  for (int mi = 0; mi < MI; ++mi)
-#pragma unroll
-    for (int ni = 0; ni < MI; ++ni) acc[mi][ni] = T4{(T)0, (T)0, (T)0, (T)0};
-
-  const bool wave_live = (i0 + wm * WT < iend) && (j0 + wn * WT < g.N) &&
-                         !((g.mode == GEMM_LOWER) && (i0 + wm * WT + WT - 1 < j0 + wn * WT));
-
-  const int nk = (ke - kb) / GBK;
-  const int l15 = lane & 15, l4 = lane >> 4;
-  auto multiply = [&](int buf) {
-    if (!wave_live) return;
-#pragma unroll
-    for (int kk = 0; kk < GBK; kk += 4) {
-      T af[MI], bf[MI];
-#pragma unroll
-      for (int mi = 0; mi < MI; ++mi) af[mi] = As[buf][kk + l4][wm * WT + mi * 16 + l15];
-#pragma unroll
-      for (int ni = 0; ni < MI; ++ni) bf[ni] = Bs[buf][kk + l4][(wn * WT + ni * 16 + l15) ^ bswz(kk + l4)];
-#pragma unroll
-      for (int mi = 0; mi < MI; ++mi)
-#pragma unroll
-        for (int ni = 0; ni < MI; ++ni)
-          acc[mi][ni] = gemm_mfma16(bf[ni], af[mi], acc[mi][ni]);
-    }
-  };
-  constexpr bool DEEP = (BT == 64) || (sizeof(T) == 4);
-  auto run = [&](auto vec) {
-    if constexpr (!DEEP) {
-      if (nk > 0) {
-        load_tiles(vec, kb, raA, rbA);
-        store_tiles(0, raA, rbA);
-      }
-      __syncthreads();
-      for (int it = 0; it < nk; ++it) {
-        const int buf = it & 1;
-        if (it + 1 < nk) load_tiles(vec, kb + (it + 1) * GBK, raA, rbA);
-        multiply(buf);
-        if (it + 1 < nk) store_tiles(buf ^ 1, raA, rbA);
-        __syncthreads();
-      }
-      return;
-    }
-    if (nk > 0) {
-      load_tiles(vec, kb, raA, rbA);
-      if (nk > 1) load_tiles(vec, kb + GBK, raB, rbB);
-      store_tiles(0, raA, rbA);
-    }
-    __syncthreads();
-    int it = 0;
-    for (; it + 3 < nk; it += 2) {
-      load_tiles(vec, kb + (it + 2) * GBK, raA, rbA);
-      multiply(0);
-      store_tiles(1, raB, rbB);
-      __syncthreads();
-      load_tiles(vec, kb + (it + 3) * GBK, raB, rbB);
-      multiply(1);
-      store_tiles(0, raA, rbA);
-      __syncthreads();
-    }
-    const int rem = nk - it;
-    if (rem == 1) {
-      multiply(0);
-    } else if (rem == 2) {
-      multiply(0);
-      store_tiles(1, raB, rbB);
-      __syncthreads();
-      multiply(1);
-    } else if (rem == 3) {
-      load_tiles(vec, kb + (it + 2) * GBK, raA, rbA);
-      multiply(0);
-      store_tiles(1, raB, rbB);
-      __syncthreads();
-      multiply(1);
-      store_tiles(0, raA, rbA);
-      __syncthreads();
-      multiply(0);
-    }
-  };
-  if (a_vec && b_vec) run(std::true_type{}); else run(std::false_type{});
-
-  if (!wave_live) return;
-  const bool mask_diag = (g.kflags & KF_MASK_DIAG) && (ti == tj);
-#pragma unroll
-  for (int mi = 0; mi < MI; ++mi) {
-    const int i = i0 + wm * WT + mi * 16 + l15;
-    if (i >= iend) continue;
-#pragma unroll
-    for (int ni = 0; ni < MI; ++ni) {
-#pragma unroll
-      for (int r = 0; r < 4; ++r) {
-        const int j = j0 + wn * WT + ni * 16 + (sizeof(T) == 8 ? l4 + 4 * r : 4 * l4 + r);
-        if (j >= g.N) continue;
-        if (mask_diag && i < j) continue;
-        T* dst = C + (size_t)((TRANSB && g.cols && !g.cols_c_off) ? g.cols[j] : j) * g.ldc + i;
-        T v = (T)g.alpha * acc[mi][ni][r];
-        if (g.beta != 0.0) v += (T)g.beta * (*dst);
-        *dst = v;
-      }
-    }
-  }
+template <int TRANSB, typename T, int BT, bool BF32 = false>
+__global__ __launch_bounds__(256, BT == 128 ? 2 : 3) void gemm_grouped_kernel_t(const GemmGroupTab* __restrict__ tab) {
+  const int bid = blockIdx.x, n = tab->nprob;
+  int pr = 0;
+  while (pr + 1 < n && bid >= tab->blk0[pr + 1]) ++pr;
+  GemmP g = tab->prob[pr];
+  const int bid_in = bid - tab->blk0[pr];
+#define GEMM_TILE_BID bid_in
+#include "gemm_tile.inc"
+#undef GEMM_TILE_BID
 }
 
 template <int TRANSB>
@@ -299,6 +96,19 @@
   *dst = (beta != 0.0) ? beta * (*dst) + s : s;
 }
 
+inline __global__ void gemm_splitk_reduce_grouped_kernel(const GemmReduceTab* __restrict__ tab) {
+  const int bid = blockIdx.x, n = tab->nent;
+  int pr = 0;
+  while (pr + 1 < n && bid >= tab->blk0[pr + 1]) ++pr;
+  const GemmReduceEntry r = tab->ent[pr];
+  const size_t e = (size_t)(bid - tab->blk0[pr]) * blockDim.x + threadIdx.x;
+  if (e >= (size_t)r.M * r.N) return;
+  const size_t i = e % r.M, j = e / r.M;
+  double s = 0.0;
+  for (int k = 0; k < r.ksplit; ++k) s += r.part[(size_t)k * r.M * r.N + e];
+  r.C[j * r.ldc + i] = s;
+}
+
 inline __global__ __launch_bounds__(256) void mfma_peak_kernel(double* out, int iters) {
   double4_t acc[8];
 #pragma unroll
@@ -360,4 +170,17 @@
   return hipGetLastError();
 }
 
+hipError_t gemm_grouped_launch(hipStream_t st, bool transb, const GemmGroupTab* tab, int nblocks) {
+  if (nblocks <= 0) return hipSuccess;
+  if (transb) hipLaunchKernelGGL((gemm_grouped_kernel_t<1, double, 64>), dim3((unsigned)nblocks), dim3(256), 0, st, tab);
+  else hipLaunchKernelGGL((gemm_grouped_kernel_t<0, double, 64>), dim3((unsigned)nblocks), dim3(256), 0, st, tab);
+  return hipGetLastError();
 }
+
+hipError_t gemm_reduce_grouped_launch(hipStream_t st, const GemmReduceTab* tab, int nblocks) {
+  if (nblocks <= 0) return hipSuccess;
+  hipLaunchKernelGGL(gemm_splitk_reduce_grouped_kernel, dim3((unsigned)nblocks), dim3(256), 0, st, tab);
+  return hipGetLastError();
+}
+
+}
diff --git a/poisson-gpfa_amd/csrc/gemm_tile.inc b/poisson-gpfa_amd/csrc/gemm_tile.inc
--- /dev/null
+++ b/poisson-gpfa_amd/csrc/gemm_tile.inc
@@ -0,0 +1,218 @@
+  using T2 = typename GemmVec<T>::v2;
+  using T4 = typename GemmVec<T>::v4;
+  constexpr int LS = BT + 16;
+  constexpr int WT = BT / 2;
+  constexpr int MI = WT / 16;
+  constexpr int NU = BT / 32;
+  __shared__ __attribute__((aligned(16))) T As[2][GBK][LS];
+  __shared__ __attribute__((aligned(16))) T Bs[2][GBK][LS];
+  if (g.skip && *g.skip) return;
+
+  const int tid = threadIdx.x;
+  const int lane = tid & 63;
+  const int wave = __builtin_amdgcn_readfirstlane(tid >> 6);
+  const int wm = wave >> 1, wn = wave & 1;
+
+  int b, tile;
+  gemm_decode_block(g, GEMM_TILE_BID, b, tile);
+  int ti, tj;
+  gemm_decode_tile(g, tile, ti, tj);
+  const T* A;
+  const T* B;
+  T* C;
+  const int hi = gemm_bind_t<T>(g, b, A, B, C);
+  const float* B32 = nullptr;
+  if (BF32) {
+    int lo2 = b, hi2 = 0;
+    if (g.nb_lo > 0) { hi2 = b / g.nb_lo; lo2 = b - hi2 * g.nb_lo; }
+    const long long slot2 = g.slots ? g.slots[lo2] : lo2;
+    B32 = reinterpret_cast<const float*>(g.B) + slot2 * g.sB + hi2 * g.sB_hi;
+  }
+
+  int i0 = ti * BT, iend = g.M;
+  const int j0 = tj * BT;
+  if (g.n_dev) {
+    g.N = *g.n_dev;
+    if (j0 >= g.N) return;
+  }
+  int kb = 0, ke = g.K;
+  if (g.kflags & KF_BEGIN_ROW) kb = i0;
+  if (g.kflags & KF_BEGIN_MAXRC) kb = (i0 > j0 ? i0 : j0);
+  if (g.kflags & KF_END_ROW) ke = (i0 + BT < g.K ? i0 + BT : g.K);
+  if (g.rtab) { i0 = g.rtab[4 * ti]; iend = g.rtab[4 * ti + 1]; kb = g.rtab[4 * ti + 2]; ke = g.rtab[4 * ti + 3]; }
+  if (kb > ke) kb = ke;
+  gemm_split_range(g.ksplit, hi, kb, ke);
+
+  const bool a_vec = ((((size_t)A) & (2 * sizeof(T) - 1)) == 0) && ((g.lda & 1) == 0) && ((i0 & 1) == 0);
+  const bool b_vec = ((((size_t)B) & (2 * sizeof(T) - 1)) == 0) && ((g.ldb & 1) == 0);
+
+  T raA[2 * NU], rbA[2 * NU], raB[2 * NU], rbB[2 * NU];
+  int bcol[NU];
+#pragma unroll
+  for (int s = 0; s < NU; ++s) {
+    const int jj = j0 + (tid + 256 * s) / 8;
+    bcol[s] = (TRANSB && g.cols) ? g.cols[jj < g.N ? jj : g.N - 1] : jj;
+  }
+  auto bswz = [](int k) { return TRANSB ? (((k >> 1) & 7) << 3) : 0; };
+
+  auto load_tiles = [&](auto vec, int k0, T (&ra)[2 * NU], T (&rb)[2 * NU]) {
+    constexpr bool VEC = decltype(vec)::value;
+#pragma unroll
+    for (int s = 0; s < NU; ++s) {
+      const int u = tid + 256 * s;
+      {
+        const int k = u / (BT / 2), r2 = (u % (BT / 2)) * 2;
+        const T* src = A + gemm_koff(g.kseg, g.sAseg, g.lda, k0) + (size_t)k * g.lda + (i0 + r2);
+        if constexpr (VEC) {
+          const T2 v = *reinterpret_cast<const T2*>(src);
+          ra[2 * s] = v.x; ra[2 * s + 1] = v.y;
+        } else {
+          ra[2 * s] = src[0]; ra[2 * s + 1] = src[1];
+        }
+      }
+      if (TRANSB == 0 && BF32) {
+        const int k = u / (BT / 2), r2 = (u % (BT / 2)) * 2;
+        const float* src = B32 + gemm_koff(g.kseg, g.sBseg, g.ldb, k0) + (size_t)k * g.ldb + (j0 + r2);
+        rb[2 * s] = (T)src[0]; rb[2 * s + 1] = (T)src[1];
+      } else if (TRANSB == 0) {
+        const int k = u / (BT / 2), r2 = (u % (BT / 2)) * 2;
+        const T* src = B + gemm_koff(g.kseg, g.sBseg, g.ldb, k0) + (size_t)k * g.ldb + (j0 + r2);
+        if constexpr (VEC) {
+          const T2 v = *reinterpret_cast<const T2*>(src);
+          rb[2 * s] = v.x; rb[2 * s + 1] = v.y;
+        } else {
+          rb[2 * s] = src[0]; rb[2 * s + 1] = src[1];
+        }
+      } else {
+        const int k2 = (u % 8) * 2;
+        const T* src = B + (size_t)bcol[s] * g.ldb + (k0 + k2);
+        if constexpr (VEC) {
+          const T2 v = *reinterpret_cast<const T2*>(src);
+          rb[2 * s] = v.x; rb[2 * s + 1] = v.y;
+        } else {
+          rb[2 * s] = src[0]; rb[2 * s + 1] = src[1];
+        }
+      }
+    }
+  };
+  auto store_tiles = [&](int buf, const T (&ra)[2 * NU], const T (&rb)[2 * NU]) {
+#pragma unroll
+    for (int s = 0; s < NU; ++s) {
+      const int u = tid + 256 * s;
+      {
+        const int k = u / (BT / 2), r2 = (u % (BT / 2)) * 2;
+        *reinterpret_cast<T2*>(&As[buf][k][r2]) = T2{ra[2 * s], ra[2 * s + 1]};
+      }
+      if (TRANSB == 0) {
+        const int k = u / (BT / 2), r2 = (u % (BT / 2)) * 2;
+        *reinterpret_cast<T2*>(&Bs[buf][k][r2]) = T2{rb[2 * s], rb[2 * s + 1]};
+      } else {
+        const int nn = (u / 8) ^ bswz(u % 8 * 2), k2 = (u % 8) * 2;
+        Bs[buf][k2][nn] = rb[2 * s];
+        Bs[buf][k2 + 1][nn] = rb[2 * s + 1];
+      }
+    }
+  };
+
+  T4 acc[MI][MI];
+#pragma unroll
+  for (int mi = 0; mi < MI; ++mi)
+#pragma unroll
+    for (int ni = 0; ni < MI; ++ni) acc[mi][ni] = T4{(T)0, (T)0, (T)0, (T)0};
+
+  const bool wave_live = (i0 + wm * WT < iend) && (j0 + wn * WT < g.N) &&
+                         !((g.mode == GEMM_LOWER) && (i0 + wm * WT + WT - 1 < j0 + wn * WT));
+
+  const int nk = (ke - kb) / GBK;
+  const int l15 = lane & 15, l4 = lane >> 4;
+  auto multiply = [&](int buf) {
+    if (!wave_live) return;
+#pragma unroll
+    for (int kk = 0; kk < GBK; kk += 4) {
+      T af[MI], bf[MI];
+#pragma unroll
+      for (int mi = 0; mi < MI; ++mi) af[mi] = As[buf][kk + l4][wm * WT + mi * 16 + l15];
+#pragma unroll
+      for (int ni = 0; ni < MI; ++ni) bf[ni] = Bs[buf][kk + l4][(wn * WT + ni * 16 + l15) ^ bswz(kk + l4)];
+#pragma unroll
+      for (int mi = 0; mi < MI; ++mi)
+#pragma unroll
+        for (int ni = 0; ni < MI; ++ni)
+          acc[mi][ni] = gemm_mfma16(bf[ni], af[mi], acc[mi][ni]);
+    }
+  };
+  constexpr bool DEEP = (BT == 64) || (sizeof(T) == 4);
+  auto run = [&](auto vec) {
+    if constexpr (!DEEP) {
+      if (nk > 0) {
+        load_tiles(vec, kb, raA, rbA);
+        store_tiles(0, raA, rbA);
+      }
+      __syncthreads();
+      for (int it = 0; it < nk; ++it) {
+        const int buf = it & 1;
+        if (it + 1 < nk) load_tiles(vec, kb + (it + 1) * GBK, raA, rbA);
+        multiply(buf);
+        if (it + 1 < nk) store_tiles(buf ^ 1, raA, rbA);
+        __syncthreads();
+      }
+      return;
+    }
+    if (nk > 0) {
+      load_tiles(vec, kb, raA, rbA);
+      if (nk > 1) load_tiles(vec, kb + GBK, raB, rbB);
+      store_tiles(0, raA, rbA);
+    }
+    __syncthreads();
+    int it = 0;
+    for (; it + 3 < nk; it += 2) {
+      load_tiles(vec, kb + (it + 2) * GBK, raA, rbA);
+      multiply(0);
+      store_tiles(1, raB, rbB);
+      __syncthreads();
+      load_tiles(vec, kb + (it + 3) * GBK, raB, rbB);
+      multiply(1);
+      store_tiles(0, raA, rbA);
+      __syncthreads();
+    }
+    const int rem = nk - it;
+    if (rem == 1) {
+      multiply(0);
+    } else if (rem == 2) {
+      multiply(0);
+      store_tiles(1, raB, rbB);
+      __syncthreads();
+      multiply(1);
+    } else if (rem == 3) {
+      load_tiles(vec, kb + (it + 2) * GBK, raA, rbA);
+      multiply(0);
+      store_tiles(1, raB, rbB);
+      __syncthreads();
+      multiply(1);
+      store_tiles(0, raA, rbA);
+      __syncthreads();
+      multiply(0);
+    }
+  };
+  if (a_vec && b_vec) run(std::true_type{}); else run(std::false_type{});
+
+  if (!wave_live) return;
+  const bool mask_diag = (g.kflags & KF_MASK_DIAG) && (ti == tj);
+#pragma unroll
+  for (int mi = 0; mi < MI; ++mi) {
+    const int i = i0 + wm * WT + mi * 16 + l15;
+    if (i >= iend) continue;
+#pragma unroll
+    for (int ni = 0; ni < MI; ++ni) {
+#pragma unroll
+      for (int r = 0; r < 4; ++r) {
+        const int j = j0 + wn * WT + ni * 16 + (sizeof(T) == 8 ? l4 + 4 * r : 4 * l4 + r);
+        if (j >= g.N) continue;
+        if (mask_diag && i < j) continue;
+        T* dst = C + (size_t)((TRANSB && g.cols && !g.cols_c_off) ? g.cols[j] : j) * g.ldc + i;
+        T v = (T)g.alpha * acc[mi][ni][r];
+        if (g.beta != 0.0) v += (T)g.beta * (*dst);
+        *dst = v;
+      }
+    }
+  }
diff --git a/poisson-gpfa_amd/csrc/linalg.hip b/poisson-gpfa_amd/csrc/linalg.hip
--- a/poisson-gpfa_amd/csrc/linalg.hip
+++ b/poisson-gpfa_amd/csrc/linalg.hip
@@ -24,17 +24,7 @@
   return per * g.nbatch;
 }
 
-int gemm(pgpfa_ctx* c, bool transb, GemmP g, bool f32) {
-  const bool live_cols = g.cols && c->cur_ndev;
-  prof_begin(c, TAG_GEMM, live_cols ? 0.0 : gemm_flops(g));
-  if (c->prof.on && c->prof.open) {
-    char key[176];
-    std::snprintf(key, sizeof key, "%s %s M=%d N=%s%d K=%d%s batch=%d%s%s%s", f32 ? "f32" : "f64", transb ? "NN" : "NT", g.M, live_cols ? "<=" : "", g.N,
-                  g.K, g.kseg ? " (segmented)" : "", std::max(g.nbatch, 1), g.mode == GEMM_LOWER ? " lower" : "",
-                  g.kflags ? " triangular-k" : "", g.rtab ? " block-sparse" : "");
-    c->prof.recs.back().shape = key;
-    if (live_cols && c->live_gemm_collect) c->live_gemms.emplace_back(key, gemm_flops(g) / std::max(g.N, 1));
-  }
+static int gemm_decide(pgpfa_ctx* c, GemmP& g, bool f32) {
   if (g.bm == 0) {
     const long long t128 = (long long)((g.M + GBM - 1) / GBM) * ((g.N + GBN - 1) / GBN) * std::max(g.nbatch, 1);
     g.bm = ((!f32 || c->f32_tile64) && c->mfma && (g.rtab || t128 < c->small_tile_below)) ? 64 : 128;
@@ -51,14 +41,34 @@
     ksplit = std::min(std::min(8, (int)(k_eff / (tiles < 64 ? 32.0 : 64.0))), (c->splitk_target + tiles - 1) / tiles);
     while (ksplit > 1 && (size_t)ksplit * g.nbatch * g.M * g.N > c->gemm_part_len) --ksplit;
   }
+  return ksplit;
+}
+
+static GemmP gemm_split_parts(const GemmP& g, int ksplit, double* part) {
+  GemmP s = g;
+  s.C = part; s.sC = (long long)g.M * g.N; s.ldc = g.M; s.beta = 0.0;
+  s.nb_lo = g.nbatch; s.nbatch = g.nbatch * ksplit; s.sA_hi = 0; s.sB_hi = 0; s.sC_hi = (long long)g.nbatch * g.M * g.N;
+  s.ksplit = ksplit;
+  s.c_by_pos = 1;
+  s.cols_c_off = 1;
+  return s;
+}
+
+int gemm(pgpfa_ctx* c, bool transb, GemmP g, bool f32) {
+  const bool live_cols = g.cols && c->cur_ndev;
+  prof_begin(c, TAG_GEMM, live_cols ? 0.0 : gemm_flops(g));
+  if (c->prof.on && c->prof.open) {
+    char key[176];
+    std::snprintf(key, sizeof key, "%s %s M=%d N=%s%d K=%d%s batch=%d%s%s%s", f32 ? "f32" : "f64", transb ? "NN" : "NT", g.M, live_cols ? "<=" : "", g.N,
+                  g.K, g.kseg ? " (segmented)" : "", std::max(g.nbatch, 1), g.mode == GEMM_LOWER ? " lower" : "",
+                  g.kflags ? " triangular-k" : "", g.rtab ? " block-sparse" : "");
+    c->prof.recs.back().shape = key;
+    if (live_cols && c->live_gemm_collect) c->live_gemms.emplace_back(key, gemm_flops(g) / std::max(g.N, 1));
+  }
+  const int ksplit = gemm_decide(c, g, f32);
   hipError_t e;
   if (ksplit > 1) {
-    GemmP s = g;
-    s.C = c->gemm_part; s.sC = (long long)g.M * g.N; s.ldc = g.M; s.beta = 0.0;
-    s.nb_lo = g.nbatch; s.nbatch = g.nbatch * ksplit; s.sA_hi = 0; s.sB_hi = 0; s.sC_hi = (long long)g.nbatch * g.M * g.N;
-    s.ksplit = ksplit;
-    s.c_by_pos = 1;
-    s.cols_c_off = 1;
+    const GemmP s = gemm_split_parts(g, ksplit, c->gemm_part);
     e = gemm_launch(c->st, c->mfma, transb, s);
     if (e == hipSuccess) {
       hipLaunchKernelGGL(gemm_splitk_reduce_kernel, dim3((unsigned)(((size_t)g.M * g.N + 255) / 256), g.nbatch), dim3(256), 0, c->st, c->gemm_part,
@@ -70,6 +80,76 @@
   }
   prof_end(c);
   if (e != hipSuccess) return fail("gemm launch failed: %s", hipGetErrorString(e));
+  return 0;
+}
+
+int gemm_grouped(pgpfa_ctx* c, bool transb, const std::vector<GemmP>& probs, DevTable& tab, DevTable& red, int expect_blocks) {
+  std::vector<GemmP> plain;
+  std::vector<int> ks;
+  bool groupable = c->mfma && probs.size() <= (size_t)GEMM_GROUP_MAX;
+  size_t part_need = 0;
+  double flops = 0.0;
+  int maxM = 0, maxN = 0, maxK = 0;
+  for (GemmP g : probs) {
+    const int ksplit = gemm_decide(c, g, false);
+    if (g.bm != 64 || g.b_f32 || g.n_dev || (g.kseg != 0 && (transb || g.kseg % GBK != 0)) || (g.cols && !transb)) groupable = false;
+    if (ksplit > 1) {
+      if (g.nbatch != 1 || g.slots || g.cols || g.skip || g.beta != 0.0) groupable = false;
+      part_need += (size_t)ksplit * g.M * g.N;
+    }
+    flops += gemm_flops(g);
+    maxM = std::max(maxM, g.M); maxN = std::max(maxN, g.N); maxK = std::max(maxK, g.K);
+    plain.push_back(g);
+    ks.push_back(ksplit);
+  }
+  if (part_need > c->gemm_part_len) groupable = false;
+  if (!groupable) {
+    for (const GemmP& g : probs) CHK(gemm(c, transb, g));
+    return 0;
+  }
+  std::vector<GemmGroupTab> Tv(1);
+  std::vector<GemmReduceTab> Rv(1);
+  GemmGroupTab& T = Tv[0];
+  GemmReduceTab& Rd = Rv[0];
+  size_t part_off = 0;
+  int nblk = 0, nblk_plain = 0, nred = 0;
+  for (size_t i = 0; i < plain.size(); ++i) {
+    GemmP g = plain[i];
+    if (ks[i] > 1) {
+      GemmReduceEntry& r = Rd.ent[Rd.nent];
+      r.part = c->gemm_part + part_off; r.C = g.C; r.ksplit = ks[i]; r.M = g.M; r.N = g.N; r.ldc = g.ldc;
+      Rd.blk0[Rd.nent] = nred;
+      nred += (int)(((size_t)g.M * g.N + 255) / 256);
+      Rd.blk0[++Rd.nent] = nred;
+      g = gemm_split_parts(g, ks[i], c->gemm_part + part_off);
+      part_off += (size_t)ks[i] * g.M * g.N;
+    }
+    g.tilesM = g.rtab ? g.ntab : (g.M + g.bm - 1) / g.bm;
+    g.tilesN = (g.N + g.bm - 1) / g.bm;
+    g.ntiles = gemm_count_tiles(g.mode, g.tilesM, g.tilesN);
+    if (g.ntiles <= 0 || g.nbatch <= 0 || g.M <= 0 || g.N <= 0) continue;
+    if (g.rtab && g.mode != GEMM_FULL) return fail("gemm_grouped: a row-tile table needs GEMM_FULL");
+    T.blk0[T.nprob] = nblk;
+    T.prob[T.nprob] = g;
+    nblk += g.ntiles * g.nbatch;
+    nblk_plain += g.ntiles * plain[i].nbatch;
+    T.blk0[++T.nprob] = nblk;
+  }
+  if (expect_blocks >= 0 && nblk_plain != expect_blocks) return fail("internal: grouped launch of %d workgroups, its plan counted %d", nblk_plain, expect_blocks);
+  if (T.nprob == 0) return 0;
+  CHK(table_sync(c, tab, &T, offsetof(GemmGroupTab, prob) + (size_t)T.nprob * sizeof(GemmP), sizeof(GemmGroupTab)));
+  if (Rd.nent > 0) CHK(table_sync(c, red, &Rd, offsetof(GemmReduceTab, ent) + (size_t)Rd.nent * sizeof(GemmReduceEntry), sizeof(GemmReduceTab)));
+  prof_begin(c, TAG_GEMM, flops);
+  if (c->prof.on && c->prof.open) {
+    char key[176];
+    std::snprintf(key, sizeof key, "f64 %s grouped x%d M<=%d N<=%d K<=%d%s%s", transb ? "NN" : "NT", T.nprob, maxM, maxN, maxK, plain[0].kseg ? " (segmented)" : "",
+                  plain[0].mode == GEMM_LOWER ? " lower" : "");
+    c->prof.recs.back().shape = key;
+  }
+  hipError_t e = gemm_grouped_launch(c->st, transb, static_cast<const GemmGroupTab*>(tab.dev), nblk);
+  if (e == hipSuccess && Rd.nent > 0) e = gemm_reduce_grouped_launch(c->st, static_cast<const GemmReduceTab*>(red.dev), nred);
+  prof_end(c);
+  if (e != hipSuccess) return fail("grouped gemm launch failed: %s", hipGetErrorString(e));
   return 0;
 }
 
diff --git a/poisson-gpfa_amd/csrc/split.h b/poisson-gpfa_amd/csrc/split.h
--- a/poisson-gpfa_amd/csrc/split.h
+++ b/poisson-gpfa_amd/csrc/split.h
@@ -820,27 +820,30 @@
 }
 
 inline __global__ __launch_bounds__(256) void sum_groups_kernel(const double* __restrict__ part, int ngroups, int M, int N, int lower, double* __restrict__ out) {
-  __shared__ double red[4][64];
-  const int el = threadIdx.x & 63, q = threadIdx.x >> 6;
-  const size_t e = (size_t)blockIdx.x * 64 + el;
-  const bool in = e < (size_t)M * N;
-  const size_t ec = in ? e : 0;
-  const int i = (int)(ec % M), j = (int)(ec / M);
-  const size_t src = (lower > 0 && (i / lower) < (j / lower)) ? (size_t)i * M + j : ec;
-  const size_t gs = (size_t)M * N;
-  double s8[8] = {0.0, 0.0, 0.0, 0.0, 0.0, 0.0, 0.0, 0.0};
-  int g = q;
-  for (; g + 28 < ngroups; g += 32) {
-    double v[8];
-#pragma unroll
-    for (int u = 0; u < 8; ++u) v[u] = part[(size_t)(g + 4 * u) * gs + src];
-#pragma unroll
-    for (int u = 0; u < 8; ++u) s8[u] += v[u];
-  }
-  for (; g < ngroups; g += 4) s8[0] += part[(size_t)g * gs + src];
-  red[q][el] = ((s8[0] + s8[1]) + (s8[2] + s8[3])) + ((s8[4] + s8[5]) + (s8[6] + s8[7]));
-  __syncthreads();
-  if (q == 0 && in) out[e] = (red[0][el] + red[1][el]) + (red[2][el] + red[3][el]);
+#define SUM_GROUPS_BID blockIdx.x
+#include "sum_groups.inc"
+#undef SUM_GROUPS_BID
+}
+
+constexpr int SUM_GROUPS_MAX = 32;
+struct SumGroupsEntry { const double* part; double* out; int ngroups, M, N, lower; };
+struct SumGroupsTab {
+  int nent;
+  int blk0[SUM_GROUPS_MAX + 1];
+  SumGroupsEntry ent[SUM_GROUPS_MAX];
+};
+inline __global__ __launch_bounds__(256) void sum_groups_table_kernel(const SumGroupsTab* __restrict__ tab) {
+  const int bid = blockIdx.x, n = tab->nent;
+  int pr = 0;
+  while (pr + 1 < n && bid >= tab->blk0[pr + 1]) ++pr;
+  const SumGroupsEntry s = tab->ent[pr];
+  const double* __restrict__ part = s.part;
+  double* __restrict__ out = s.out;
+  const int ngroups = s.ngroups, M = s.M, N = s.N, lower = s.lower;
+  const unsigned bid_in = (unsigned)(bid - tab->blk0[pr]);
+#define SUM_GROUPS_BID bid_in
+#include "sum_groups.inc"
+#undef SUM_GROUPS_BID
 }
 
 constexpr int PACC_TS = 32;
diff --git a/poisson-gpfa_amd/csrc/split_plan.h b/poisson-gpfa_amd/csrc/split_plan.h
--- /dev/null
+++ b/poisson-gpfa_amd/csrc/split_plan.h
@@ -0,0 +1,75 @@
+#pragma once
+#include <algorithm>
+#include <cstddef>
+#include <vector>
+
+namespace split_plan {
+
+constexpr int NS = 256;
+constexpr size_t PACKED_BUDGET_BYTES = (size_t)1 << 30;
+
+struct Latent { int rk, kw; };
+
+struct Region { bool live; size_t Spart, Xpart, Ssum, Xsum, Zb; };
+
+struct SProb { int latent, first, per, ng, group0, M, K, kseg, tiles, blocks; };
+
+struct Plan {
+  int spsS, ngS, ngroups;
+  std::vector<Region> reg;
+  std::vector<SProb> sprobs;
+  std::vector<int> sblk0;
+  size_t total;
+};
+
+inline int lower_tiles(int rows, int bm) {
+  const int t = (rows + bm - 1) / bm;
+  return t * (t + 1) / 2;
+}
+
+inline int prefix_blocks(const std::vector<int>& blocks, std::vector<int>* blk0) {
+  blk0->assign(blocks.size() + 1, 0);
+  for (size_t i = 0; i < blocks.size(); ++i) (*blk0)[i + 1] = (*blk0)[i] + blocks[i];
+  return blk0->back();
+}
+
+inline size_t even(size_t n) { return (n + 1) & ~(size_t)1; }
+
+inline Plan plan_tail(const std::vector<Latent>& lat, int T, int nb, int sps) {
+  Plan P{};
+  P.spsS = std::max(1, (nb + NS - 1) / NS);
+  P.ngS = (nb + P.spsS - 1) / P.spsS;
+  P.ngroups = (nb + sps - 1) / sps;
+  size_t off = 0;
+  std::vector<int> blocks;
+  for (size_t k = 0; k < lat.size(); ++k) {
+    const int rk = lat[k].rk, kw = lat[k].kw;
+    Region r{};
+    r.live = rk > 0 && kw > 0;
+    if (r.live) {
+      const size_t rr = (size_t)rk * rk, rt = (size_t)rk * T;
+      r.Spart = off; off += even((size_t)P.ngS * rr);
+      r.Xpart = off; off += even((size_t)P.ngroups * rt);
+      r.Ssum = off; off += even(rr);
+      r.Xsum = off; off += even(rt);
+      r.Zb = off; off += even(rt);
+      const int nfull = nb / P.spsS, rem = nb - nfull * P.spsS;
+      for (int part = 0; part < 2; ++part) {
+        const int first = part ? nfull * P.spsS : 0, per = part ? rem : P.spsS, ng = part ? (rem ? 1 : 0) : nfull;
+        if (ng == 0 || per == 0) continue;
+        SProb s{};
+        s.latent = (int)k; s.first = first; s.per = per; s.ng = ng; s.group0 = part ? nfull : 0;
+        s.M = rk; s.kseg = kw; s.K = per * kw;
+        s.tiles = lower_tiles(rk, 64); s.blocks = s.tiles * ng;
+        P.sprobs.push_back(s);
+        blocks.push_back(s.blocks);
+      }
+    }
+    P.reg.push_back(r);
+  }
+  prefix_blocks(blocks, &P.sblk0);
+  P.total = off;
+  return P;
+}
+
+}
diff --git a/poisson-gpfa_amd/csrc/sum_groups.inc b/poisson-gpfa_amd/csrc/sum_groups.inc
--- /dev/null
+++ b/poisson-gpfa_amd/csrc/sum_groups.inc
@@ -0,0 +1,21 @@
+  __shared__ double red[4][64];
+  const int el = threadIdx.x & 63, q = threadIdx.x >> 6;
+  const size_t e = (size_t)SUM_GROUPS_BID * 64 + el;
+  const bool in = e < (size_t)M * N;
+  const size_t ec = in ? e : 0;
+  const int i = (int)(ec % M), j = (int)(ec / M);
+  const size_t src = (lower > 0 && (i / lower) < (j / lower)) ? (size_t)i * M + j : ec;
+  const size_t gs = (size_t)M * N;
+  double s8[8] = {0.0, 0.0, 0.0, 0.0, 0.0, 0.0, 0.0, 0.0};
+  int g = q;
+  for (; g + 28 < ngroups; g += 32) {
+    double v[8];
+#pragma unroll
+    for (int u = 0; u < 8; ++u) v[u] = part[(size_t)(g + 4 * u) * gs + src];
+#pragma unroll
+    for (int u = 0; u < 8; ++u) s8[u] += v[u];
+  }
+  for (; g < ngroups; g += 4) s8[0] += part[(size_t)g * gs + src];
+  red[q][el] = ((s8[0] + s8[1]) + (s8[2] + s8[3])) + ((s8[4] + s8[5]) + (s8[6] + s8[7]));
+  __syncthreads();
+  if (q == 0 && in) out[e] = (red[0][el] + red[1][el]) + (red[2][el] + red[3][el]);
diff --git a/poisson-gpfa_amd/csrc/types.h b/poisson-gpfa_amd/csrc/types.h
--- a/poisson-gpfa_amd/csrc/types.h
+++ b/poisson-gpfa_amd/csrc/types.h
@@ -97,6 +97,19 @@
   }
 }
 
+constexpr int GEMM_GROUP_MAX = 64;
+struct GemmGroupTab {
+  int nprob;
+  int blk0[GEMM_GROUP_MAX + 1];
+  GemmP prob[GEMM_GROUP_MAX];
+};
+struct GemmReduceEntry { const double* part; double* C; int ksplit, M, N, ldc; };
+struct GemmReduceTab {
+  int nent;
+  int blk0[GEMM_GROUP_MAX + 1];
+  GemmReduceEntry ent[GEMM_GROUP_MAX];
+};
+
 constexpr int GBM = 128, GBN = 128, GBK = 16;
 
 typedef float float2_t __attribute__((ext_vector_type(2)));
@@ -139,5 +152,7 @@
 };
 
 hipError_t gemm_launch(hipStream_t st, bool use_mfma, bool transb, GemmP g, bool f32 = false);
+hipError_t gemm_grouped_launch(hipStream_t st, bool transb, const GemmGroupTab* tab, int nblocks);
+hipError_t gemm_reduce_grouped_launch(hipStream_t st, const GemmReduceTab* tab, int nblocks);
 
 }
```
